# CompVis/retrieval-augmented-diffusion-models

Hardware: AMD Instinct MI355X
Metric: images/sec at 256x256, 50 DDIM steps, k=4 OpenImages retrieval (higher is better)
Workload: dtype bf16; 1 GPU; BASELINE config #3: RDM sampling, exact kNN (k=4) over a synthetic 20927907 x 512 fp16 CLIP DB -> 50-step DDIM (eta 0, CFG scale 2.0) over the shipped-config UNet (400.9M params, random weights) -> VQ-f4 decode to 256x256; batch_per_gpu=64, global_batch=64, sampler_steps=50, k=4, db_rows=20927907, parallelism=dp1 (batch-sharded, weights + DB replicated, all-gather of images only), deterministic_mode=False

## Files before the change

### include/rdm_hip.h

```cpp
#ifndef RDM_HIP_H
#define RDM_HIP_H
#include <stddef.h>
#include <stdint.h>

#ifdef __cplusplus
extern "C" {
#endif

typedef struct rdm_ctx rdm_ctx;

#define RDM_MAX_LEVELS 8

typedef struct {
    int in_channels, out_channels, model_channels, num_res_blocks;
    int n_attention_resolutions, attention_resolutions[RDM_MAX_LEVELS];
    int n_channel_mult, channel_mult[RDM_MAX_LEVELS];
    int num_head_channels, context_dim;
} rdm_unet_cfg;

typedef struct {
    int embed_dim, n_embed, z_channels, ch, n_ch_mult, ch_mult[RDM_MAX_LEVELS];
    int num_res_blocks, out_ch, resolution, mid_attn, kl;
    int n_attn_resolutions, attn_resolutions[RDM_MAX_LEVELS];
} rdm_vq_cfg;
// ... 45 lines not shown
    int lower_order_final;
    int log_every_t;
    int T; const float* alphas_cumprod;
    int n_nodes; const int* nodes;
} rdm_unipc_args;

typedef struct {
    int timesteps;
    int batch, k, channels, height, width;
    int clip_denoised; float temperature;
    int T;
    const float* sqrt_recip_alphas_cumprod; const float* sqrt_recipm1_alphas_cumprod;
    const float* posterior_mean_coef1; const float* posterior_mean_coef2;
    const float* posterior_log_variance_clipped;
} rdm_ddpm_args;

int rdm_ctx_create(int device_id, rdm_ctx** out);
void rdm_ctx_destroy(rdm_ctx* ctx);
const char* rdm_last_error(rdm_ctx* ctx);
int rdm_release_scratch(rdm_ctx* ctx);
int rdm_set_stream(rdm_ctx* ctx, void* hip_stream);
const char* rdm_version(void);
int rdm_set_deterministic(rdm_ctx* ctx, int on);
int rdm_get_deterministic(rdm_ctx* ctx);

long long rdm_unet_manifest(const rdm_unet_cfg* cfg, char* buf, size_t buflen, size_t* blob_bytes);
long long rdm_vq_manifest(const rdm_vq_cfg* cfg, char* buf, size_t buflen, size_t* blob_bytes);
long long rdm_clip_manifest(const rdm_clip_cfg* cfg, char* buf, size_t buflen, size_t* blob_bytes);
int rdm_load_unet(rdm_ctx* ctx, const rdm_unet_cfg* cfg, const void* packed, size_t nbytes);
int rdm_load_vq(rdm_ctx* ctx, const rdm_vq_cfg* cfg, const void* packed, size_t nbytes);
int rdm_load_clip(rdm_ctx* ctx, const rdm_clip_cfg* cfg, const void* packed, size_t nbytes);
long long rdm_rarm_manifest(const rdm_rarm_cfg* cfg, char* buf, size_t buflen, size_t* blob_bytes);
int rdm_load_rarm(rdm_ctx* ctx, const rdm_rarm_cfg* cfg, const void* packed, size_t nbytes);

int rdm_unet_forward(rdm_ctx* ctx, const float* x, const int64_t* t, const float* context, int b, int k, int H, int W,
                     float* eps_out);

int rdm_ddim_num_intermediates(int S, int log_every_t);
int rdm_ddim_sample(rdm_ctx* ctx, const rdm_ddim_args* args, const float* x_T, const float* cond, const float* uncond,
                    const float* noise, float* z_out, float* x_inter, float* pred_x0_inter);
int rdm_plms_sample(rdm_ctx* ctx, const rdm_ddim_args* args, const float* x_T, const float* cond, const float* uncond,
                    float* z_out, float* x_inter, float* pred_x0_inter);
int rdm_dpmpp_sample(rdm_ctx* ctx, const rdm_dpmpp_args* args, const float* x_T, const float* cond, const float* uncond,
                     float* z_out, float* x_inter, float* pred_x0_inter);
int rdm_dpmpp_timesteps(const float* alphas_cumprod, int T, int S, int skip_type, int* nodes_out);
int rdm_unipc_sample(rdm_ctx* ctx, const rdm_unipc_args* args, const float* x_T, const float* cond, const float* uncond,
                     float* z_out, float* x_inter, float* pred_x0_inter);
int rdm_unipc_coefficients(const float* alphas_cumprod, int T, const int* nodes, int n_nodes, int j, int order, int variant, int corrector,
                           int lower_order_final, double* out);
int rdm_ddpm_sample(rdm_ctx* ctx, const rdm_ddpm_args* args, const float* x_T, const float* cond, const float* noise,
                    float* z_out);

int rdm_rng_words(uint64_t seed, uint32_t row, uint32_t step, uint32_t stream, uint32_t block, uint32_t* out);
int rdm_op_rng_words(rdm_ctx* ctx, uint64_t seed, int64_t row0, int64_t B, int64_t per_row, uint32_t step, uint32_t stream, uint32_t* out);
int rdm_op_randn(rdm_ctx* ctx, uint64_t seed, int64_t row0, int64_t B, int64_t per_row, uint32_t step, uint32_t stream, float* out);
int rdm_ddim_sample_seeded(rdm_ctx* ctx, const rdm_ddim_args* args, uint64_t seed, int64_t row0, const float* x_T, const float* cond,
                           const float* uncond, float* z_out, float* x_inter, float* pred_x0_inter);
int rdm_ddpm_sample_seeded(rdm_ctx* ctx, const rdm_ddpm_args* args, uint64_t seed, int64_t row0, const float* x_T, const float* cond,
                           float* z_out);
int rdm_dpmpp_sde_sample(rdm_ctx* ctx, const rdm_dpmpp_args* args, const float* x_T, const float* cond, const float* uncond,
                         const float* noise, float* z_out, float* x_inter, float* pred_x0_inter);
int rdm_dpmpp_sde_sample_seeded(rdm_ctx* ctx, const rdm_dpmpp_args* args, uint64_t seed, int64_t row0, const float* x_T, const float* cond,
                                const float* uncond, float* z_out, float* x_inter, float* pred_x0_inter);

int rdm_ddim_decode(rdm_ctx* ctx, const rdm_ddim_args* args, int t_start, const float* x_latent, const float* cond, const float* uncond,
                    const float* noise, float* z_out, float* x_inter, float* pred_x0_inter);
int rdm_ddim_decode_seeded(rdm_ctx* ctx, const rdm_ddim_args* args, int t_start, uint64_t seed, int64_t row0, const float* x_latent,
                           const float* cond, const float* uncond, float* z_out, float* x_inter, float* pred_x0_inter);
int rdm_ddim_encode(rdm_ctx* ctx, const rdm_ddim_args* args, int t_enc, const float* x0, const float* cond, const float* uncond,
                    float* z_out, float* x_inter);
int rdm_op_ddim_inverse_step(rdm_ctx* ctx, const float* x, const float* eps, long long n, int cfg, float scale, float sqrt_a_cur,
                             float sqrt_one_minus_a_cur, float sqrt_a_next, float sqrt_one_minus_a_next, float* x_out,
                             float* x_dup_or_null, float* pred_x0_or_null);
int rdm_op_q_sample_seeded(rdm_ctx* ctx, const float* x0, int64_t B, int64_t per_row, float sqrt_a, float sqrt_1ma, uint64_t seed,
                           int64_t row0, float* out);

int rdm_op_masked_blend(rdm_ctx* ctx, const float* x, const float* x0, const float* mask, const float* z_or_null, int64_t B, int C, int H,
                        int W, int mask_channels, float sqrt_a, float sqrt_1ma, float* out, float* x_dup_or_null);
int rdm_op_masked_blend_seeded(rdm_ctx* ctx, const float* x, const float* x0, const float* mask, int64_t B, int C, int H, int W,
                               int mask_channels, float sqrt_a, float sqrt_1ma, uint64_t seed, int64_t row0, uint32_t step, float* out,
                               float* x_dup_or_null);
int rdm_ddim_inpaint(rdm_ctx* ctx, const rdm_ddim_args* args, int t_start, const float* x_latent, const float* x0, const float* mask,
                     int mask_channels, const float* cond, const float* uncond, const float* noise, const float* q_noise, float* z_out,
                     float* x_inter, float* pred_x0_inter);
int rdm_ddim_inpaint_seeded(rdm_ctx* ctx, const rdm_ddim_args* args, int t_start, uint64_t seed, int64_t row0, const float* x_latent,
                            const float* x0, const float* mask, int mask_channels, const float* cond, const float* uncond, float* z_out,
                            float* x_inter, float* pred_x0_inter);
int rdm_unet_forward_guided(rdm_ctx* ctx, const float* x, int64_t t, const float* cond, const float* uncond, int B, int k, int H, int W,
                            float* eps_out);

int rdm_vq_decode(rdm_ctx* ctx, const float* z, int b, int force_not_quantize, float* img_out, int32_t* indices_out);
int rdm_vq_quantize(rdm_ctx* ctx, const float* z, int b, float* zq_out, int32_t* indices_out);
int rdm_vq_decode_indices(rdm_ctx* ctx, const int64_t* indices, int b, float* img_out);
int rdm_vq_decode_hw(rdm_ctx* ctx, const float* z, int b, int h, int w, int force_not_quantize, float* img_out, int32_t* indices_out);
int rdm_vq_quantize_hw(rdm_ctx* ctx, const float* z, int b, int h, int w, float* zq_out, int32_t* indices_out);
long long rdm_vqenc_manifest(const rdm_vq_cfg* cfg, char* buf, size_t buflen, size_t* blob_bytes);
int rdm_load_vqenc(rdm_ctx* ctx, const rdm_vq_cfg* cfg, const void* packed, size_t nbytes);
int rdm_vq_encode(rdm_ctx* ctx, const float* img, int b, float* z_out);
int rdm_vq_encode_indices(rdm_ctx* ctx, const float* img , int b, int64_t* indices_out ,
                          float* quant_out_or_null );
int rdm_vq_encode_hw(rdm_ctx* ctx, const float* img, int b, int H, int W, float* z_out);
int rdm_to_uint8(rdm_ctx* ctx, const float* img, int b, int c, int h, int w, uint8_t* out);

int rdm_rarm_forward(rdm_ctx* ctx, const int64_t* tokens, int b, int t, const float* context, int k, float* logits_out);
int rdm_rarm_sample(rdm_ctx* ctx, const rdm_rarm_sample_args* args, const int64_t* cond_tokens, const float* context,
                    const float* uniforms, int64_t* tokens_out);
int rdm_rarm_sample_top_p(rdm_ctx* ctx, const rdm_rarm_sample_args* args, float top_p, const int64_t* cond_tokens, const float* context,
                          const float* uniforms, int64_t* tokens_out);
int rdm_rarm_forward_seq(rdm_ctx* ctx, const int64_t* tokens, int b, int t, const float* context, int k, float* logits_out);
int rdm_rarm_nll(rdm_ctx* ctx, const int64_t* tokens, const int64_t* targets, int b, int t, const float* context, int k, float* nll_out);
int rdm_rarm_sample_prefill(rdm_ctx* ctx, const rdm_rarm_sample_args* args, float top_p, const int64_t* cond_tokens, const float* context,
                            const float* uniforms, int64_t* tokens_out);

int rdm_clip_encode_text(rdm_ctx* ctx, const int64_t* tokens, int b, float* out);
int rdm_clip_encode_image(rdm_ctx* ctx, const float* image, int b, float* out);
int rdm_clip_preprocess(rdm_ctx* ctx, const float* image, int b, int h, int w, float* out);
int rdm_clip_encode_image_raw(rdm_ctx* ctx, const float* image, int b, int h, int w, float* out);

int rdm_db_load(rdm_ctx* ctx, const void* emb, long long n, int dim, int dtype, int is_device);
long long rdm_db_size(rdm_ctx* ctx);
int rdm_knn(rdm_ctx* ctx, const float* q, int b, int k, uint32_t* idx_out, float* score_out);
int rdm_knn_f64(rdm_ctx* ctx, const float* q, int b, int k, uint32_t* idx_out, double* score_out);
int rdm_knn_last_fallback(rdm_ctx* ctx);
int rdm_db_gather(rdm_ctx* ctx, const uint32_t* idx, long long n_idx, float* out);
enum { RDM_KNN_SCAN_GENERIC = 1, RDM_KNN_SCAN_D512 = 2, RDM_KNN_SCAN_BULK = 3 };
typedef struct rdm_knn_form { int path, ksel, rescored, lists_per_block, queries_per_launch; float eps; } rdm_knn_form;
typedef struct rdm_knn_stages {
    int rows_cap, nlists_cap;
    float* qn; void* qh; void* ql;
    float* cand_s; uint32_t* cand_i;
    int* flag; double* tau; uint32_t* tau_idx; float* theta;
    int rows, nlists; rdm_knn_form form;
} rdm_knn_stages;
int rdm_knn_select(long long n, int dim, int b, int k, rdm_knn_form* form_out);
int rdm_op_knn_stages(rdm_ctx* ctx, const float* q, int b, int k, uint32_t* idx_out, float* score_out, rdm_knn_stages* stages);
int rdm_db_rows(rdm_ctx* ctx, long long row0, long long rows, void* out_f16);

int rdm_comm_unique_id(rdm_ctx* ctx, void* id128 );
int rdm_comm_init(rdm_ctx* ctx, const void* id128 , int rank, int world);
int rdm_comm_all_gather(rdm_ctx* ctx, const void* send , void* recv , size_t nbytes);
int rdm_comm_all_reduce_f32(rdm_ctx* ctx, float* buf , size_t count, int average);
int rdm_comm_destroy(rdm_ctx* ctx);

enum { RDM_PROF_CONV3X3 = 0, RDM_PROF_LINEAR = 1, RDM_PROF_KNN = 2, RDM_PROF_ATTENTION = 3, RDM_PROF_GROUPNORM = 4,
       RDM_PROF_LAYERNORM = 5,
       RDM_PROF_UPSCONV = 6  };
int rdm_prof_enable(rdm_ctx* ctx, int kind_mask);
int rdm_prof_collect(rdm_ctx* ctx, int kind, long long* launches, double* ms, double* flops);
int rdm_prof_reset(rdm_ctx* ctx);
int rdm_prof_dump(rdm_ctx* ctx, const char* path);
int rdm_calib_probe(rdm_ctx* ctx, void* buf , size_t buf_bytes, double mfma_ms, size_t stream_bytes, int stream_reps,
                    double* mfma_tflops , double* stream_gbps );
int rdm_debug_tap(rdm_ctx* ctx, void* buf , size_t nbytes, int block, int sub);

int rdm_op_linear(rdm_ctx* ctx, const void* a_bf16, const void* w_bf16, const float* bias, const void* residual_bf16,
                  void* out_bf16, float* out_f32, int M, int N, int K, int act, float alpha);
int rdm_op_linear_rowvec(rdm_ctx* ctx, const void* a_bf16, const void* w_bf16, const float* bias, const float* rowvec, int rows_per_group,
                         const void* residual_bf16, void* out_bf16, int M, int N, int K);
int rdm_op_linear_ln(rdm_ctx* ctx, const void* x_bf16, const void* w_bf16, const float* bias, const float* gamma, const float* beta,
                     void* out_bf16, int M, int N, int K, int act, float eps);
int rdm_op_conv3x3(rdm_ctx* ctx, const void* x0_bf16, const void* x1_bf16, int C0, int C1, const void* w_bf16,
                   const float* bias, const float* rowvec, int rowvec_ld, const void* residual_bf16, void* out_bf16,
                   int B, int Hin, int Win, int N, int stride, int ups);
int rdm_op_vq_nearest_code(rdm_ctx* ctx, const float* z , const float* codebook , long long M, int N, int E,
                           int32_t* idx_out );
int rdm_op_moments_f64(rdm_ctx* ctx, const float* x, int n, int d, double* sum, double* outer);
int rdm_op_knn_radius(rdm_ctx* ctx, const float* x, int n, int d, int k, float* radius2_out);
int rdm_op_manifold_hits(rdm_ctx* ctx, const float* probe , int m, const float* ref , const float* ref_radius2, int n, int d,
                         unsigned char* hit_out);
int rdm_op_manifold_counts(rdm_ctx* ctx, const float* probe , int m, const float* ref , const float* ref_radius2 ,
                           int n, int d, int32_t* count_out );
int rdm_op_nearest_d2(rdm_ctx* ctx, const float* probe , int m, const float* ref , int n, int d, float* d2_out );
int rdm_op_poly3_rowsums(rdm_ctx* ctx, const float* probe , int m, const float* ref , int n, int d, int groups,
                         int exclude_same_index, float gamma, float coef0, double* rowsum_out );
int rdm_op_rarm_sampler(rdm_ctx* ctx, const float* logits, int b, int vocab, int cfg, float guidance_scale, float temperature,
                        int top_k, const float* uniforms, int64_t* tokens_out);
int rdm_op_rarm_sampler_top_p(rdm_ctx* ctx, const float* logits, int b, int vocab, int cfg, float guidance_scale, float temperature,
                              int top_k, float top_p, const float* uniforms, int64_t* tokens_out, int32_t* kept_out);
int rdm_op_conv3x3_dgrad(rdm_ctx* ctx, const void* dy_bf16 , const void* w_bf16, void* dx_bf16 , int B, int H, int W,
                         int C, int N);
int rdm_op_conv3x3_wgrad(rdm_ctx* ctx, const void* x_bf16 , const void* dy_bf16 , float* dw , int B, int H,
                         int W, int C, int N);
int rdm_op_groupnorm_bwd(rdm_ctx* ctx, const void* x_bf16, const void* dy_bf16, const float* gamma, const float* beta, int B, int HW, int C,
                         float eps, int silu, void* dx_bf16, float* dgamma, float* dbeta);
int rdm_op_layernorm_bwd(rdm_ctx* ctx, const void* x_bf16, const void* dy_bf16, const float* gamma, int M, int C, float eps, void* dx_bf16,
                         float* dgamma, float* dbeta);
int rdm_op_groupnorm_bwd_add(rdm_ctx* ctx, const void* x_bf16, const void* dy_bf16, const float* gamma, const float* beta, int B, int HW, int C,
                             float eps, int silu, const void* residual_bf16, void* dx_bf16, float* dgamma, float* dbeta);
int rdm_op_layernorm_bwd_add(rdm_ctx* ctx, const void* x_bf16, const void* dy_bf16, const float* gamma, int M, int C, float eps,
                             const void* residual_bf16, void* dx_bf16, float* dgamma, float* dbeta);
int rdm_op_linear_wgrad(rdm_ctx* ctx, const void* dy_bf16, const void* a_bf16, float* dw, long long M, int N, int K);
enum { RDM_WGRAD_CONV9_LW4 = 1, RDM_WGRAD_CONV9_LW5 = 2, RDM_WGRAD_CONV9_LW6 = 3, RDM_WGRAD_TN9 = 4, RDM_WGRAD_TN1 = 5, RDM_WGRAD_CONV_FALLBACK = 6,
       RDM_WGRAD_LINEAR_FALLBACK = 7 };
typedef struct rdm_wgrad_form { int path, Z, per_plane, remap; } rdm_wgrad_form;
int rdm_wgrad_select(int conv, int B, int H, int W, int C, int N, long long M, int K, rdm_wgrad_form* form_out);
int rdm_op_colsum(rdm_ctx* ctx, const void* x_bf16 , float* out , long long M, int N);
int rdm_op_transpose(rdm_ctx* ctx, const void* x_bf16 , void* y_bf16 , int rows, int cols);
int rdm_op_add(rdm_ctx* ctx, const void* a_bf16, const void* b_bf16, void* out_bf16, long long n);
int rdm_op_ddim_step(rdm_ctx* ctx, const float* x, const float* eps, const float* noise_or_null, long long n, int cfg, float scale, float a_t,
                     float a_prev, float sigma_t, float sqrt_one_minus_at, float temperature, float* x_prev, float* x_dup_or_null,
                     float* pred_x0_or_null);
int rdm_op_ddim_step_seeded(rdm_ctx* ctx, const float* x, const float* eps, long long n, int64_t per_row, int cfg, float scale, float a_t,
                            float a_prev, float sigma_t, float sqrt_one_minus_at, float temperature, uint64_t seed, int64_t row0,
                            uint32_t step, float* x_prev, float* x_dup_or_null, float* pred_x0_or_null);
int rdm_op_plms_step(rdm_ctx* ctx, const float* x, const float* eps, const float* e_prev_or_null, const float* h1_or_null,
                     const float* h2_or_null, const float* h3_or_null, long long n, int cfg, float scale, float a_t, float a_prev,
                     float sqrt_one_minus_at, int mode, int order, float* e_store_or_null, float* x_out, float* x_dup_or_null,
                     float* pred_x0_or_null);
int rdm_op_ddpm_step(rdm_ctx* ctx, const float* x, const float* eps, const float* noise_or_null, long long n, float sqrt_recip,
                     float sqrt_recipm1, float coef1, float coef2, float log_var, int clip, int nonzero, float temperature, float* x_prev);
int rdm_op_ddpm_step_seeded(rdm_ctx* ctx, const float* x, const float* eps, long long n, int64_t per_row, float sqrt_recip, float sqrt_recipm1,
                            float coef1, float coef2, float log_var, int clip, int nonzero, float temperature, uint64_t seed, int64_t row0,
                            uint32_t step, float* x_prev);
int rdm_op_dpmpp_step(rdm_ctx* ctx, const float* x, const float* eps, const float* m_prev_or_null, long long n, int cfg, float scale,
                      float sqrt_a_s, float sqrt_one_minus_a_s, float c_x, float c_0, float c_1, float* x_out, float* x_dup_or_null,
                      float* m_store_or_null, float* pred_x0_or_null);
int rdm_op_dpmpp_sde_step(rdm_ctx* ctx, const float* x, const float* eps, const float* m_prev_or_null, const float* noise, long long n, int cfg,
                          float scale, float sqrt_a_s, float sqrt_one_minus_a_s, float c_x, float c_0, float c_1, float c_n, float* x_out,
                          float* x_dup_or_null, float* m_store_or_null, float* pred_x0_or_null);
int rdm_op_dpmpp_sde_step_seeded(rdm_ctx* ctx, const float* x, const float* eps, const float* m_prev_or_null, long long n, int64_t per_row,
                                 int cfg, float scale, float sqrt_a_s, float sqrt_one_minus_a_s, float c_x, float c_0, float c_1, float c_n,
                                 uint64_t seed, int64_t row0, uint32_t step, float* x_out, float* x_dup_or_null, float* m_store_or_null,
                                 float* pred_x0_or_null);
int rdm_op_unipc_step(rdm_ctx* ctx, const float* u, const float* eps, const float* xc_prev_or_null, const float* h1_or_null,
                      const float* h2_or_null, const float* h3_or_null, long long n, int cfg, float scale, const double* coefficients,
                      float* xc_out_or_null, float* u_next, float* x_dup_or_null, float* m_store_or_null, float* pred_x0_or_null);
int rdm_op_silu(rdm_ctx* ctx, const float* x, const float* dy_or_null, void* out_bf16_or_f32, long long n);
int rdm_op_sumpool2(rdm_ctx* ctx, const void* x_bf16, void* out_bf16, int B, int H, int W, int C);
int rdm_op_q_sample(rdm_ctx* ctx, const float* x0, const float* noise, const float* sqrt_ac, const float* sqrt_1mac, float* out_or_null,
                    void* out_nhwc_bf16_or_null, int B, int C, int H, int W, int cpad);
int rdm_op_mse_loss(rdm_ctx* ctx, const void* eps_nhwc_bf16, const float* target, const float* coef_or_null, float* se, void* deps_nhwc_bf16_or_null,
                    int B, int C, int H, int W, int ldc);
int rdm_op_where_rows(rdm_ctx* ctx, const unsigned char* mask, const float* a, const float* x, float* out, long long rows, long long n);
int rdm_op_timestep_embedding(rdm_ctx* ctx, const int64_t* t, void* out_bf16, int B, int dim, int ld);
int rdm_op_colsum_samples(rdm_ctx* ctx, const void* x_bf16, void* out_bf16, int B, int HW, int N);
int rdm_op_expand2(rdm_ctx* ctx, const void* x_bf16, void* out_bf16, int B, int H, int W, int C, int mode);
int rdm_op_ema(rdm_ctx* ctx, float* shadow, const float* param, long long n, float one_minus_decay);
int rdm_op_adamw(rdm_ctx* ctx, float* p, const float* grad, float* exp_avg, float* exp_avg_sq, void* p_bf16_or_null, long long n, double lr,
                 double beta1, double beta2, double eps, double weight_decay, int step);
int rdm_op_adamw_multi(rdm_ctx* ctx, int n, float* const* p, const float* const* grad, float* const* exp_avg, float* const* exp_avg_sq,
                       void* const* p_bf16_or_null, const long long* numel, double lr, double beta1, double beta2, double eps, double weight_decay, int step);
int rdm_op_ema_multi(rdm_ctx* ctx, int n, float* const* shadow, const float* const* param, const long long* numel, float one_minus_decay);
int rdm_op_attention_bwd(rdm_ctx* ctx, const void* q, const void* k, const void* v, const void* o, const void* dout, int B, int n, int m, int heads,
                         void* dq, void* dk, void* dv);
int rdm_op_bmm(rdm_ctx* ctx, const void* a_bf16, const void* w_bf16, void* out_bf16_or_null, float* out_f32_or_null, int batch, int M, int N, int K,
               float alpha);
int rdm_op_heads(rdm_ctx* ctx, const void* x_bf16, void* out_bf16, int B, int n, int H, int D, int ldx, int mode);
int rdm_op_transpose_batched(rdm_ctx* ctx, const void* x_bf16, void* y_bf16, int batch, int rows, int cols);
int rdm_op_softmax(rdm_ctx* ctx, const float* scores, void* p_bf16, long long rows, int n, int n_valid );
int rdm_op_softmax_bwd(rdm_ctx* ctx, const void* p_bf16, const float* dp, void* ds_bf16, long long rows, int n);
int rdm_op_geglu(rdm_ctx* ctx, const void* pre_bf16, const void* dh_bf16_or_null, void* out_bf16, long long M, int F);
int rdm_op_groupnorm(rdm_ctx* ctx, const void* x0_bf16, const void* x1_bf16, int C0, int C1, int B, int HW,
                     const float* gamma, const float* beta, float eps, int silu, void* out_bf16);
int rdm_op_layernorm(rdm_ctx* ctx, const void* x, int in_is_f32, const float* gamma, const float* beta, int M, int C,
                     float eps, void* out_bf16);
int rdm_op_layernorm_f32(rdm_ctx* ctx, const float* x, const float* gamma, const float* beta, int M, int C, float eps, float* out_f32);
int rdm_op_linear_res_f32(rdm_ctx* ctx, const void* a_bf16, const void* w_bf16, const float* bias, const float* res_f32, float* out_f32,
                          int M, int N, int K, int act);
int rdm_op_self_attention(rdm_ctx* ctx, const void* qk_bf16, const void* vt_bf16, int B, int n, int heads,
                          void* out_bf16);
int rdm_op_self_attention_qkv(rdm_ctx* ctx, const void* qkv_bf16, int B, int n, int heads, void* out_bf16);
int rdm_op_xattn_fused(rdm_ctx* ctx, const void* x_bf16, const float* ln_gamma, const float* ln_beta, float ln_eps, const void* G_bf16,
                       const void* U_bf16, const float* bias, const void* res_bf16, int B, int n, int C, int NP, int ncols, int group,
                       void* out_bf16);
int rdm_op_xattn_fused_ln3(rdm_ctx* ctx, void* x_bf16_inout, const float* ln_gamma, const float* ln_beta, float ln_eps, const void* G_bf16,
                           const void* U_bf16, const float* bias, int B, int n, int C, int NP, int ncols, int group,
                           const float* ln3_gamma, const float* ln3_beta, void* ln3_out_bf16);
int rdm_op_causal_attention_d64(rdm_ctx* ctx, const void* qkv_bf16, int ldq, int B, int n, int heads, float scale, void* out_bf16, int ldo,
                                void* kcache_bf16_or_null, void* vcache_bf16_or_null, int L);
enum { RDM_LINEAR_ROWS_REFUSED = 0, RDM_LINEAR_ROWS_SGEMM = 1, RDM_LINEAR_ROWS_MGEMM = 2, RDM_LINEAR_ROWS_TILED = 3 };
typedef struct rdm_linear_rows_form { int kernel, ma, nb, u, nw, ln, geglu; } rdm_linear_rows_form;
int rdm_linear_rows_select(int M, int N, int K, int act, int ln, int deterministic, rdm_linear_rows_form* form_out);
int rdm_op_linear_rows(rdm_ctx* ctx, const void* a_bf16_or_null, const float* ln_x_f32_or_null, const float* ln_gamma, const float* ln_beta,
                       const void* w_bf16, const float* bias_or_null, const float* res_f32_or_null, void* out_bf16_or_null, float* out_f32_or_null,
                       int M, int N, int K, int act);
int rdm_op_rarm_decode_attention(rdm_ctx* ctx, const void* q_bf16, int ldq, const void* k_new_bf16_or_null, const void* v_new_bf16_or_null,
                                 void* kcache_bf16, void* vcache_bf16, long long batch_stride, int row_stride, long long head_stride, int nkv, int pos,
                                 float scale, void* out_bf16, int ldo, int heads, int batch);
int rdm_op_rarm_xattn_decode(rdm_ctx* ctx, float* x_f32_inout, const float* ln_gamma, const float* ln_beta, float ln_eps, const void* G_bf16,
                             const void* UT_bf16, const float* bias, int B2, int Bc, int C, int NP, int heads, int k, const float* ln3_gamma_or_null,
                             const float* ln3_beta_or_null, void* ln3_out_bf16_or_null);
int rdm_op_rarm_embed(rdm_ctx* ctx, const int64_t* tokens, int tok_ld, int tok_rows, int seq0, const float* emb_f32, const float* pos_t_f32,
                      float* x_f32, long long rows, int t, int C, int vocab, int L, int pos);
int rdm_op_vq_attention(rdm_ctx* ctx, const void* q_bf16, int ldq, const void* k_bf16, int ldk, const void* v_bf16, int ldv,
                        const float* bias_v_or_null, int B, int n, int C, float scale, void* out_bf16, int ldo);
int rdm_op_rarm_nll(rdm_ctx* ctx, const float* logits, long long rows, int vocab, const int64_t* targets, float* nll_out);
int rdm_op_causal_attention_d64_bwd(rdm_ctx* ctx, const void* qkv_bf16, int ldq, const void* out_bf16, int ldo, const void* dout_bf16, int lddo,
                                    int B, int n, int heads, float scale, void* dqkv_bf16, int ldd);
int rdm_op_rarm_nll_bwd(rdm_ctx* ctx, const float* logits, long long rows, int vocab, const int64_t* targets, float gscale, void* dlogits_bf16,
                        float* nll_out_or_null);
int rdm_op_embedding_grad(rdm_ctx* ctx, const int64_t* tokens, const void* dy_bf16, int M, int C, int V, float* dw_f32);
int rdm_op_head_conv(rdm_ctx* ctx, const void* x_bf16, const float* gn_gamma, const float* gn_beta, float gn_eps, const float* w,
                     const float* bias, int B, int H, int W, int C, int Cout, float* out_f32);
int rdm_op_small_attention(rdm_ctx* ctx, const void* q_bf16, int ldq, const void* k_bf16, const void* v_bf16, int ldkv,
                           int B, int nq, int nkv, int heads, int D, int causal, float scale, void* out_bf16, int ldo);
int rdm_op_small_attention_bwd(rdm_ctx* ctx, const void* q_bf16, int ldq, const void* k_bf16, const void* v_bf16, int ldkv, const void* dout_bf16, int ldo,
                               int B, int nq, int nkv, int heads, float scale, void* dq_bf16, void* dk_bf16, void* dv_bf16);
int rdm_op_conv_in(rdm_ctx* ctx, const float* x_f32, const float* w_f32, const float* bias_f32, int B, int Cin, int H, int W, int Cout,
                   void* out_bf16);
int rdm_op_conv_out(rdm_ctx* ctx, const void* x_bf16, const float* w_f32, const float* bias_f32, int B, int H, int W, int Cin, int Cout,
                    float* out_f32);

#ifdef __cplusplus
}
#endif
#endif
// ... 1 lines not shown
```

### retrieval-augmented-diffusion-models_amd/_lib.py

```python
import ctypes as C
import os

import numpy as np
import torch

_HERE = os.path.dirname(os.path.abspath(__file__))
LIB_PATH = os.environ.get("RDM_HIP_LIB") or os.path.join(_HERE, "librdm_hip.so")

RDM_MAX_LEVELS = 8
ACT_NONE, ACT_GEGLU, ACT_QUICKGELU, ACT_SILU = 0, 1, 2, 3
PROF_CONV3X3, PROF_LINEAR, PROF_KNN, PROF_ATTENTION, PROF_GROUPNORM, PROF_LAYERNORM, PROF_UPSCONV = range(7)


class UNetCfg(C.Structure):
    _fields_ = [("in_channels", C.c_int), ("out_channels", C.c_int), ("model_channels", C.c_int),
                ("num_res_blocks", C.c_int), ("n_attention_resolutions", C.c_int),
                ("attention_resolutions", C.c_int * RDM_MAX_LEVELS), ("n_channel_mult", C.c_int),
                ("channel_mult", C.c_int * RDM_MAX_LEVELS), ("num_head_channels", C.c_int), ("context_dim", C.c_int)]


class VqCfg(C.Structure):
    _fields_ = [("embed_dim", C.c_int), ("n_embed", C.c_int), ("z_channels", C.c_int), ("ch", C.c_int),
                ("n_ch_mult", C.c_int), ("ch_mult", C.c_int * RDM_MAX_LEVELS), ("num_res_blocks", C.c_int),
                ("out_ch", C.c_int), ("resolution", C.c_int), ("mid_attn", C.c_int), ("kl", C.c_int),
# ... 8 lines not shown
class RarmSampleArgs(C.Structure):
    _fields_ = [("batch", C.c_int), ("k", C.c_int), ("cond_len", C.c_int), ("steps", C.c_int), ("temperature", C.c_float),
                ("top_k", C.c_int), ("guidance_scale", C.c_float)]


class LinearRowsForm(C.Structure):
    _fields_ = [("kernel", C.c_int), ("ma", C.c_int), ("nb", C.c_int), ("u", C.c_int), ("nw", C.c_int), ("ln", C.c_int), ("geglu", C.c_int)]


LINEAR_ROWS_REFUSED, LINEAR_ROWS_SGEMM, LINEAR_ROWS_MGEMM, LINEAR_ROWS_TILED = range(4)


class WgradForm(C.Structure):
    _fields_ = [("path", C.c_int), ("Z", C.c_int), ("per_plane", C.c_int), ("remap", C.c_int)]


WGRAD_PATHS = (None, "conv9<4>", "conv9<5>", "conv9<6>", "tn9", "tn1", "conv_fallback", "linear_fallback")


class ClipCfg(C.Structure):
    _fields_ = [("embed_dim", C.c_int), ("image_resolution", C.c_int), ("vision_layers", C.c_int),
                ("vision_width", C.c_int), ("vision_patch_size", C.c_int), ("context_length", C.c_int),
                ("vocab_size", C.c_int), ("transformer_width", C.c_int), ("transformer_heads", C.c_int),
                ("transformer_layers", C.c_int)]


class DdimArgs(C.Structure):
    _fields_ = [("S", C.c_int), ("batch", C.c_int), ("k", C.c_int), ("channels", C.c_int), ("height", C.c_int),
                ("width", C.c_int), ("eta", C.c_float), ("temperature", C.c_float),
                ("unconditional_guidance_scale", C.c_float), ("log_every_t", C.c_int), ("T", C.c_int),
                ("alphas_cumprod", C.POINTER(C.c_float))]


class DpmppArgs(C.Structure):
    _fields_ = [("batch", C.c_int), ("k", C.c_int), ("channels", C.c_int), ("height", C.c_int), ("width", C.c_int),
                ("unconditional_guidance_scale", C.c_float), ("order", C.c_int), ("lower_order_final", C.c_int),
                ("log_every_t", C.c_int), ("T", C.c_int), ("alphas_cumprod", C.POINTER(C.c_float)), ("n_nodes", C.c_int),
                ("nodes", C.POINTER(C.c_int))]


DPMPP_SKIP_TYPES = {"time_uniform": 0, "logSNR": 1}


class UnipcArgs(C.Structure):
    _fields_ = [("batch", C.c_int), ("k", C.c_int), ("channels", C.c_int), ("height", C.c_int), ("width", C.c_int),
                ("unconditional_guidance_scale", C.c_float), ("order", C.c_int), ("variant", C.c_int), ("corrector", C.c_int),
                ("lower_order_final", C.c_int), ("log_every_t", C.c_int), ("T", C.c_int), ("alphas_cumprod", C.POINTER(C.c_float)),
                ("n_nodes", C.c_int), ("nodes", C.POINTER(C.c_int))]


UNIPC_VARIANTS = {"bh1": 0, "bh2": 1}
UNIPC_COEFFICIENTS = ("alpha", "sigma", "a_x", "a_t", "a_1", "a_2", "a_3", "b_x", "b_0", "b_1", "b_2", "order_c", "order_p")
PLMS_STEP, PLMS_EULER_A, PLMS_EULER_B = 0, 1, 2


class DdpmArgs(C.Structure):
    _fields_ = [("timesteps", C.c_int), ("batch", C.c_int), ("k", C.c_int), ("channels", C.c_int), ("height", C.c_int),
                ("width", C.c_int), ("clip_denoised", C.c_int), ("temperature", C.c_float), ("T", C.c_int),
                ("sqrt_recip_alphas_cumprod", C.POINTER(C.c_float)), ("sqrt_recipm1_alphas_cumprod", C.POINTER(C.c_float)),
                ("posterior_mean_coef1", C.POINTER(C.c_float)), ("posterior_mean_coef2", C.POINTER(C.c_float)),
                ("posterior_log_variance_clipped", C.POINTER(C.c_float))]


KNN_SCAN_PATHS = (None, "generic", "d512", "bulk")


class KnnForm(C.Structure):
    _fields_ = [("path", C.c_int), ("ksel", C.c_int), ("rescored", C.c_int), ("lists_per_block", C.c_int), ("queries_per_launch", C.c_int),
                ("eps", C.c_float)]


class KnnStages(C.Structure):
    _fields_ = [("rows_cap", C.c_int), ("nlists_cap", C.c_int), ("qn", C.c_void_p), ("qh", C.c_void_p), ("ql", C.c_void_p),
                ("cand_s", C.c_void_p), ("cand_i", C.c_void_p), ("flag", C.c_void_p), ("tau", C.c_void_p), ("tau_idx", C.c_void_p),
                ("theta", C.c_void_p), ("rows", C.c_int), ("nlists", C.c_int), ("form", KnnForm)]


_P = C.c_void_p
SIGNATURES = {
    "rdm_ctx_create": (C.c_int, [C.c_int, C.POINTER(_P)]),
    "rdm_ctx_destroy": (None, [_P]),
    "rdm_last_error": (C.c_char_p, [_P]),
    "rdm_set_stream": (C.c_int, [_P, _P]),
    "rdm_version": (C.c_char_p, []),
    "rdm_unet_manifest": (C.c_longlong, [C.POINTER(UNetCfg), C.c_char_p, C.c_size_t, C.POINTER(C.c_size_t)]),
    "rdm_vq_manifest": (C.c_longlong, [C.POINTER(VqCfg), C.c_char_p, C.c_size_t, C.POINTER(C.c_size_t)]),
    "rdm_clip_manifest": (C.c_longlong, [C.POINTER(ClipCfg), C.c_char_p, C.c_size_t, C.POINTER(C.c_size_t)]),
    "rdm_load_unet": (C.c_int, [_P, C.POINTER(UNetCfg), _P, C.c_size_t]),
    "rdm_load_vq": (C.c_int, [_P, C.POINTER(VqCfg), _P, C.c_size_t]),
    "rdm_load_clip": (C.c_int, [_P, C.POINTER(ClipCfg), _P, C.c_size_t]),
    "rdm_rarm_manifest": (C.c_longlong, [C.POINTER(RarmCfg), C.c_char_p, C.c_size_t, C.POINTER(C.c_size_t)]),
    "rdm_load_rarm": (C.c_int, [_P, C.POINTER(RarmCfg), _P, C.c_size_t]),
    "rdm_rarm_forward": (C.c_int, [_P, _P, C.c_int, C.c_int, _P, C.c_int, _P]),
    "rdm_rarm_sample": (C.c_int, [_P, C.POINTER(RarmSampleArgs), _P, _P, _P, _P]),
    "rdm_rarm_sample_top_p": (C.c_int, [_P, C.POINTER(RarmSampleArgs), C.c_float, _P, _P, _P, _P]),
    "rdm_rarm_forward_seq": (C.c_int, [_P, _P, C.c_int, C.c_int, _P, C.c_int, _P]),
    "rdm_rarm_nll": (C.c_int, [_P, _P, _P, C.c_int, C.c_int, _P, C.c_int, _P]),
    "rdm_rarm_sample_prefill": (C.c_int, [_P, C.POINTER(RarmSampleArgs), C.c_float, _P, _P, _P, _P]),
    "rdm_vq_decode_indices": (C.c_int, [_P, _P, C.c_int, _P]),
    "rdm_unet_forward": (C.c_int, [_P, _P, _P, _P, C.c_int, C.c_int, C.c_int, C.c_int, _P]),
    "rdm_ddim_num_intermediates": (C.c_int, [C.c_int, C.c_int]),
    "rdm_ddim_sample": (C.c_int, [_P, C.POINTER(DdimArgs), _P, _P, _P, _P, _P, _P, _P]),
    "rdm_plms_sample": (C.c_int, [_P, C.POINTER(DdimArgs), _P, _P, _P, _P, _P, _P]),
    "rdm_dpmpp_sample": (C.c_int, [_P, C.POINTER(DpmppArgs), _P, _P, _P, _P, _P, _P]),
    "rdm_dpmpp_timesteps": (C.c_int, [C.POINTER(C.c_float), C.c_int, C.c_int, C.c_int, C.POINTER(C.c_int)]),
    "rdm_unipc_sample": (C.c_int, [_P, C.POINTER(UnipcArgs), _P, _P, _P, _P, _P, _P]),
    "rdm_unipc_coefficients": (C.c_int, [C.POINTER(C.c_float), C.c_int, C.POINTER(C.c_int), C.c_int, C.c_int, C.c_int, C.c_int, C.c_int,
                                         C.c_int, C.POINTER(C.c_double)]),
    "rdm_ddpm_sample": (C.c_int, [_P, C.POINTER(DdpmArgs), _P, _P, _P, _P]),
    "rdm_rng_words": (C.c_int, [C.c_uint64, C.c_uint32, C.c_uint32, C.c_uint32, C.c_uint32, C.POINTER(C.c_uint32)]),
    "rdm_op_rng_words": (C.c_int, [_P, C.c_uint64, C.c_int64, C.c_int64, C.c_int64, C.c_uint32, C.c_uint32, _P]),
    "rdm_op_randn": (C.c_int, [_P, C.c_uint64, C.c_int64, C.c_int64, C.c_int64, C.c_uint32, C.c_uint32, _P]),
    "rdm_ddim_sample_seeded": (C.c_int, [_P, C.POINTER(DdimArgs), C.c_uint64, C.c_int64, _P, _P, _P, _P, _P, _P]),
    "rdm_ddpm_sample_seeded": (C.c_int, [_P, C.POINTER(DdpmArgs), C.c_uint64, C.c_int64, _P, _P, _P]),
    "rdm_dpmpp_sde_sample": (C.c_int, [_P, C.POINTER(DpmppArgs), _P, _P, _P, _P, _P, _P, _P]),
    "rdm_dpmpp_sde_sample_seeded": (C.c_int, [_P, C.POINTER(DpmppArgs), C.c_uint64, C.c_int64, _P, _P, _P, _P, _P, _P]),
    "rdm_unet_forward_guided": (C.c_int, [_P, _P, C.c_int64, _P, _P, C.c_int, C.c_int, C.c_int, C.c_int, _P]),
    "rdm_ddim_decode": (C.c_int, [_P, C.POINTER(DdimArgs), C.c_int, _P, _P, _P, _P, _P, _P, _P]),
    "rdm_ddim_decode_seeded": (C.c_int, [_P, C.POINTER(DdimArgs), C.c_int, C.c_uint64, C.c_int64, _P, _P, _P, _P, _P, _P]),
    "rdm_ddim_encode": (C.c_int, [_P, C.POINTER(DdimArgs), C.c_int, _P, _P, _P, _P, _P]),
    "rdm_op_ddim_inverse_step": (C.c_int, [_P, _P, _P, C.c_longlong, C.c_int, C.c_float, C.c_float, C.c_float, C.c_float, C.c_float, _P, _P, _P]),
    "rdm_op_q_sample_seeded": (C.c_int, [_P, _P, C.c_int64, C.c_int64, C.c_float, C.c_float, C.c_uint64, C.c_int64, _P]),
    "rdm_op_masked_blend": (C.c_int, [_P, _P, _P, _P, _P, C.c_int64, C.c_int, C.c_int, C.c_int, C.c_int, C.c_float, C.c_float, _P, _P]),
    "rdm_op_masked_blend_seeded": (C.c_int, [_P, _P, _P, _P, C.c_int64, C.c_int, C.c_int, C.c_int, C.c_int, C.c_float, C.c_float, C.c_uint64,
                                             C.c_int64, C.c_uint32, _P, _P]),
    "rdm_ddim_inpaint": (C.c_int, [_P, C.POINTER(DdimArgs), C.c_int, _P, _P, _P, C.c_int, _P, _P, _P, _P, _P, _P, _P]),
    "rdm_ddim_inpaint_seeded": (C.c_int, [_P, C.POINTER(DdimArgs), C.c_int, C.c_uint64, C.c_int64, _P, _P, _P, C.c_int, _P, _P, _P, _P, _P]),
    "rdm_vq_decode": (C.c_int, [_P, _P, C.c_int, C.c_int, _P, _P]),
    "rdm_release_scratch": (C.c_int, [_P]),
    "rdm_vq_quantize": (C.c_int, [_P, _P, C.c_int, _P, _P]),
    "rdm_vq_decode_hw": (C.c_int, [_P, _P, C.c_int, C.c_int, C.c_int, C.c_int, _P, _P]),
    "rdm_vq_quantize_hw": (C.c_int, [_P, _P, C.c_int, C.c_int, C.c_int, _P, _P]),
    "rdm_to_uint8": (C.c_int, [_P, _P, C.c_int, C.c_int, C.c_int, C.c_int, _P]),
    "rdm_clip_encode_text": (C.c_int, [_P, _P, C.c_int, _P]),
    "rdm_clip_encode_image": (C.c_int, [_P, _P, C.c_int, _P]),
    "rdm_clip_preprocess": (C.c_int, [_P, _P, C.c_int, C.c_int, C.c_int, _P]),
    "rdm_clip_encode_image_raw": (C.c_int, [_P, _P, C.c_int, C.c_int, C.c_int, _P]),
    "rdm_db_load": (C.c_int, [_P, _P, C.c_longlong, C.c_int, C.c_int, C.c_int]),
    "rdm_db_size": (C.c_longlong, [_P]),
    "rdm_knn": (C.c_int, [_P, _P, C.c_int, C.c_int, _P, _P]),
    "rdm_knn_f64": (C.c_int, [_P, _P, C.c_int, C.c_int, _P, _P]),
    "rdm_knn_last_fallback": (C.c_int, [_P]),
    "rdm_db_gather": (C.c_int, [_P, _P, C.c_longlong, _P]),
    "rdm_knn_select": (C.c_int, [C.c_longlong, C.c_int, C.c_int, C.c_int, C.POINTER(KnnForm)]),
    "rdm_op_knn_stages": (C.c_int, [_P, _P, C.c_int, C.c_int, _P, _P, C.POINTER(KnnStages)]),
    "rdm_db_rows": (C.c_int, [_P, C.c_longlong, C.c_longlong, _P]),
    "rdm_set_deterministic": (C.c_int, [_P, C.c_int]),
    "rdm_get_deterministic": (C.c_int, [_P]),
    "rdm_prof_enable": (C.c_int, [_P, C.c_int]),
    "rdm_prof_collect": (C.c_int, [_P, C.c_int, C.POINTER(C.c_longlong), C.POINTER(C.c_double), C.POINTER(C.c_double)]),
    "rdm_prof_reset": (C.c_int, [_P]),
    "rdm_prof_dump": (C.c_int, [_P, C.c_char_p]),
    "rdm_debug_tap": (C.c_int, [_P, _P, C.c_size_t, C.c_int, C.c_int]),
    "rdm_calib_probe": (C.c_int, [_P, _P, C.c_size_t, C.c_double, C.c_size_t, C.c_int, C.POINTER(C.c_double), C.POINTER(C.c_double)]),
    "rdm_comm_unique_id": (C.c_int, [_P, _P]),
    "rdm_comm_init": (C.c_int, [_P, _P, C.c_int, C.c_int]),
    "rdm_comm_all_gather": (C.c_int, [_P, _P, _P, C.c_size_t]),
    "rdm_comm_all_reduce_f32": (C.c_int, [_P, _P, C.c_size_t, C.c_int]),
    "rdm_comm_destroy": (C.c_int, [_P]),
    "rdm_vqenc_manifest": (C.c_longlong, [_P, _P, C.c_size_t, _P]),
    "rdm_load_vqenc": (C.c_int, [_P, _P, _P, C.c_size_t]),
    "rdm_vq_encode": (C.c_int, [_P, _P, C.c_int, _P]),
    "rdm_vq_encode_hw": (C.c_int, [_P, _P, C.c_int, C.c_int, C.c_int, _P]),
    "rdm_vq_encode_indices": (C.c_int, [_P, _P, C.c_int, _P, _P]),
    "rdm_op_q_sample": (C.c_int, [_P, _P, _P, _P, _P, _P, _P, C.c_int, C.c_int, C.c_int, C.c_int, C.c_int]),
    "rdm_op_mse_loss": (C.c_int, [_P, _P, _P, _P, _P, _P, C.c_int, C.c_int, C.c_int, C.c_int, C.c_int]),
    "rdm_op_where_rows": (C.c_int, [_P, _P, _P, _P, _P, C.c_longlong, C.c_longlong]),
    "rdm_op_timestep_embedding": (C.c_int, [_P, _P, _P, C.c_int, C.c_int, C.c_int]),
    "rdm_op_colsum_samples": (C.c_int, [_P, _P, _P, C.c_int, C.c_int, C.c_int]),
    "rdm_op_expand2": (C.c_int, [_P, _P, _P, C.c_int, C.c_int, C.c_int, C.c_int, C.c_int]),
    "rdm_op_linear": (C.c_int, [_P, _P, _P, _P, _P, _P, _P, C.c_int, C.c_int, C.c_int, C.c_int, C.c_float]),
    "rdm_op_conv3x3": (C.c_int, [_P, _P, _P, C.c_int, C.c_int, _P, _P, _P, C.c_int, _P, _P, C.c_int, C.c_int, C.c_int,
                                 C.c_int, C.c_int, C.c_int]),
    "rdm_op_vq_nearest_code": (C.c_int, [_P, _P, _P, C.c_longlong, C.c_int, C.c_int, _P]),
    "rdm_op_moments_f64": (C.c_int, [_P, _P, C.c_int, C.c_int, _P, _P]),
    "rdm_op_knn_radius": (C.c_int, [_P, _P, C.c_int, C.c_int, C.c_int, _P]),
    "rdm_op_manifold_hits": (C.c_int, [_P, _P, C.c_int, _P, _P, C.c_int, C.c_int, _P]),
    "rdm_op_manifold_counts": (C.c_int, [_P, _P, C.c_int, _P, _P, C.c_int, C.c_int, _P]),
    "rdm_op_nearest_d2": (C.c_int, [_P, _P, C.c_int, _P, C.c_int, C.c_int, _P]),
    "rdm_op_poly3_rowsums": (C.c_int, [_P, _P, C.c_int, _P, C.c_int, C.c_int, C.c_int, C.c_int, C.c_float, C.c_float, _P]),
    "rdm_op_rarm_sampler": (C.c_int, [_P, _P, C.c_int, C.c_int, C.c_int, C.c_float, C.c_float, C.c_int, _P, _P]),
    "rdm_op_rarm_sampler_top_p": (C.c_int, [_P, _P, C.c_int, C.c_int, C.c_int, C.c_float, C.c_float, C.c_int, C.c_float, _P, _P, _P]),
    "rdm_op_conv3x3_dgrad": (C.c_int, [_P, _P, _P, _P, C.c_int, C.c_int, C.c_int, C.c_int, C.c_int]),
    "rdm_op_conv3x3_wgrad": (C.c_int, [_P, _P, _P, _P, C.c_int, C.c_int, C.c_int, C.c_int, C.c_int]),
    "rdm_op_groupnorm_bwd": (C.c_int, [_P, _P, _P, _P, _P, C.c_int, C.c_int, C.c_int, C.c_float, C.c_int, _P, _P, _P]),
    "rdm_op_layernorm_bwd": (C.c_int, [_P, _P, _P, _P, C.c_int, C.c_int, C.c_float, _P, _P, _P]),
    "rdm_op_groupnorm_bwd_add": (C.c_int, [_P, _P, _P, _P, _P, C.c_int, C.c_int, C.c_int, C.c_float, C.c_int, _P, _P, _P, _P]),
    "rdm_op_layernorm_bwd_add": (C.c_int, [_P, _P, _P, _P, C.c_int, C.c_int, C.c_float, _P, _P, _P, _P]),
    "rdm_op_colsum": (C.c_int, [_P, _P, _P, C.c_longlong, C.c_int]),
    "rdm_op_transpose": (C.c_int, [_P, _P, _P, C.c_int, C.c_int]),
    "rdm_op_add": (C.c_int, [_P, _P, _P, _P, C.c_longlong]),
    "rdm_op_dpmpp_step": (C.c_int, [_P, _P, _P, _P, C.c_longlong, C.c_int, C.c_float, C.c_float, C.c_float, C.c_float, C.c_float, C.c_float,
                                    _P, _P, _P, _P]),
    "rdm_op_dpmpp_sde_step": (C.c_int, [_P, _P, _P, _P, _P, C.c_longlong, C.c_int, C.c_float, C.c_float, C.c_float, C.c_float, C.c_float,
                                        C.c_float, C.c_float, _P, _P, _P, _P]),
    "rdm_op_dpmpp_sde_step_seeded": (C.c_int, [_P, _P, _P, _P, C.c_longlong, C.c_int64, C.c_int, C.c_float, C.c_float, C.c_float, C.c_float,
                                               C.c_float, C.c_float, C.c_float, C.c_uint64, C.c_int64, C.c_uint32, _P, _P, _P, _P]),
    "rdm_op_unipc_step": (C.c_int, [_P, _P, _P, _P, _P, _P, _P, C.c_longlong, C.c_int, C.c_float, C.POINTER(C.c_double), _P, _P, _P, _P, _P]),
    "rdm_op_ddim_step": (C.c_int, [_P, _P, _P, _P, C.c_longlong, C.c_int, C.c_float, C.c_float, C.c_float, C.c_float, C.c_float, C.c_float,
                                   _P, _P, _P]),
    "rdm_op_ddim_step_seeded": (C.c_int, [_P, _P, _P, C.c_longlong, C.c_int64, C.c_int, C.c_float, C.c_float, C.c_float, C.c_float, C.c_float,
                                          C.c_float, C.c_uint64, C.c_int64, C.c_uint32, _P, _P, _P]),
    "rdm_op_plms_step": (C.c_int, [_P, _P, _P, _P, _P, _P, _P, C.c_longlong, C.c_int, C.c_float, C.c_float, C.c_float, C.c_float, C.c_int,
                                   C.c_int, _P, _P, _P, _P]),
    "rdm_op_ddpm_step": (C.c_int, [_P, _P, _P, _P, C.c_longlong, C.c_float, C.c_float, C.c_float, C.c_float, C.c_float, C.c_int, C.c_int,
                                   C.c_float, _P]),
    "rdm_op_ddpm_step_seeded": (C.c_int, [_P, _P, _P, C.c_longlong, C.c_int64, C.c_float, C.c_float, C.c_float, C.c_float, C.c_float, C.c_int,
                                          C.c_int, C.c_float, C.c_uint64, C.c_int64, C.c_uint32, _P]),
    "rdm_op_geglu": (C.c_int, [_P, _P, _P, _P, C.c_longlong, C.c_int]),
    "rdm_op_linear_ln": (C.c_int, [_P, _P, _P, _P, _P, _P, _P, C.c_int, C.c_int, C.c_int, C.c_int, C.c_float]),
    "rdm_op_linear_wgrad": (C.c_int, [_P, _P, _P, _P, C.c_longlong, C.c_int, C.c_int]),
    "rdm_op_ema": (C.c_int, [_P, _P, _P, C.c_longlong, C.c_float]),
    "rdm_op_silu": (C.c_int, [_P, _P, _P, _P, C.c_longlong]),
    "rdm_op_sumpool2": (C.c_int, [_P, _P, _P, C.c_int, C.c_int, C.c_int, C.c_int]),
    "rdm_op_adamw": (C.c_int, [_P, _P, _P, _P, _P, _P, C.c_longlong, C.c_double, C.c_double, C.c_double, C.c_double, C.c_double, C.c_int]),
    "rdm_op_attention_bwd": (C.c_int, [_P, _P, _P, _P, _P, _P, C.c_int, C.c_int, C.c_int, C.c_int, _P, _P, _P]),
    "rdm_op_bmm": (C.c_int, [_P, _P, _P, _P, _P, C.c_int, C.c_int, C.c_int, C.c_int, C.c_float]),
    "rdm_op_heads": (C.c_int, [_P, _P, _P, C.c_int, C.c_int, C.c_int, C.c_int, C.c_int, C.c_int]),
    "rdm_op_transpose_batched": (C.c_int, [_P, _P, _P, C.c_int, C.c_int, C.c_int]),
    "rdm_op_softmax": (C.c_int, [_P, _P, _P, C.c_longlong, C.c_int, C.c_int]),
    "rdm_op_softmax_bwd": (C.c_int, [_P, _P, _P, _P, C.c_longlong, C.c_int]),
    "rdm_op_groupnorm": (C.c_int, [_P, _P, _P, C.c_int, C.c_int, C.c_int, C.c_int, _P, _P, C.c_float, C.c_int, _P]),
    "rdm_op_layernorm": (C.c_int, [_P, _P, C.c_int, _P, _P, C.c_int, C.c_int, C.c_float, _P]),
    "rdm_op_layernorm_f32": (C.c_int, [_P, _P, _P, _P, C.c_int, C.c_int, C.c_float, _P]),
    "rdm_op_linear_res_f32": (C.c_int, [_P, _P, _P, _P, _P, _P, C.c_int, C.c_int, C.c_int, C.c_int]),
    "rdm_op_self_attention": (C.c_int, [_P, _P, _P, C.c_int, C.c_int, C.c_int, _P]),
    "rdm_op_self_attention_qkv": (C.c_int, [_P, _P, C.c_int, C.c_int, C.c_int, _P]),
    "rdm_op_head_conv": (C.c_int, [_P, _P, _P, _P, C.c_float, _P, _P, C.c_int, C.c_int, C.c_int, C.c_int, C.c_int, _P]),
    "rdm_op_conv_in": (C.c_int, [_P, _P, _P, _P, C.c_int, C.c_int, C.c_int, C.c_int, C.c_int, _P]),
    "rdm_op_conv_out": (C.c_int, [_P, _P, _P, _P, C.c_int, C.c_int, C.c_int, C.c_int, C.c_int, _P]),
    "rdm_op_linear_rowvec": (C.c_int, [_P, _P, _P, _P, _P, C.c_int, _P, _P, C.c_int, C.c_int, C.c_int]),
    "rdm_op_xattn_fused_ln3": (C.c_int, [_P, _P, _P, _P, C.c_float, _P, _P, _P, C.c_int, C.c_int, C.c_int, C.c_int, C.c_int, C.c_int, _P, _P, _P]),
    "rdm_op_xattn_fused": (C.c_int, [_P, _P, _P, _P, C.c_float, _P, _P, _P, _P, C.c_int, C.c_int, C.c_int, C.c_int, C.c_int, C.c_int, _P]),
    "rdm_op_causal_attention_d64": (C.c_int, [_P, _P, C.c_int, C.c_int, C.c_int, C.c_int, C.c_float, _P, C.c_int, _P, _P, C.c_int]),
    "rdm_op_rarm_nll": (C.c_int, [_P, _P, C.c_longlong, C.c_int, _P, _P]),
    "rdm_linear_rows_select": (C.c_int, [C.c_int, C.c_int, C.c_int, C.c_int, C.c_int, C.c_int, C.POINTER(LinearRowsForm)]),
    "rdm_op_linear_rows": (C.c_int, [_P, _P, _P, _P, _P, _P, _P, _P, _P, _P, C.c_int, C.c_int, C.c_int, C.c_int]),
    "rdm_wgrad_select": (C.c_int, [C.c_int, C.c_int, C.c_int, C.c_int, C.c_int, C.c_int, C.c_longlong, C.c_int, C.POINTER(WgradForm)]),
    "rdm_op_rarm_decode_attention": (C.c_int, [_P, _P, C.c_int, _P, _P, _P, _P, C.c_longlong, C.c_int, C.c_longlong, C.c_int, C.c_int, C.c_float, _P,
                                               C.c_int, C.c_int, C.c_int]),
    "rdm_op_rarm_xattn_decode": (C.c_int, [_P, _P, _P, _P, C.c_float, _P, _P, _P, C.c_int, C.c_int, C.c_int, C.c_int, C.c_int, C.c_int, _P, _P, _P]),
    "rdm_op_rarm_embed": (C.c_int, [_P, _P, C.c_int, C.c_int, C.c_int, _P, _P, _P, C.c_longlong, C.c_int, C.c_int, C.c_int, C.c_int, C.c_int]),
    "rdm_op_vq_attention": (C.c_int, [_P, _P, C.c_int, _P, C.c_int, _P, C.c_int, _P, C.c_int, C.c_int, C.c_int, C.c_float, _P, C.c_int]),
    "rdm_op_causal_attention_d64_bwd": (C.c_int, [_P, _P, C.c_int, _P, C.c_int, _P, C.c_int, C.c_int, C.c_int, C.c_int, C.c_float, _P, C.c_int]),
    "rdm_op_rarm_nll_bwd": (C.c_int, [_P, _P, C.c_longlong, C.c_int, _P, C.c_float, _P, _P]),
    "rdm_op_embedding_grad": (C.c_int, [_P, _P, _P, C.c_int, C.c_int, C.c_int, _P]),
    "rdm_op_small_attention": (C.c_int, [_P, _P, C.c_int, _P, _P, C.c_int, C.c_int, C.c_int, C.c_int, C.c_int, C.c_int,
                                         C.c_int, C.c_float, _P, C.c_int]),
    "rdm_op_adamw_multi": (C.c_int, [_P, C.c_int, _P, _P, _P, _P, _P, _P, C.c_double, C.c_double, C.c_double, C.c_double, C.c_double, C.c_int]),
    "rdm_op_ema_multi": (C.c_int, [_P, C.c_int, _P, _P, _P, C.c_float]),
    "rdm_op_small_attention_bwd": (C.c_int, [_P, _P, C.c_int, _P, _P, C.c_int, _P, C.c_int, C.c_int, C.c_int, C.c_int, C.c_int, C.c_float, _P, _P, _P]),
}


def load_library(path: str = LIB_PATH):
    if not os.path.exists(path):
        raise ImportError(
            f"librdm_hip.so not found at {path}. Build it with `python -c 'import __graft_entry__ as g; g.build()'` "
            f"(or `make -C retrieval-augmented-diffusion-models_amd/csrc`). There is no CPU fallback.")
    lib = C.CDLL(path)
    for name, (res, args) in SIGNATURES.items():
        fn = getattr(lib, name)
        fn.restype, fn.argtypes = res, args
    return lib


lib = load_library()


def linear_rows_select(M, N, K, act=ACT_NONE, ln=False, deterministic=False):
    f = LinearRowsForm()
    rc = lib.rdm_linear_rows_select(int(M), int(N), int(K), int(act), int(bool(ln)), int(bool(deterministic)), C.byref(f))
    if rc != 0:
        raise RdmError(f"rdm_linear_rows_select({M}, {N}, {K}, act={act}, ln={ln}, deterministic={deterministic}) failed ({rc})")
    if f.kernel == LINEAR_ROWS_SGEMM:
        return ("sgemm", f.ma, f.nb, f.u, f.nw, bool(f.ln), bool(f.geglu))
    return (("refused", "sgemm", "mgemm", "tiled")[f.kernel],)


def wgrad_select(*shape):
    f = WgradForm()
    if len(shape) == 5:
        B, H, W, Cc, N = (int(v) for v in shape)
        rc = lib.rdm_wgrad_select(1, B, H, W, Cc, N, 0, 0, C.byref(f))
    elif len(shape) == 3:
        M, N, K = (int(v) for v in shape)
        rc = lib.rdm_wgrad_select(0, 0, 0, 0, 0, N, M, K, C.byref(f))
    else:
        raise RdmError(f"wgrad_select takes (B, H, W, C, N) or (M, N, K), got {shape}")
    if rc != 0:
        raise RdmError(f"rdm_wgrad_select{shape} failed ({rc})")
    return (WGRAD_PATHS[f.path], f.Z, f.per_plane, f.remap)


def knn_select(n, dim, b, k):
    f = KnnForm()
    if lib.rdm_knn_select(int(n), int(dim), int(b), int(k), C.byref(f)) != 0:
        raise RdmError(f"rdm_knn_select(n={n}, dim={dim}, b={b}, k={k}): arguments the search refuses")
    return {"path": KNN_SCAN_PATHS[f.path], "ksel": f.ksel, "rescored": f.rescored, "lists_per_block": f.lists_per_block,
            "queries_per_launch": f.queries_per_launch, "eps": float(f.eps)}


def _ptr(t):
    if t is None:
        return None
    if isinstance(t, torch.Tensor):
# ... 828 lines not shown

    def clip_encode_image(self, image):
        image = self._dev(image, torch.float32)
        cfg = self._need("clip_encode_image", "clip")
        if image.ndim != 4 or tuple(image.shape[1:]) != (3, cfg.image_resolution, cfg.image_resolution):
            raise RdmError(f"clip_encode_image: image must be [b,3,{cfg.image_resolution},{cfg.image_resolution}] (already resized / normalised), got {tuple(image.shape)}")
        out = torch.empty((image.shape[0], self.clip_cfg.embed_dim), device=self.device, dtype=torch.float32)
        self._check(lib.rdm_clip_encode_image(self._h, _ptr(image), image.shape[0], _ptr(out)))
        return out

    def clip_preprocess(self, image):
        image = self._dev(image, torch.float32)
        if image.ndim != 4 or image.shape[1] != 3:
            raise RdmError(f"clip_preprocess: image must be [b,3,h,w], got {tuple(image.shape)}")
        r = self._need("clip_preprocess", "clip").image_resolution
        out = torch.empty((image.shape[0], 3, r, r), device=self.device, dtype=torch.float32)
        self._check(lib.rdm_clip_preprocess(self._h, _ptr(image), image.shape[0], image.shape[2], image.shape[3], _ptr(out)))
        return out

    def clip_encode_image_raw(self, image):
        image = self._dev(image, torch.float32)
        if image.ndim != 4 or image.shape[1] != 3:
            raise RdmError(f"clip_encode_image_raw: image must be [b,3,h,w], got {tuple(image.shape)}")
        self._need("clip_encode_image_raw", "clip")
        out = torch.empty((image.shape[0], self.clip_cfg.embed_dim), device=self.device, dtype=torch.float32)
        self._check(lib.rdm_clip_encode_image_raw(self._h, _ptr(image), image.shape[0], image.shape[2], image.shape[3], _ptr(out)))
        return out

    def db_load(self, emb):
        if isinstance(emb, torch.Tensor) and emb.is_cuda:
            emb = emb.contiguous()
            dt = {torch.float16: 0, torch.float32: 1}[emb.dtype]
            self._check(lib.rdm_db_load(self._h, _ptr(emb), emb.shape[0], emb.shape[1], dt, 1))
            self._db_dim = int(emb.shape[1])
        else:
            emb = np.ascontiguousarray(emb.numpy() if isinstance(emb, torch.Tensor) else emb)
            dt = {np.dtype(np.float16): 0, np.dtype(np.float32): 1}[emb.dtype]
            self._check(lib.rdm_db_load(self._h, emb.ctypes.data_as(_P), emb.shape[0], emb.shape[1], dt, 0))
            self._db_dim = int(emb.shape[1])

    def db_size(self):
        return int(lib.rdm_db_size(self._h))

    def knn(self, q, k, f64=False):
        q = self._dev(q, torch.float32)
        if q.ndim != 2:
            raise RdmError(f"knn: queries must be [b,dim], got {tuple(q.shape)}")
        idx = torch.empty((q.shape[0], k), device=self.device, dtype=torch.int32)
        sc = torch.empty((q.shape[0], k), device=self.device, dtype=torch.float64 if f64 else torch.float32)
        fn = lib.rdm_knn_f64 if f64 else lib.rdm_knn
        self._check(fn(self._h, _ptr(q), q.shape[0], k, _ptr(idx), _ptr(sc)))
        return idx, sc

    def knn_last_fallback(self):
        return int(lib.rdm_knn_last_fallback(self._h))

    def knn_stages(self, q, k):
        q = self._dev(q, torch.float32)
        if q.ndim != 2:
            raise RdmError(f"knn_stages: queries must be [b,dim], got {tuple(q.shape)}")
        b, dim = q.shape
        n = self.db_size()
        form = knn_select(n, dim, b, k)
        rows = form["queries_per_launch"]
        ntiles = (n + 255) // 256
        cap = 8 * min(ntiles, torch.cuda.get_device_properties(self.device).multi_processor_count)
        dv = self.device
        t = {"idx": torch.empty((b, k), device=dv, dtype=torch.int32), "score": torch.empty((b, k), device=dv, dtype=torch.float32),
             "qn": torch.zeros((rows, dim), device=dv, dtype=torch.float32), "qh": torch.zeros((rows, dim), device=dv, dtype=torch.float16),
             "ql": torch.zeros((rows, dim), device=dv, dtype=torch.float16),
             "cand_s": torch.zeros(rows * cap * form["ksel"], device=dv, dtype=torch.float32),
             "cand_i": torch.zeros(rows * cap * form["ksel"], device=dv, dtype=torch.int32),
             "flag": torch.zeros(b, device=dv, dtype=torch.int32), "tau": torch.zeros(b, device=dv, dtype=torch.float64),
             "tau_idx": torch.zeros(b, device=dv, dtype=torch.int32), "theta": torch.zeros(b, device=dv, dtype=torch.float32)}
        st = KnnStages(rows_cap=rows, nlists_cap=cap)
        for name in ("qn", "qh", "ql", "cand_s", "cand_i", "flag", "tau", "tau_idx", "theta"):
            setattr(st, name, t[name].data_ptr())
        self._check(lib.rdm_op_knn_stages(self._h, _ptr(q), b, k, _ptr(t["idx"]), _ptr(t["score"]), C.byref(st)))
        used = st.rows * st.nlists * st.form.ksel
        for name in ("qn", "qh", "ql"):
            t[name] = t[name][:st.rows]
        for name in ("cand_s", "cand_i"):
            t[name] = t[name][:used].reshape(st.rows, st.nlists, st.form.ksel)
        t.update(form)
        return t

    def db_rows(self, row0, rows):
        dim = self._db_dim
        out = torch.empty((rows, dim), device=self.device, dtype=torch.float16)
        self._check(lib.rdm_db_rows(self._h, int(row0), int(rows), _ptr(out)))
        return out

    def db_gather(self, idx, dim):
        idx = idx.contiguous()
        out = torch.empty((idx.numel(), dim), device=self.device, dtype=torch.float32)
        self._check(lib.rdm_db_gather(self._h, _ptr(idx), idx.numel(), _ptr(out)))
        return out.reshape(tuple(idx.shape) + (dim,))

    def prof_enable(self, kinds=(0, 1)):
        if kinds is True:
            kinds = (PROF_CONV3X3, PROF_LINEAR)
        mask = 0
        for k in (kinds or ()):
            mask |= 1 << int(k)
        self._check(lib.rdm_prof_enable(self._h, mask))

    def set_deterministic(self, on: bool = True):
        self._check(lib.rdm_set_deterministic(self._h, int(bool(on))))

    @property
    def deterministic(self) -> bool:
        return lib.rdm_get_deterministic(self._h) == 1

    def comm_unique_id(self) -> bytes:
        buf = C.create_string_buffer(128)
        self._check(lib.rdm_comm_unique_id(self._h, buf))
        return buf.raw

    def new_comm_context(self):
        c = Context(self.device.index)
        c._side_stream = torch.cuda.Stream(self.device)
        c._check(lib.rdm_set_stream(c._h, C.c_void_p(c._side_stream.cuda_stream)))
        return c

    def comm_init(self, uid: bytes, rank: int, world: int):
        if len(uid) != 128:
            raise RdmError(f"comm_init: the unique id is 128 bytes, got {len(uid)}")
        self._check(lib.rdm_comm_init(self._h, C.create_string_buffer(uid, 128), int(rank), int(world)))
        self.comm_world = int(world)

    def comm_all_gather(self, local: torch.Tensor, world: int) -> torch.Tensor:
        local = local.contiguous()
        out = torch.empty((world,) + tuple(local.shape), device=self.device, dtype=local.dtype)
        self._check(lib.rdm_comm_all_gather(self._h, _ptr(local), _ptr(out), local.numel() * local.element_size()))
        return out

    def comm_all_reduce(self, buf: torch.Tensor, average=True):
        if buf.dtype != torch.float32 or not buf.is_contiguous():
            raise RdmError("comm_all_reduce: contiguous float32 tensor required")
        self._check(lib.rdm_comm_all_reduce_f32(self._h, _ptr(buf), buf.numel(), int(bool(average))))
        return buf

    def comm_destroy(self):
        self._check(lib.rdm_comm_destroy(self._h))
        self.comm_world = 0

    def prof_reset(self):
        self._check(lib.rdm_prof_reset(self._h))

    def debug_tap(self, buf, block, sub=0):
        self._tap_keepalive = buf
        self._check(lib.rdm_debug_tap(self._h, _ptr(buf) if buf is not None else None, 0 if buf is None else buf.numel() * buf.element_size(), int(block), int(sub)))

    def calib_probe(self, mfma_ms=800.0, stream_bytes=1 << 30, stream_reps=6):
        buf = torch.empty(max(1 << 20, 2 * stream_bytes), device=self.device, dtype=torch.uint8)
        tf, gb = C.c_double(0.0), C.c_double(0.0)
        self._check(lib.rdm_calib_probe(self._h, _ptr(buf), buf.numel(), float(mfma_ms), int(stream_bytes), int(stream_reps), C.byref(tf), C.byref(gb)))
        del buf
        return float(tf.value), float(gb.value)

    def prof_dump(self, path):
        self._check(lib.rdm_prof_dump(self._h, os.fsencode(path)))

    def prof_collect(self, kind):
        n, ms, fl = C.c_longlong(0), C.c_double(0), C.c_double(0)
        self._check(lib.rdm_prof_collect(self._h, kind, C.byref(n), C.byref(ms), C.byref(fl)))
        return int(n.value), float(ms.value), float(fl.value)

    def op_linear(self, a, w, bias=None, residual=None, act=ACT_NONE, alpha=1.0, out_f32=False):
        M, K = a.shape; N = w.shape[0]
        No = N // 2 if act == ACT_GEGLU else N
        ob = None if out_f32 else torch.empty((M, No), device=self.device, dtype=torch.bfloat16)
        of = torch.empty((M, No), device=self.device, dtype=torch.float32) if out_f32 else None
        self._check(lib.rdm_op_linear(self._h, _ptr(a), _ptr(w), _ptr(bias), _ptr(residual), _ptr(ob), _ptr(of), M, N, K,
                                      act, float(alpha)))
        return of if out_f32 else ob

    def op_linear_rowvec(self, a, w, bias, rowvec, rows_per_group, residual=None):
        M, K = a.shape; N = w.shape[0]
        assert rowvec.dtype == torch.float32 and rowvec.shape == ((M + rows_per_group - 1) // rows_per_group, N) and rowvec.is_contiguous()
        out = torch.empty((M, N), device=self.device, dtype=torch.bfloat16)
        self._check(lib.rdm_op_linear_rowvec(self._h, _ptr(a), _ptr(w), _ptr(bias), _ptr(rowvec), int(rows_per_group), _ptr(residual), _ptr(out), M, N, K))
        return out

    def op_linear_ln(self, x, w, bias, gamma, beta, act=ACT_NONE, eps=1e-5):
        M, K = x.shape; N = w.shape[0]
        out = torch.empty((M, N // 2 if act == ACT_GEGLU else N), device=self.device, dtype=torch.bfloat16)
        self._check(lib.rdm_op_linear_ln(self._h, _ptr(x), _ptr(w), _ptr(bias), _ptr(gamma), _ptr(beta), _ptr(out), M, N, K, act, float(eps)))
        return out

    def op_conv3x3(self, x0, w, bias, x1=None, rowvec=None, residual=None, stride=1, ups=0):
        B, Hin, Win, C0 = x0.shape
        C1 = 0 if x1 is None else x1.shape[3]
        N = w.shape[0]
        Ho = Hin * 2 if ups else (Hin // 2 if stride == 2 else Hin)
        Wo = Win * 2 if ups else (Win // 2 if stride == 2 else Win)
        out = torch.empty((B, Ho, Wo, N), device=self.device, dtype=torch.bfloat16)
        self._check(lib.rdm_op_conv3x3(self._h, _ptr(x0), _ptr(x1), C0, C1, _ptr(w), _ptr(bias), _ptr(rowvec),
                                       0 if rowvec is None else rowvec.shape[1], _ptr(residual), _ptr(out), B, Hin, Win, N,
                                       stride, ups))
        return out

    def op_rarm_sampler(self, logits, uniforms, guidance_scale=1.0, temperature=1.0, top_k=None, top_p=None, return_kept=False):
        top_p = check_top_p("op_rarm_sampler", top_p)
        logits = self._dev(logits, torch.float32); uniforms = self._dev(uniforms, torch.float32)
        b = uniforms.shape[0]
        cfg = guidance_scale > 1.0
        if logits.ndim != 2 or logits.shape[0] != (2 * b if cfg else b):
            raise RdmError(f"op_rarm_sampler: logits must be [{2 * b if cfg else b}, vocab], got {tuple(logits.shape)}")
        out = torch.empty((b,), device=self.device, dtype=torch.int64)
        k = int(top_k) if top_k is not None else 0
        if top_p is None and not return_kept:
            self._check(lib.rdm_op_rarm_sampler(self._h, _ptr(logits), b, logits.shape[1], int(cfg), float(guidance_scale), float(temperature),
                                                k, _ptr(uniforms), _ptr(out)))
            return out
        kept = torch.empty((b,), device=self.device, dtype=torch.int32) if return_kept else None
        self._check(lib.rdm_op_rarm_sampler_top_p(self._h, _ptr(logits), b, logits.shape[1], int(cfg), float(guidance_scale), float(temperature),
                                                  k, 1.0 if top_p is None else top_p, _ptr(uniforms), _ptr(out), _ptr(kept)))
        return (out, kept) if return_kept else out

    def op_conv3x3_dgrad(self, dy, w):
        B, H, W, N = dy.shape
        Cc = w.shape[3]
        dx = torch.empty((B, H, W, Cc), device=self.device, dtype=torch.bfloat16)
        self._check(lib.rdm_op_conv3x3_dgrad(self._h, _ptr(dy), _ptr(w), _ptr(dx), B, H, W, Cc, N))
        return dx

    def op_conv3x3_wgrad(self, x, dy):
        B, H, W, Cc = x.shape
        N = dy.shape[3]
        dw = torch.empty((N, 3, 3, Cc), device=self.device, dtype=torch.float32)
        self._check(lib.rdm_op_conv3x3_wgrad(self._h, _ptr(x), _ptr(dy), _ptr(dw), B, H, W, Cc, N))
        return dw

    def op_groupnorm_bwd(self, x, dy, gamma, beta, eps, silu, residual=None):
        B, HW, Cc = x.shape
        dx = torch.empty_like(x); dg = torch.empty((Cc,), device=self.device, dtype=torch.float32); db = torch.empty_like(dg)
        assert residual is None or (residual.is_contiguous() and residual.numel() == x.numel())
        self._check(lib.rdm_op_groupnorm_bwd_add(self._h, _ptr(x), _ptr(dy), _ptr(gamma), _ptr(beta), B, HW, Cc, float(eps), int(silu), _ptr(residual),
                                                 _ptr(dx), _ptr(dg), _ptr(db)))
        return dx, dg, db

    def op_layernorm_bwd(self, x, dy, gamma, eps=1e-5, residual=None):
        M, Cc = x.shape
        dx = torch.empty_like(x); dg = torch.empty((Cc,), device=self.device, dtype=torch.float32); db = torch.empty_like(dg)
        assert residual is None or (residual.is_contiguous() and residual.numel() == x.numel())
        self._check(lib.rdm_op_layernorm_bwd_add(self._h, _ptr(x), _ptr(dy), _ptr(gamma), M, Cc, float(eps), _ptr(residual), _ptr(dx), _ptr(dg), _ptr(db)))
        return dx, dg, db

    def op_colsum(self, x):
        M, N = x.shape
        out = torch.empty((N,), device=self.device, dtype=torch.float32)
        self._check(lib.rdm_op_colsum(self._h, _ptr(x), _ptr(out), M, N))
        return out

    def op_transpose(self, x):
        r, c_ = x.shape
        y = torch.empty((c_, r), device=self.device, dtype=torch.bfloat16)
        self._check(lib.rdm_op_transpose(self._h, _ptr(x), _ptr(y), r, c_))
        return y

    def op_add(self, a, b):
        out = torch.empty_like(a)
        self._check(lib.rdm_op_add(self._h, _ptr(a), _ptr(b), _ptr(out), a.numel()))
        return out

    def op_linear_wgrad(self, dy, a):
        M, N = dy.shape; K = a.shape[1]
        dw = torch.empty((N, K), device=self.device, dtype=torch.float32)
        self._check(lib.rdm_op_linear_wgrad(self._h, _ptr(dy), _ptr(a), _ptr(dw), M, N, K))
        return dw

    @staticmethod
    def _ptr_array(ts, optional=False):
        arr = (C.c_void_p * len(ts))()
        for i, t in enumerate(ts):
            if t is None:
                assert optional
                arr[i] = None
            else:
                assert t.is_contiguous(), "tensor must be contiguous"
                arr[i] = t.data_ptr()
        return arr

    def op_adamw_multi(self, ps, gs, ms, vs, step, lr=1e-3, betas=(0.9, 0.999), eps=1e-8, weight_decay=1e-2, p_bf16s=None):
        n = len(ps)
        assert n == len(gs) == len(ms) == len(vs) and all(g.numel() == p.numel() and g.dtype == torch.float32 for p, g in zip(ps, gs))
        numel = (C.c_longlong * n)(*[p.numel() for p in ps])
        self._check(lib.rdm_op_adamw_multi(self._h, n, self._ptr_array(ps), self._ptr_array(gs), self._ptr_array(ms), self._ptr_array(vs),
                                           self._ptr_array(p_bf16s, True) if p_bf16s is not None else None, numel, float(lr), float(betas[0]),
                                           float(betas[1]), float(eps), float(weight_decay), int(step)))

    def op_ema_multi(self, shadows, ps, one_minus_decay):
        n = len(ps)
        numel = (C.c_longlong * n)(*[p.numel() for p in ps])
        self._check(lib.rdm_op_ema_multi(self._h, n, self._ptr_array(shadows), self._ptr_array(ps), numel, float(one_minus_decay)))

    def op_ema(self, shadow, p, one_minus_decay):
        self._check(lib.rdm_op_ema(self._h, _ptr(shadow), _ptr(p), p.numel(), float(one_minus_decay)))

    def op_silu(self, x, dy=None):
        out = torch.empty(x.shape, device=self.device, dtype=torch.bfloat16 if dy is None else torch.float32)
        self._check(lib.rdm_op_silu(self._h, _ptr(x), _ptr(dy) if dy is not None else None, _ptr(out), x.numel()))
        return out

    def op_q_sample(self, x0, noise, sqrt_ac, sqrt_1mac, want_nchw=True, cpad=0):
# ... 386 lines not shown
```

### retrieval-augmented-diffusion-models_amd/csrc/common.h

```cpp
#pragma once
#include <hip/hip_runtime.h>
#include <stdint.h>
#include <stdlib.h>

typedef uint16_t bf16_t;
typedef __attribute__((ext_vector_type(8))) short bf16x8;
typedef __attribute__((ext_vector_type(4))) short bf16x4;
typedef __attribute__((ext_vector_type(16))) float f32x16;
typedef __attribute__((ext_vector_type(4))) float f32x4;
typedef __attribute__((ext_vector_type(8))) _Float16 f16x8;

#define GLOBAL_AS __attribute__((address_space(1)))
#define LDS_AS __attribute__((address_space(3)))

__device__ __forceinline__ float bf2f(bf16_t v) { return __uint_as_float(((uint32_t)v) << 16); }
__device__ __forceinline__ bf16_t f2bf(float f) {
    uint32_t u = __float_as_uint(f);
    u += 0x7fffu + ((u >> 16) & 1u);
    return (bf16_t)(u >> 16);
}
__device__ __forceinline__ uint32_t pack2bf(float lo, float hi) {
    return (uint32_t)f2bf(lo) | ((uint32_t)f2bf(hi) << 16);
}
__device__ __forceinline__ uint32_t cvt_pk_bf16(float lo, float hi) {
    uint32_t r;
    asm("v_cvt_pk_bf16_f32 %0, %1, %2" : "=v"(r) : "v"(lo), "v"(hi));
    return r;
}
__device__ __forceinline__ float swap_adjacent_lane(float v) {
    return __builtin_bit_cast(float, __builtin_amdgcn_update_dpp(0, __builtin_bit_cast(int, v), 0xB1, 0xf, 0xf, true));
}
__device__ __forceinline__ float silu_f(float x) { return x * __builtin_amdgcn_rcpf(1.0f + __expf(-x)); }
__device__ __forceinline__ float gelu_erf_f(float x) {
    const float z = fabsf(x) * 0.70710678118654752f;
    const float t = __builtin_amdgcn_rcpf(1.0f + 0.3275911f * z);
    const float poly = t * (0.254829592f + t * (-0.284496736f + t * (1.421413741f + t * (-1.453152027f + t * 1.061405429f))));
    const float erf_abs = 1.0f - poly * __expf(-z * z);
    return 0.5f * x + 0.5f * fabsf(x) * erf_abs;
}
typedef float f32x2_t __attribute__((ext_vector_type(2)));
__device__ __forceinline__ f32x2_t gelu_erf_f2(f32x2_t x) {
    f32x2_t ax; ax.x = fabsf(x.x); ax.y = fabsf(x.y);
    const f32x2_t z = ax * 0.70710678118654752f;
    const f32x2_t d = z * 0.3275911f + 1.0f;
    f32x2_t t; t.x = __builtin_amdgcn_rcpf(d.x); t.y = __builtin_amdgcn_rcpf(d.y);
    const f32x2_t poly = t * (0.254829592f + t * (-0.284496736f + t * (1.421413741f + t * (-1.453152027f + t * 1.061405429f))));
    const f32x2_t a = (z * z) * -1.4426950408889634f;
    f32x2_t e; e.x = __builtin_amdgcn_exp2f(a.x); e.y = __builtin_amdgcn_exp2f(a.y);
    const f32x2_t erf_abs = 1.0f - poly * e;
    return (x + ax * erf_abs) * 0.5f;
}
__device__ __forceinline__ float quickgelu_f(float x) { return x * __builtin_amdgcn_rcpf(1.0f + __expf(-1.702f * x)); }

__device__ __forceinline__ void glds16(const void* gptr, void* lds_wave_base) {
    __builtin_amdgcn_global_load_lds((const GLOBAL_AS void*)gptr, (LDS_AS void*)lds_wave_base, 16, 0, 0);
}

enum { ACT_NONE = 0, ACT_GEGLU = 1, ACT_QUICKGELU = 2, ACT_SILU = 3, ACT_SOFTMAXG = 4 };

constexpr int RDM_EYE_OFFSET = 4096, RDM_EYE_N = 256;

constexpr int RDM_MAX_DEVICES = 32;
inline int rdm_cur_device() { int d = 0; (void)hipGetDevice(&d); return (d >= 0 && d < RDM_MAX_DEVICES) ? d : 0; }

inline int rdm_env_int(const char* value, int def) { return value ? atoi(value) : def; }

struct IgemmParams {
    const bf16_t* A0; const bf16_t* A1;
    int C0, C1;
    const bf16_t* W;
    int M, N, K;
    int Hin, Win, Hout, Wout, stride, ups;
    int phase2;
    int asym;
    float alpha;
    const float* bias;
    const float* rowvec;
    int rowvec_ld, rows_per_sample;
    const bf16_t* res_bf16;
    const float* res_f32;
    bf16_t* out_bf16; float* out_f32;
    int ldo;
    int act;
    int sm_group;
    long long sA, sW, sO;
    const void* zero_page;
    int ksplit; float* ws;
    int res_k;
    int lda, ldw;
    int l4_any_tiles;
    int res_wrap_rows;
    int a1_wrap_rows;
    const bf16_t* Wfrag;
    const float* ln_sb; float ln_inv_c, ln_eps;
    int dbg;
};
inline IgemmParams igemm_plain(int M, int N, int K, const void* zero_page) {
    IgemmParams p{}; p.M = M; p.N = N; p.K = K; p.alpha = 1.f; p.ldo = N; p.zero_page = zero_page;
    p.Hin = p.Win = p.Hout = p.Wout = 1; p.stride = 1; p.rows_per_sample = 1; return p;
}

struct Halo4Geom { int RS, NS, HPW, NROW, RSTR, NPR, NPT, HBYTES; };
__host__ __device__ inline Halo4Geom halo4_geom(int H, int W) {
    Halo4Geom g;
    const int HW = H * W;
    g.RS = (HW >= 256) ? 256 / W : H;
    g.NS = 256 / (g.RS * W);
    g.HPW = W + 2;
    g.NROW = g.NS * (g.RS + 2);
    g.RSTR = g.HPW * 144 + (W <= 16 ? 224 : 0);
    g.NPR = (g.HPW + 7) >> 3;
    g.NPT = g.NROW * g.NPR;
    g.HBYTES = (g.NROW * g.RSTR + 255) & ~255;
    return g;
}
constexpr int H4_HALO_MAX = 66560;
```

### retrieval-augmented-diffusion-models_amd/csrc/dispatch.hip

```cpp
#include "host.h"

static int gn_chunks(int HW) { const int n = HW / 64; return n < 1 ? 1 : n > 32 ? 32 : n; }

static bool skinny_rows(bool deterministic, bool single_row, int M, int single_max) {
    return deterministic ? single_row : (M <= 128 || (single_row && M <= single_max));
}
static int linear_kernel(SgemmParams& q, bool deterministic, bool single_row) {
    constexpr int SGEMM_MAX_ROWS = 4096;
    constexpr int SGEMM_GEGLU_MAX_ROWS = 192;
    if (skinny_rows(deterministic, single_row, q.M, q.act == ACT_GEGLU ? SGEMM_GEGLU_MAX_ROWS : SGEMM_MAX_ROWS)) {
        static const int mg_from = rdm_env_int(getenv("RDM_MGEMM_FROM"), 1536);
        if (!deterministic && single_row && mg_from > 0 && q.M >= mg_from && q.act != ACT_GEGLU && mgemm_supported(q)) return RDM_LINEAR_ROWS_MGEMM;
        q.fixed_split = deterministic ? 1 : 0;
        if (sgemm_supported(q)) return RDM_LINEAR_ROWS_SGEMM;
    }
    static const int mg_any = rdm_env_int(getenv("RDM_MGEMM_ANY"), 0);
    if (!single_row && mg_any > 0 && q.M >= mg_any && q.act != ACT_GEGLU && mgemm_supported(q)) return RDM_LINEAR_ROWS_MGEMM;
    return RDM_LINEAR_ROWS_TILED;
}
static bool linear_ln_takes(SgemmParams& q, bool deterministic, bool single_row) {
    constexpr int SGEMM_LN_MAX_ROWS = 192;
    if (!deterministic && q.M > SGEMM_LN_MAX_ROWS) return false;
    q.fixed_split = deterministic ? 1 : 0;
    return skinny_rows(deterministic, single_row, q.M, 1024) && sgemm_supported(q);
}

const bf16_t* Ops::derived(const bf16_t* W, int N, int K, int kind) {
    if (const_weights) return c->cached_derived(W, N, K, kind);
    if (ensure_bytes(c, &c->wfrag_tmp, &c->wfrag_tmp_bytes, rdm_ctx::derived_bytes(kind, N, K)) != 0) return nullptr;
    bf16_t* d = (bf16_t*)c->wfrag_tmp;
    return c->pack_derived(kind, W, d, N, K) == hipSuccess ? d : nullptr;
}

static SgemmParams skinny_params(const LinearOp& op) {
    SgemmParams q{}; q.A = op.A0; q.lda = op.C0; q.W = op.W; q.M = op.M; q.N = op.N; q.K = op.C0; q.bias = op.bias;
    q.act = op.act; q.res_f32 = op.res_f32; q.res_bf16 = op.res_bf16; q.out_f32 = op.out_f32; q.out_bf16 = op.out_bf16;
    q.ldo = op.act == ACT_GEGLU ? op.N / 2 : op.N;
    return q;
}
bool Ops::lin4_takes(const LinearOp& op) {
    if (c->deterministic) return false;
    IgemmParams t = base(op.M, op.N, op.C0 + op.C1);
    t.C0 = op.C0; t.C1 = op.C1; t.W = (const bf16_t*)blob; t.Wfrag = t.W; t.out_bf16 = (bf16_t*)blob; t.a1_wrap_rows = op.a1_wrap_rows;
    if (op.res_wrap_rows > 0) { t.res_bf16 = (const bf16_t*)blob; t.res_wrap_rows = op.res_wrap_rows; }
    return lin4_supported(t, 1);
}
void Ops::linear(const LinearOp& op) {
    if (plan) return;
    const int M = op.M, N = op.N, K = op.C0 + op.C1;
    if (!op.A1 && op.C1 == 0 && !op.rowvec && op.alpha == 1.f) {
        SgemmParams q = skinny_params(op);
        const int kernel = linear_kernel(q, c->deterministic, op.single_row);
        if (kernel != RDM_LINEAR_ROWS_TILED) {
            const bool mid = kernel == RDM_LINEAR_ROWS_MGEMM;
            prof_begin(RDM_PROF_LINEAR, 2.0 * M * N * (double)K, M, N, K);
            check(mid ? launch_mgemm(q, c->stream) : launch_sgemm(q, c->stream), mid ? "mid-size linear" : "skinny linear");
            prof_end();
            return;
        }
    }
    IgemmParams p = base(M, N, K);
    p.A0 = op.A0; p.A1 = op.A1; p.C0 = op.C0; p.C1 = op.C1; p.W = op.W; p.bias = op.bias; p.alpha = op.alpha;
    p.act = op.act; p.res_bf16 = op.res_bf16; p.res_f32 = op.res_f32; p.out_bf16 = op.out_bf16; p.out_f32 = op.out_f32;
    p.a1_wrap_rows = op.a1_wrap_rows; p.res_wrap_rows = op.res_wrap_rows;
    if (op.rowvec) { p.rowvec = op.rowvec; p.rowvec_ld = op.rowvec_ld; p.rows_per_sample = op.rows_per_sample; }
    if (op.act == ACT_GEGLU) p.ldo = N / 2;
    {
        IgemmParams t = p; t.Wfrag = p.W;
        const int tile_rows = (N % 384 == 0) ? 128 : 256;
        const bool det_ok = op.sample_rows > 0 && op.sample_rows % tile_rows == 0;
        if (c->deterministic) t.l4_any_tiles = p.l4_any_tiles = 1;
        if ((!c->deterministic || det_ok) && lin4_supported(t, 1)) p.Wfrag = derived(p.W, N, K, op.act == ACT_GEGLU ? 2 : 1);
    }
    prof_begin(RDM_PROF_LINEAR, 2.0 * M * N * (double)K, M, N, K);
    check(launch_igemm(p, false, 1, c->stream), "linear");
    prof_end();
}
bool Ops::linear_ln(const LinearOp& op) {
    SgemmParams q = skinny_params(op);
    q.ln_x = op.ln_x; q.ln_g = op.ln_g; q.ln_b = op.ln_b; q.ln_eps = 1e-5f;
    if (!linear_ln_takes(q, c->deterministic, op.single_row)) return false;
    if (plan) return true;
    prof_begin(RDM_PROF_LINEAR, 2.0 * op.M * op.N * (double)op.C0, op.M, op.N, op.C0);
    check(launch_sgemm(q, c->stream), "skinny linear on a LayerNorm");
    prof_end();
    return true;
}
void Ops::conv3(const Conv3Op& op) {
    if (plan) return;
    const bf16_t* A0 = op.A0; const bf16_t* A1 = op.A1; const bf16_t* W = op.W; const float* bias = op.bias;
    const int C0 = op.C0, C1 = op.C1, B = op.B, Hin = op.Hin, Win = op.Win, N = op.N, stride = op.stride, ups = op.ups;
    const float* rowvec = op.rowvec; const bf16_t* res = op.res_bf16; bf16_t* out = op.out_bf16;
    const int Hout = ups ? Hin * 2 : (stride == 2 ? Hin / 2 : Hin), Wout = ups ? Win * 2 : (stride == 2 ? Win / 2 : Win);
    IgemmParams p = base(B * Hout * Wout, N, 9 * (C0 + C1));
    p.asym = op.asym;
    p.A0 = A0; p.A1 = A1; p.C0 = C0; p.C1 = C1; p.W = W; p.bias = bias;
    p.Hin = Hin; p.Win = Win; p.Hout = Hout; p.Wout = Wout; p.stride = stride; p.ups = ups;
    p.rowvec = rowvec; p.rowvec_ld = op.rowvec_ld; p.rows_per_sample = Hout * Wout; p.res_bf16 = res; p.out_bf16 = out;
    if (ups && !A1 && C1 == 0 && C0 % 64 == 0 && N % 8 == 0 && !rowvec && !res && stride == 1) {
        const bf16_t* wp = derived(W, N, C0, 5);
        if (wp) {
            IgemmParams q = base(B * Hin * Win, N, 4 * C0);
            q.A0 = A0; q.C0 = C0; q.W = wp; q.bias = bias; q.out_bf16 = out; q.phase2 = 1;
            q.Hin = Hin; q.Win = Win; q.Hout = Hout; q.Wout = Wout; q.stride = 1; q.rows_per_sample = Hin * Win;
            q.sA = 0; q.sW = (long long)N * 4 * C0; q.sO = 0;
            prof_begin(RDM_PROF_UPSCONV, 2.0 * 4.0 * q.M * N * (double)q.K, 4 * q.M, N, q.K);
            check(launch_igemm(q, true, 4, c->stream), "conv3x3 on a 2x upsample, by phase");
            prof_end();
            return;
        }
    }
    const bool det_generic = c->deterministic && ((Hout * Wout) % 256 != 0);
    if (!det_generic && conv3x3_kernel(p) != CONV_IGEMM) p.Wfrag = derived(W, N, C0 + C1, 0);
    const int ks = (p.Wfrag && !c->deterministic) ? conv_halo_ksplit(p) : 1;
    if (ks > 1 && ensure_bytes(c, &c->splitk_ws, &c->splitk_ws_bytes, (size_t)ks * p.M * N * 4) == 0) { p.ksplit = ks; p.ws = (float*)c->splitk_ws; }
    prof_begin(RDM_PROF_CONV3X3, 2.0 * p.M * N * (double)p.K, p.M, N, p.K);
    check(launch_conv3x3(p, c->stream), "conv3x3");
    prof_end();
}
void Ops::tap(int stage, const void* ptr, size_t nbytes) {
    if (plan || !c->tap_buf || c->tap_block != cur_block || c->tap_sub != cur_layer * 16 + stage) return;
    if (nbytes > c->tap_bytes) nbytes = c->tap_bytes;
    check(hipMemcpyAsync(c->tap_buf, ptr, nbytes, hipMemcpyDeviceToDevice, c->stream), "debug tap");
}
void Ops::prof_begin(int kind, double work, int d0, int d1, int d2) {
    prof_open = (c->prof >> kind) & 1u;
    if (!prof_open) return;
    rdm_ctx::ProfRec r; r.a = c->prof_event(); r.b = c->prof_event(); r.kind = kind; r.flops = work; r.tag = tag; r.d0 = d0; r.d1 = d1; r.d2 = d2;
    hipEventRecord(r.a, c->stream); c->prof_recs.push_back(r);
}
void Ops::prof_end() { if (prof_open) hipEventRecord(c->prof_recs.back().b, c->stream); prof_open = false; }
void Ops::groupnorm(GnParams p) {
    if (plan) return;
    p.groups = 32; p.nchunk = gn_chunks(p.HW); p.partial = c->gn_partial;
    if (p.L0 <= 0) p.L0 = p.C0;
    if (p.L1 <= 0) p.L1 = p.C1;
    prof_begin(RDM_PROF_GROUPNORM, (double)p.B * p.HW * (p.C0 + p.C1) * 4.0, p.B * p.HW, p.C0 + p.C1, p.silu);
    check(launch_groupnorm(p, c->stream), "groupnorm");
    prof_end();
}
HeadParams Ops::head_params(HeadParams hp) const {
    hp.groups = 32;
    if (hp.gamma) { hp.partial = c->gn_partial; hp.nchunk = gn_chunks(hp.H * hp.W); }
    return hp;
}
void Ops::head(HeadParams hp, int Clog, bf16_t* tmp) {
    if (plan) return;
    hp = head_params(hp);
    const int B = hp.B, H = hp.H, W = hp.W, C = hp.C;
    if ((Clog <= 0 || Clog == C) && head_conv_supported(hp)) {
        if (hp.gamma) {
            GnParams p{}; p.x0 = hp.x; p.C0 = C; p.HW = H * W; p.B = B; p.groups = 32; p.L0 = C; p.nchunk = hp.nchunk; p.partial = c->gn_partial;
            prof_begin(RDM_PROF_GROUPNORM, (double)B * H * W * C * 2.0, B * H * W, C, 2);
            check(launch_gn_stats(p, c->stream), "head groupnorm statistics");
            prof_end();
        }
        check(launch_head_conv(hp, c->stream), "head conv");
        return;
    }
    groupnorm({.x0 = hp.x, .C0 = C, .HW = H * W, .B = B, .L0 = Clog, .gamma = hp.gamma, .beta = hp.beta, .eps = hp.eps, .silu = 1, .out = tmp});
    check(launch_conv_out(tmp, hp.w, hp.bias, hp.out, B, H, W, C, hp.Cout, c->stream), "conv_out");
}
void Ops::vq_nearest(const VqNearestOp& op) {
    if (plan) return;
    check(launch_vq_nearest(op.z, op.codebook, op.norms, op.M, op.N, op.E, op.ws, op.idx32, op.idx64, c->stream), "vq nearest code");
}
void Ops::layernorm(const LayerNormOp& op) {
    if (plan) return;
    const bool in_f32 = op.x_f32 != nullptr, out_f32 = op.out_f32 != nullptr;
    prof_begin(RDM_PROF_LAYERNORM, (double)op.M * op.C * ((in_f32 ? 4.0 : 2.0) + (out_f32 ? 4.0 : 2.0)), op.M, op.C, 0);
    check(launch_layernorm(in_f32 ? (const void*)op.x_f32 : op.x_bf16, in_f32, op.gamma, op.beta, out_f32 ? (void*)op.out_f32 : op.out_bf16, out_f32,
                           op.M, op.C, op.eps, c->stream, op.Clog < 0 ? op.C : op.Clog), "layernorm");
    prof_end();
}
void Ops::flash_d32(FlashParams f, int heads, int B) {
    if (plan) return;
    const int C = heads * 32, n = f.n;
    f.k = f.q + C; f.ldk = f.ldq; f.ldv = f.v ? f.ldq : 0; f.ldo = C; f.C = C;
    f.scale_log2e = (1.0f / sqrtf(32.f)) * 1.4426950408889634f;
    prof_begin(RDM_PROF_ATTENTION, 4.0 * B * heads * (double)n * n * 32, B, n, C);
    check(launch_flash_d32(f, heads, B, c->stream), "flash attention");
    prof_end();
}
void Ops::causal_d64(CausalD64Params f, int heads, int B, float scale) {
    if (plan) return;
    const int n = f.n;
    f.C = heads * 64; f.scale_log2e = scale * 1.4426950408889634f;
    prof_begin(RDM_PROF_ATTENTION, 2.0 * B * heads * (double)n * n * 64, B, n, f.C);
    check(launch_causal_d64(f, heads, B, c->stream), "causal attention");
    prof_end();
}
void Ops::vq_attention(const VqAttnParams& f, int B) {
    if (plan) return;
    prof_begin(RDM_PROF_ATTENTION, 6.0 * B * (double)f.n * f.n * f.C, B, f.n, f.C);
    check(launch_vq_attn_stream(f, B, c->stream), "vq attention");
    prof_end();
}
void Ops::small_attention(const SmallAttnParams& p, int D, int heads, int B, const char* what) {
    if (plan) return;
    check(launch_small_attention(p, D, heads, B, c->stream), what);
}
void Ops::xattn_fused(const XattnParams& q) {
    if (plan) return;
    prof_begin(RDM_PROF_LINEAR, 4.0 * q.rows * q.NP * (double)q.C, q.rows, q.NP, q.C);
    check(launch_xattn_fused(q, c->stream), "fused cross attention");
    prof_end();
}

int rdm_linear_rows_select(int M, int N, int K, int act, int ln, int deterministic, rdm_linear_rows_form* out) {
    if (!out || M < 1 || N < 1 || K < 1 || act < ACT_NONE || act > ACT_SILU) return -1;
    *out = rdm_linear_rows_form{};
    static const float some = 0.f;
    SgemmParams q{}; q.M = M; q.N = N; q.K = K; q.lda = K; q.act = act; q.ldo = act == ACT_GEGLU ? N / 2 : N;
    if (ln) { q.ln_x = &some; q.ln_g = &some; q.ln_b = &some; q.ln_eps = 1e-5f; }
    out->kernel = ln ? (linear_ln_takes(q, deterministic != 0, true) ? RDM_LINEAR_ROWS_SGEMM : RDM_LINEAR_ROWS_REFUSED) : linear_kernel(q, deterministic != 0, true);
    if (out->kernel == RDM_LINEAR_ROWS_SGEMM) {
        const SgemmForm f = sgemm_form(q);
        if (!sgemm_form_compiled(f)) return -3;
        out->ma = f.ma; out->nb = f.nb; out->u = f.u; out->nw = f.nw; out->ln = f.ln; out->geglu = f.geglu;
    }
    return 0;
}
```

### retrieval-augmented-diffusion-models_amd/csrc/host.h

```cpp
#pragma once
#include <stdarg.h>
#include <stdio.h>
#include <stdlib.h>
#include <string.h>

#include <cmath>
#include <string>
#include <unordered_map>
#include <vector>

#include "../../include/rdm_hip.h"
#include "kernels.h"
#include "knn.h"

#define RDM_CHECK_HIP(ctx, expr)                                                            \
    do {                                                                                    \
        hipError_t _e = (expr);                                                             \
        if (_e != hipSuccess) return (ctx)->fail(-2, "%s failed: %s (%s:%d)", #expr, hipGetErrorString(_e), __FILE__, __LINE__); \
    } while (0)
#define RDM_TRY(expr)            \
    do {                         \
        int _r = (expr);         \
        if (_r != 0) return _r;  \
    } while (0)
// ... 17 lines not shown
        const size_t off = total;
        text += std::to_string(off) + " " + std::to_string(nbytes) + " " + kind + " "; text += srcs; text += "\n";
        total += nbytes;
        return off;
    }
    size_t f32(const std::string& n, size_t numel) { return add("f32", n, numel * 4); }
    size_t bf16(const std::string& n, size_t numel) { return add("bf16", n, numel * 2); }
    size_t conv3(const std::string& n, size_t cout, size_t cin) { return add("conv3", n, cout * cin * 9 * 2); }
};

struct Arena {
    char* base = nullptr; size_t cap = 0, off = 0, peak = 0; bool planning = false;
    void reset() { off = 0; }
    void* alloc(size_t bytes) {
        off = (off + 255) & ~(size_t)255;
        void* p = base ? base + off : (void*)(uintptr_t)(off + 256);
        off += bytes;
        if (off > peak) peak = off;
        return p;
    }
};

template <typename T> static void free_dev(T*& p, size_t& bytes) { if (p) (void)hipFree(p); p = nullptr; bytes = 0; }
struct ModelBase {
    char* blob = nullptr; size_t blob_bytes = 0; Arena arena; bool loaded = false;
    void release() { free_dev(blob, blob_bytes); free_dev(arena.base, arena.cap); loaded = false; }
};

inline int pad64(int c) { return (c + 63) & ~63; }
struct ResW { int cin, cout; size_t gn1g, gn1b, w1, b1, gn2g, gn2b, w2, b2, wsk, bsk; int emb_off; bool skip; int l0, l1, lout, p0, p1; };
constexpr int XA_NP = 128;

struct StW {
    int c, heads; size_t gng, gnb, win, bin, ln1g, ln1b, wqk, wv, wo1, bo1, ln2g, ln2b, wq2, wo2, bo2, ln3g, ln3b, wff1,
        bff1, wff2, bff2, wout, bout, wfo, bfo; int kv_off; long long xa_unit;
    int lc;
    bool v_follows;
};
struct ConvW { int c; size_t w, b; int lc; };
struct ULayer { int kind; int idx; };
struct UBlock { int where; std::vector<ULayer> layers; };

struct UNet : ModelBase {
    rdm_unet_cfg cfg{};
    std::vector<UBlock> blocks; std::vector<ResW> res; std::vector<StW> st; std::vector<ConvW> down, up;
    size_t te0w, te0b, te2w, te2b, embw, embb, kvw, cinw, cinb, outg, outb, outw, outbias;
    int emb_total = 0, kv_total = 0; long long xa_total = 0;
    bf16_t* xa_cache = nullptr; size_t xa_cache_bytes = 0;
    bf16_t* kv_cache = nullptr; size_t kv_cache_bytes = 0;
    float* emb_table = nullptr; size_t emb_table_bytes = 0;
    int ctx_rows = 0;
    void release() { free_dev(xa_cache, xa_cache_bytes); free_dev(kv_cache, kv_cache_bytes); free_dev(emb_table, emb_table_bytes); ModelBase::release(); }
};

struct VqRes { int cin, cout; size_t n1g, n1b, w1, b1, n2g, n2b, w2, b2, wsk, bsk; bool skip; };
struct VqAttn { int c; size_t ng, nb, wq, bq, wk, bk, wv, bv, wo, bo; };
struct VqLevel {
    std::vector<VqRes> blocks;
    std::vector<VqAttn> attn;
    ConvW resample{};
};
struct VqMid { VqRes res1, res2; VqAttn attn; bool has_attn; };

struct VqModel : ModelBase {
    rdm_vq_cfg cfg{};
    bool wide = false;
    size_t codebook, pqw, pqb, cinw, cinb, noutg, noutb, coutw, coutb;
    VqMid mid;
    std::vector<VqLevel> levels;
    float* code_norms = nullptr;
    void release() { if (code_norms) (void)hipFree(code_norms); code_norms = nullptr; ModelBase::release(); }
};

struct VqEncModel : ModelBase {
    rdm_vq_cfg cfg{};
    bool wide = false;
    size_t cinw, cinb, noutg, noutb, coutw, coutb, qw, qb;
    std::vector<VqLevel> levels;
    VqMid mid;
};

struct ClipBlk { size_t ln1g, ln1b, wqkv, bqkv, wo, bo, ln2g, ln2b, wfc, bfc, wpj, bpj; };
struct ClipModel : ModelBase {
    rdm_clip_cfg cfg{};
    std::vector<ClipBlk> text, vis;
    size_t tok, pos, lnfg, lnfb, tproj;
    size_t conv1, cls, vpos, lnpreg, lnpreb, lnpostg, lnpostb, vproj;
};

struct RarmBlk { size_t ln1g, ln1b, wqkv, wo1, bo1, ln2g, ln2b, wq2, wo2, bo2, ln3g, ln3b, wff1, bff1, wff2, bff2; };
struct RarmModel : ModelBase {
    rdm_rarm_cfg cfg{}; int C = 0, kv_total = 0;
    std::vector<RarmBlk> blk;
    size_t emb, pos, kvw, wpo, bpo;
    char* cache = nullptr; size_t cache_bytes = 0;
    char* ctxkv = nullptr; size_t ctxkv_bytes = 0;
    char* state = nullptr; size_t state_bytes = 0;
    char* xa = nullptr; size_t xa_bytes = 0; int xa_B = 0, xa_k = 0;
    void release() { free_dev(cache, cache_bytes); free_dev(ctxkv, ctxkv_bytes); free_dev(state, state_bytes); free_dev(xa, xa_bytes); xa_B = xa_k = 0; ModelBase::release(); }
};

struct rdm_ctx {
    int device = 0; hipStream_t stream = nullptr; char err[512] = {0};
    void* zero_page = nullptr; float* eye3 = nullptr;
    UNet unet; VqModel vq; VqEncModel vqenc; ClipModel clip; RarmModel rarm; KnnDb db;
    float* gn_partial = nullptr; size_t gn_partial_bytes = 0;
    char* splitk_ws = nullptr; size_t splitk_ws_bytes = 0;
    char* samp = nullptr; size_t samp_bytes = 0;
    struct FragKey {
        const void* W; int N, K, kind; const void* aux;
        bool operator==(const FragKey& o) const { return W == o.W && N == o.N && K == o.K && kind == o.kind && aux == o.aux; }
    };
    struct FragKeyHash {
        size_t operator()(const FragKey& k) const {
            size_t h = std::hash<const void*>()(k.W);
            for (size_t v : {(size_t)k.N, (size_t)k.K, (size_t)k.kind, (size_t)(uintptr_t)k.aux}) h = (h ^ v) * 0x9E3779B97F4A7C15ull + (h >> 29);
            return h;
        }
    };
    struct FragVal { bf16_t* frag; float* sb; };
    std::unordered_map<FragKey, FragVal, FragKeyHash> wfrag;
    char* bwd_tmp = nullptr; size_t bwd_tmp_bytes = 0;
    char* wfrag_tmp = nullptr; size_t wfrag_tmp_bytes = 0;
    void drop_frags() { for (auto& kv : wfrag) { (void)hipFree(kv.second.frag); if (kv.second.sb) (void)hipFree(kv.second.sb); } wfrag.clear(); }
    static size_t derived_bytes(int kind, int N, int K) { return (size_t)N * K * 2 * (kind == 0 ? 9 : kind == 5 ? 16 : 1); }
    hipError_t pack_derived(int kind, const bf16_t* W, bf16_t* d, int N, int K) {
        return kind == 0 ? launch_conv_w_fragpack(W, d, N, K, stream)
             : kind == 5 ? launch_conv_phase_weights(W, d, N, K, stream)
                         : launch_lin_w_fragpack(W, d, N, K, K, kind == 2, stream);
    }
    const bf16_t* cached_derived(const bf16_t* W, int N, int K, int kind) {
        const FragKey key{W, N, K, kind, nullptr};
        auto it = wfrag.find(key);
        if (it != wfrag.end()) return it->second.frag;
        bf16_t* d = nullptr;
        if (hipMalloc((void**)&d, derived_bytes(kind, N, K)) != hipSuccess) return nullptr;
        if (pack_derived(kind, W, d, N, K) != hipSuccess) { (void)hipFree(d); return nullptr; }
        wfrag[key] = FragVal{d, nullptr};
        return d;
    }
    const float* zero_bias_pair(const float* b, int C) {
        const FragKey key{b, C, 2, 6, nullptr};
        auto it = wfrag.find(key);
        if (it != wfrag.end()) return it->second.sb;
        float* t = nullptr;
        if (hipMalloc((void**)&t, (size_t)2 * C * sizeof(float)) != hipSuccess) return nullptr;
        if (hipMemsetAsync(t, 0, (size_t)C * sizeof(float), stream) != hipSuccess ||
            hipMemcpyAsync(t + C, b, (size_t)C * sizeof(float), hipMemcpyDeviceToDevice, stream) != hipSuccess) { (void)hipFree(t); return nullptr; }
        wfrag[key] = FragVal{nullptr, t};
        return t;
    }
    bool deterministic = rdm_env_int(getenv("RDM_DETERMINISTIC"), 0) != 0;
    void* tap_buf = nullptr; size_t tap_bytes = 0; int tap_block = -1, tap_sub = 0;
    void* rccl_lib = nullptr; void* comm = nullptr; int comm_world = 0;
    unsigned prof = 0;
    struct ProfRec { hipEvent_t a, b; int kind; double flops; const char* tag; int d0, d1, d2; };
    std::vector<ProfRec> prof_recs; std::vector<hipEvent_t> prof_pool;
    hipEvent_t prof_event() {
        if (!prof_pool.empty()) { hipEvent_t e = prof_pool.back(); prof_pool.pop_back(); return e; }
        hipEvent_t e; hipEventCreate(&e); return e;
    }
    int fail(int code, const char* fmt, ...) {
        va_list ap; va_start(ap, fmt); vsnprintf(err, sizeof err, fmt, ap); va_end(ap); return code;
    }
};

inline int ensure_bytes(rdm_ctx* c, char** p, size_t* have, size_t need) {
    if (*have >= need) return 0;
    if (*p) { RDM_CHECK_HIP(c, hipStreamSynchronize(c->stream)); RDM_CHECK_HIP(c, hipFree(*p)); *p = nullptr; *have = 0; }
    RDM_CHECK_HIP(c, hipMalloc((void**)p, need));
    *have = need; return 0;
}

inline int ensure_gn_partial(rdm_ctx* c, int B) {
    const size_t need = (size_t)B * 32 * 64 * 2 * sizeof(float);
    return ensure_bytes(c, (char**)&c->gn_partial, &c->gn_partial_bytes, need);
}


struct LinearOp {
    const bf16_t* A0 = nullptr; const bf16_t* A1 = nullptr; int C0 = 0, C1 = 0;
    const float* ln_x = nullptr; const float* ln_g = nullptr; const float* ln_b = nullptr;
    const bf16_t* W = nullptr; const float* bias = nullptr;
    int M = 0, N = 0;
    int act = ACT_NONE;
    const bf16_t* res_bf16 = nullptr; const float* res_f32 = nullptr;
    bf16_t* out_bf16 = nullptr; float* out_f32 = nullptr;
    const float* rowvec = nullptr; int rowvec_ld = 0, rows_per_sample = 1;
    int a1_wrap_rows = 0, res_wrap_rows = 0;
    float alpha = 1.f;
    bool single_row = false;
    int sample_rows = 0;
};
struct Conv3Op {
    const bf16_t* A0 = nullptr; const bf16_t* A1 = nullptr; int C0 = 0, C1 = 0;
    const bf16_t* W = nullptr; const float* bias = nullptr;
    int B = 0, Hin = 0, Win = 0, N = 0, stride = 1, ups = 0;
    const bf16_t* res_bf16 = nullptr; bf16_t* out_bf16 = nullptr;
    const float* rowvec = nullptr; int rowvec_ld = 0;
    int asym = 0;
};
struct LayerNormOp {
    const float* x_f32 = nullptr; const bf16_t* x_bf16 = nullptr;
    const float* gamma = nullptr; const float* beta = nullptr;
    int M = 0, C = 0;
    float* out_f32 = nullptr; bf16_t* out_bf16 = nullptr;
    int Clog = -1;
    float eps = 1e-5f;
};
struct VqNearestOp {
    const float* z = nullptr; const float* codebook = nullptr; const float* norms = nullptr;
    long long M = 0; int N = 0, E = 0;
    char* ws = nullptr; int* idx32 = nullptr; long long* idx64 = nullptr;
};

struct Ops {
    rdm_ctx* c; Arena* ar; const char* blob; bool plan; int rc = 0;
    template <typename T> const T* w(size_t off) const { return (const T*)(blob + off); }
    bf16_t* abf(size_t n) { return (bf16_t*)ar->alloc(n * 2); }
    float* af32(size_t n) { return (float*)ar->alloc(n * 4); }
    void check(hipError_t e, const char* what) {
        if (e != hipSuccess && rc == 0) rc = c->fail(-3, "%s: %s", what, hipGetErrorString(e));
    }
    IgemmParams base(int M, int N, int K) const { return igemm_plain(M, N, K, c->zero_page); }
    bool const_weights = true;
    const bf16_t* derived(const bf16_t* W, int N, int K, int kind);
    bool lin4_takes(const LinearOp& op);
    void linear(const LinearOp& op);
    bool linear_ln(const LinearOp& op);
    void conv3(const Conv3Op& op);
    int cur_block = -1, cur_layer = 0;
    void tap(int stage, const void* ptr, size_t nbytes);
    bool prof_open = false;
    const char* tag = "";
    void prof_begin(int kind, double work, int d0 = 0, int d1 = 0, int d2 = 0);
    void prof_end();
    void groupnorm(GnParams p);
    HeadParams head_params(HeadParams hp) const;
    void head(HeadParams hp, int Clog = 0, bf16_t* tmp = nullptr);
    void vq_nearest(const VqNearestOp& op);
    void layernorm(const LayerNormOp& op);
    void flash_d32(FlashParams f, int heads, int B);
    void causal_d64(CausalD64Params f, int heads, int B, float scale);
    void vq_attention(const VqAttnParams& f, int B);
    void small_attention(const SmallAttnParams& p, int D, int heads, int B, const char* what);
    void xattn_fused(const XattnParams& q);
};

template <typename F>
static int run_with_arena(rdm_ctx* c, Arena& ar, const char* blob, F&& body) {
    Ops plan{c, &ar, blob, true};
    char* keep = ar.base; ar.base = nullptr; ar.reset(); ar.peak = 0;
    body(plan);
    const size_t need = ar.peak + 4096;
    ar.base = keep;
    RDM_TRY(ensure_bytes(c, &ar.base, &ar.cap, need));
    ar.reset();
    Ops run{c, &ar, blob, false};
    body(run);
    return run.rc;
}

int unet_prepare_kv(rdm_ctx* c, float* cat, const float* cond, const float* uncond, int B, int k);
int unet_emb_table(rdm_ctx* c, const std::vector<int>& ts, const float** table);
int unet_forward_impl(rdm_ctx* c, const float* x, const int64_t* t, const float* context, const bf16_t* kv_cached,
                      int b, int k, int H, int W, float* eps_out, int ctx_rows = -1, int shared_half = 0, const float* emb_row = nullptr);
```

### retrieval-augmented-diffusion-models_amd/csrc/igemm.hip

```cpp

#include <type_traits>

#include "kernels.h"

__device__ __forceinline__ void softmax_group16(float (&v)[16], int g) {
#pragma unroll
    for (int r = 0; r < 16; r++) {
        float mx = v[r];
        if (g >= 2) mx = fmaxf(mx, __shfl_xor(mx, 1));
        if (g >= 4) mx = fmaxf(mx, __shfl_xor(mx, 2));
        const float e = __expf(v[r] - mx);
        float sum = e;
        if (g >= 2) sum += __shfl_xor(sum, 1);
        if (g >= 4) sum += __shfl_xor(sum, 2);
        v[r] = e / sum;
    }
}

template <int BM, int BN, int WAVES_M, int CONV, bool GEGLU>
__global__ __launch_bounds__(WAVES_M * 128, 2) void igemm_kernel(IgemmParams p) {
    constexpr int BK = 64;
    constexpr int WAVES_N = 2, NW = WAVES_M * WAVES_N, NT = NW * 64;
    constexpr int WM = BM / WAVES_M, WN = BN / WAVES_N;
    constexpr int FM = WM / 32, FN = WN / 32;
// ... 361 lines not shown
            const bool plain = simple && (GEGLU || p.act == ACT_NONE);
            bool done = false;
            if constexpr (BN == 128 && CONV == 0 && !GEGLU) {
                if (simple && p.act == ACT_SOFTMAXG) { lds_epilogue(std::integral_constant<int, 2>{}); done = true; }
            }
            if (!done) { if (plain) lds_epilogue(std::integral_constant<int, 1>{}); else lds_epilogue(std::integral_constant<int, 0>{}); }
        } else {
#pragma unroll
            for (int i = 0; i < FM; i++) {
                const int mf = em0 + wm * WM + i * 32;
                constexpr bool BATCH_RES = !GEGLU && (CONV == 0 || BN == 128);
                uint32_t rw[2][8];
                auto load_res = [&](int j0) {
                    if constexpr (BATCH_RES) {
                        if (rb) {
#pragma unroll
                            for (int jj = 0; jj < 2; jj++) {
                                const int j = j0 + jj;
                                if (j >= FN) continue;
                                const int pc = en0 + wn * WN + j * 32 + frow - odd;
                                const long long rbase = (long long)(mf + 4 * fhalf + odd) * p.ldo + pc;
                                const bool pok = full || (pc + 1 < p.N);
#pragma unroll
                                for (int t = 0; t < 8; t++) {
                                    const int roff = ((2 * t) & 3) + 8 * ((2 * t) >> 2);
                                    rw[jj][t] = 0;
                                    if (full || (pok && mf + 4 * fhalf + odd + roff < p.M)) rw[jj][t] = *(const uint32_t*)(rb + rbase + (long long)roff * p.ldo);
                                }
                            }
                        }
                    }
                };
#pragma unroll
                for (int j = 0; j < FN; j++) {
                    if constexpr (GEGLU) { if (j & 1) continue; }
                    if ((j & 1) == 0) load_res(j);
                    const int ncol = en0 + wn * WN + j * 32 + frow;
                    const bool col_ok = full || ncol < p.N;
                    const int ocol = GEGLU ? ((en0 + wn * WN + j * 32) >> 1) + frow : ncol;
                    const float bias = pbias[i][j];
                    float gbias = 0.f;
                    if constexpr (GEGLU) gbias = pbias[i][(j + 1) < FN ? (j + 1) : j];
                    float v[16];
#pragma unroll
                    for (int r = 0; r < 16; r++) {
                        float x = acc[i][j][r] * p.alpha + bias;
                        if (p.rowvec && !uniform_sample) {
                            const int m = mf + (r & 3) + 8 * (r >> 2) + 4 * fhalf;
                            if (col_ok && m < p.M) x += p.rowvec[(long long)(m / p.rows_per_sample) * p.rowvec_ld + ncol];
                        }
                        if constexpr (GEGLU) {
                            const float g = acc[i][(j + 1) < FN ? (j + 1) : j][r] * p.alpha + gbias;
                            x = x * gelu_erf_f(g);
                        } else {
                            if (p.act == ACT_QUICKGELU) x = quickgelu_f(x);
                            else if (p.act == ACT_SILU) x = silu_f(x);
                        }
                        v[r] = x;
                    }
                    const int mrow = mf + 4 * fhalf + odd;
                    const int pcol = ocol - odd;
                    const bool pair_ok = full || (pcol + 1 < (GEGLU ? p.N / 2 : p.N));
                    const long long base = (long long)mrow * p.ldo + pcol;
#pragma unroll
                    for (int t = 0; t < 8; t++) {
                        const int roff = ((2 * t) & 3) + 8 * ((2 * t) >> 2);
                        const float give = odd ? v[2 * t] : v[2 * t + 1];
                        const float got = swap_adjacent_lane(give);
                        float lo = odd ? got : v[2 * t];
                        float hi = odd ? v[2 * t + 1] : got;
                        if (full || (pair_ok && mrow + roff < p.M)) {
                            long long o = base + (long long)roff * p.ldo;
                            if constexpr (BATCH_RES) { if (rb) { const uint32_t u = rw[j & 1][t]; lo += __uint_as_float(u << 16); hi += __uint_as_float(u & 0xffff0000u); } }
                            else { if (rb) { const uint32_t u = *(const uint32_t*)(rb + o); lo += __uint_as_float(u << 16); hi += __uint_as_float(u & 0xffff0000u); } }
                            if (rf) { const float2 f = *(const float2*)(rf + o); lo += f.x; hi += f.y; }
                            if (ob) *(uint32_t*)(ob + o) = cvt_pk_bf16(lo, hi);
                            if (of) *(float2*)(of + o) = make_float2(lo, hi);
                        }
                    }
                }
            }
        }
        if (!has_next) break;
        tile = next;
        {
            constexpr int NFRAG = GEGLU ? FM * FN / 2 : FM * FN;
            const int nout = (ob ? 1 : 0) + (of ? 1 : 0);
            if (lds_epi) pending_stores = full ? FM * ((32 * (WNO / 8)) / 64) : 0;
            else pending_stores = (full && nout == 1) ? NFRAG * 8 : 0;
            if (pending_stores == 0) asm volatile("s_waitcnt vmcnt(0)" ::: "memory");
        }
    }
}

template <int BM, int BN, int WAVES_M, int CONV, bool GEGLU>
static hipError_t launch_cfg(const IgemmParams& p, int batch, hipStream_t st) {
    constexpr int smem = ((BM >= 256 ? 3 : 2) * BM + 2 * BN) * 128;
    constexpr int NT = WAVES_M * 128;
    static int bpc_dev[RDM_MAX_DEVICES] = {0}, ncu_dev[RDM_MAX_DEVICES] = {0};
    const int dev = rdm_cur_device();
    if (!bpc_dev[dev]) {
        hipError_t e = hipFuncSetAttribute((const void*)igemm_kernel<BM, BN, WAVES_M, CONV, GEGLU>,
                                           hipFuncAttributeMaxDynamicSharedMemorySize, smem);
        if (e != hipSuccess) return e;
        hipDeviceGetAttribute(&ncu_dev[dev], hipDeviceAttributeMultiprocessorCount, dev);
        int occ = 0;
        e = hipOccupancyMaxActiveBlocksPerMultiprocessor(&occ, (const void*)igemm_kernel<BM, BN, WAVES_M, CONV, GEGLU>, NT, smem);
        if (e != hipSuccess) return e;
        bpc_dev[dev] = occ < 1 ? 1 : occ;
    }
    const int blocks_per_cu = bpc_dev[dev], ncu = ncu_dev[dev];
    const int nbm = (p.M + BM - 1) / BM, nbn = (p.N + BN - 1) / BN;
    const long long ntiles = (long long)nbm * nbn;
    long long g = (long long)ncu * blocks_per_cu;
    if (batch > 1) g = (g + batch - 1) / batch;
    g = (g + 7) & ~7LL;
    if (g > ntiles) g = ntiles;
    if (g < 1) g = 1;
    dim3 grid((unsigned)g, 1, batch);
    igemm_kernel<BM, BN, WAVES_M, CONV, GEGLU><<<grid, NT, smem, st>>>(p);
    return hipGetLastError();
}

__global__ __launch_bounds__(256) void conv_phase_weights_kernel(const bf16_t* __restrict__ W, bf16_t* __restrict__ Wp, int N, int C) {
    const long long total = (long long)4 * N * 4 * C;
    for (long long i = (long long)blockIdx.x * 256 + threadIdx.x; i < total; i += (long long)gridDim.x * 256) {
        const int c = (int)(i % C); long long r = i / C;
        const int tx = (int)(r & 1), ty = (int)((r >> 1) & 1); r >>= 2;
        const int n = (int)(r % N), ph = (int)(r / N), a = ph >> 1, b = ph & 1;
        const int ky0 = a == 0 ? (ty == 0 ? 0 : 1) : (ty == 0 ? 0 : 2), ky1 = a == 0 ? (ty == 0 ? 0 : 2) : (ty == 0 ? 1 : 2);
        const int kx0 = b == 0 ? (tx == 0 ? 0 : 1) : (tx == 0 ? 0 : 2), kx1 = b == 0 ? (tx == 0 ? 0 : 2) : (tx == 0 ? 1 : 2);
        float s = 0.f;
        for (int ky = ky0; ky <= ky1; ky++)
            for (int kx = kx0; kx <= kx1; kx++) s += bf2f(W[((long long)n * 9 + ky * 3 + kx) * C + c]);
        Wp[i] = f2bf(s);
    }
}
hipError_t launch_conv_phase_weights(const bf16_t* W, bf16_t* Wp, int N, int C, hipStream_t st) {
    long long g = ((long long)16 * N * C + 255) / 256; if (g > 8192) g = 8192;
    conv_phase_weights_kernel<<<dim3((unsigned)g), 256, 0, st>>>(W, Wp, N, C);
    return hipGetLastError();
}

hipError_t launch_igemm(const IgemmParams& p_in, bool conv, int batch, hipStream_t st) {
    IgemmParams p = p_in;
    p.res_k = 0;
    if (p.K % 64 != 0 || p.C0 % 64 != 0 || p.C1 % 64 != 0) return hipErrorInvalidValue;
    if (p.N % 2 != 0 || p.ldo % 2 != 0 || p.sO % 2 != 0) return hipErrorInvalidValue;
    if (p.act == ACT_GEGLU && (p.N % 64 != 0)) return hipErrorInvalidValue;
    if (p.act == ACT_SOFTMAXG && (conv || p.N % 192 == 0 || p.alpha != 1.0f || !p.out_bf16 || p.out_f32 || p.res_f32 || p.ldo % 8 ||
                                  !(p.sm_group == 1 || p.sm_group == 2 || p.sm_group == 4)))
        return hipErrorInvalidValue;
    const bool wide = (p.N % 192 == 0);
    const long long tiles256 = (long long)((p.M + 255) / 256) * ((p.N + (wide ? 191 : 127)) / (wide ? 192 : 128)) * batch;
    const bool tall = tiles256 >= 256 && p.M > 128;
    if (!conv && p.Wfrag && lin4_supported(p, batch)) return launch_lin4(p, st);
    if (p.a1_wrap_rows > 0 || p.res_wrap_rows > 0) return hipErrorInvalidValue;
    if (p.act == ACT_GEGLU) {
        if (conv) return hipErrorInvalidValue;
        if (tall && p.N % 256 == 0 && (long long)((p.M + 255) / 256) * (p.N / 256) * batch >= 256)
            return launch_cfg<256, 256, 4, 0, true>(p, batch, st);
        return tall ? launch_cfg<256, 128, 4, 0, true>(p, batch, st) : launch_cfg<128, 128, 2, 0, true>(p, batch, st);
    }
    if (conv && p.phase2) {
        if (batch != 4 || !p.out_bf16 || p.out_f32 || p.res_bf16 || p.res_f32 || p.rowvec || p.act != ACT_NONE || p.alpha != 1.0f || p.ldo % 8 || p.N % 8 ||
            p.C1 != 0 || p.K != 4 * p.C0 || p.M != (long long)(p.M / (p.Hin * p.Win)) * p.Hin * p.Win || p.Hout != 2 * p.Hin || p.Wout != 2 * p.Win)
            return hipErrorInvalidValue;
        if (wide) return tall ? launch_cfg<256, 192, 4, 3, false>(p, batch, st) : launch_cfg<128, 192, 2, 3, false>(p, batch, st);
        return tall ? launch_cfg<256, 128, 4, 3, false>(p, batch, st) : launch_cfg<128, 128, 2, 3, false>(p, batch, st);
    }
    if (conv && p.ups) {
        if (wide) return tall ? launch_cfg<256, 192, 4, 2, false>(p, batch, st) : launch_cfg<128, 192, 2, 2, false>(p, batch, st);
        return tall ? launch_cfg<256, 128, 4, 2, false>(p, batch, st) : launch_cfg<128, 128, 2, 2, false>(p, batch, st);
    }
    if (conv) {
        if (wide) return tall ? launch_cfg<256, 192, 4, 1, false>(p, batch, st) : launch_cfg<128, 192, 2, 1, false>(p, batch, st);
        return tall ? launch_cfg<256, 128, 4, 1, false>(p, batch, st) : launch_cfg<128, 128, 2, 1, false>(p, batch, st);
    }
    if (p.res_bf16 && !p.res_f32 && p.out_bf16 && !p.out_f32 && p.alpha == 1.0f && p.act == ACT_NONE &&
        p.N % (wide ? 192 : 128) == 0 && p.ldo % 8 == 0 && p.ldo >= p.N)
        p.res_k = 1;
    if (wide) return tall ? launch_cfg<256, 192, 4, 0, false>(p, batch, st) : launch_cfg<128, 192, 2, 0, false>(p, batch, st);
    return tall ? launch_cfg<256, 128, 4, 0, false>(p, batch, st) : launch_cfg<128, 128, 2, 0, false>(p, batch, st);
}
```

### retrieval-augmented-diffusion-models_amd/csrc/lin4.hip

```cpp

#include <type_traits>

#include "kernels.h"
#include "h4_asm.h"

__host__ __device__ inline int l4_geglu_row(int n) {
    const int nb = n >> 5, fr = n & 31;
    return 64 * (nb >> 1) + 16 * (nb & 1) + (fr < 16 ? fr : 32 + (fr - 16));
}
__global__ __launch_bounds__(256) void lin_w_fragpack_kernel(const bf16_t* __restrict__ W, bf16_t* __restrict__ dst, int N, int K, int ldw, int geglu,
                                                             const float* __restrict__ gamma) {
    const int KQ = K >> 4;
    const long long nvec = (long long)N * K / 8;
    for (long long v = (long long)blockIdx.x * 256 + threadIdx.x; v < nvec; v += (long long)gridDim.x * 256) {
        const int lane = (int)(v & 63);
        const long long f = v >> 6;
        const int kq = (int)(f % KQ), nb = (int)(f / KQ);
        int n = nb * 32 + (lane & 31);
        const int c = kq * 16 + (lane >> 5) * 8;
        if (geglu) n = l4_geglu_row(n);
        uint4 w = *(const uint4*)(W + (long long)n * ldw + c);
        if (gamma) {
            uint32_t* u = (uint32_t*)&w;
#pragma unroll
            for (int e = 0; e < 4; e++)
                u[e] = pack2bf(gamma[c + 2 * e] * __uint_as_float(u[e] << 16), gamma[c + 2 * e + 1] * __uint_as_float(u[e] & 0xffff0000u));
        }
        *(uint4*)(dst + v * 8) = w;
    }
}
hipError_t launch_lin_w_fragpack(const bf16_t* W, bf16_t* dst, int N, int K, int ldw, int geglu, hipStream_t st, const float* gamma) {
    const long long nvec = (long long)N * K / 8;
    long long g = (nvec + 255) / 256; if (g > 8192) g = 8192;
    lin_w_fragpack_kernel<<<dim3((unsigned)g), 256, 0, st>>>(W, dst, N, K, ldw > 0 ? ldw : K, geglu, gamma);
    return hipGetLastError();
}
__global__ __launch_bounds__(256) void lin_ln_sb_kernel(const bf16_t* __restrict__ W, const float* __restrict__ gamma, const float* __restrict__ beta,
                                                        const float* __restrict__ bias, float* __restrict__ sb, int N, int K) {
    const int lane = threadIdx.x & 63, n = blockIdx.x * 4 + (threadIdx.x >> 6);
    if (n >= N) return;
    float s = 0.f, b = 0.f;
    for (int k = lane; k < K; k += 64) {
        const float w = bf2f(W[(long long)n * K + k]);
        s += bf2f(f2bf(gamma[k] * w));
        b += beta[k] * w;
    }
#pragma unroll
    for (int o = 32; o > 0; o >>= 1) { s += __shfl_xor(s, o); b += __shfl_xor(b, o); }
    if (lane == 0) { sb[2 * n] = s; sb[2 * n + 1] = b + (bias ? bias[n] : 0.f); }
}
hipError_t launch_lin_ln_sb(const bf16_t* W, const float* gamma, const float* beta, const float* bias, float* sb, int N, int K, hipStream_t st) {
    lin_ln_sb_kernel<<<dim3((unsigned)((N + 3) / 4)), 256, 0, st>>>(W, gamma, beta, bias, sb, N, K);
    return hipGetLastError();
}


struct ASrc { const char* base; unsigned pstride; unsigned voff; };
__device__ __forceinline__ unsigned long long l4_uni64(unsigned long long v) {
    const unsigned lo = __builtin_amdgcn_readfirstlane((unsigned)v), hi = __builtin_amdgcn_readfirstlane((unsigned)(v >> 32));
    return ((unsigned long long)hi << 32) | lo;
}
__device__ __forceinline__ ASrc l4_asrc(bool dead, int row0, int kc, int C0, const char* A0p, const char* A1p, unsigned ld0, unsigned ld1,
                                        const char* zero, unsigned voffA0, unsigned voffA1, unsigned lane16, int wrap1) {
    ASrc s;
    const bool second = kc >= C0;
    const unsigned ld = second ? ld1 : ld0;
    if (second && row0 >= wrap1) row0 -= wrap1;
    const char* b = (second ? A1p : A0p) + (unsigned long long)row0 * ld + (unsigned)((second ? kc - C0 : kc) * 2);
    s.base = (const char*)l4_uni64((unsigned long long)(dead ? zero : b));
    s.pstride = (unsigned)__builtin_amdgcn_readfirstlane((int)(dead ? 0u : 32u * ld));
    s.voff = dead ? lane16 : (second ? voffA1 : voffA0);
    return s;
}

template <bool GEGLU, int WM, bool LN>
__global__ __launch_bounds__(256, 1) void lin4_kernel(IgemmParams p) {
    constexpr int BM = 128 * WM, BK = 64, FM = 4, FN = 3, WN = FN * 32, BN = (4 / WM) * WN;
    constexpr int L4_ABUF = BM * 144;
    constexpr int NPC = 4 * WM;
    extern __shared__ __attribute__((aligned(16))) char smem[];

    const int tid = threadIdx.x, lane = tid & 63;
    const int wave = __builtin_amdgcn_readfirstlane(tid >> 6);
    const int wm = WM == 2 ? wave >> 1 : 0, wn = WM == 2 ? wave & 1 : wave;
    const int frow = lane & 31, fhalf = lane >> 5;
    const int lp = lane >> 3, lc = lane & 7;

    const int K = p.K, nslice = K / BK, KQ = K >> 4;
    const int nbn = p.N / BN, nbm = p.M / BM;
    const int ntiles = nbm * nbn;
    const int G = gridDim.x, xcd = blockIdx.x & 7;
    const int gx = (G - xcd + 7) >> 3;
    const int tq = ntiles >> 3, tr = ntiles & 7;
    const int t_begin = xcd < tr ? xcd * (tq + 1) : tr * (tq + 1) + (xcd - tr) * tq;
    const int t_end = t_begin + tq + (xcd < tr ? 1 : 0);
    const int tile0 = t_begin + (blockIdx.x >> 3);
    if (tile0 >= t_end) return;
    const int gxq = gx / nbn, gxr = gx - gxq * nbn;

    const char* const A0p = (const char*)p.A0; const char* const A1p = (const char*)p.A1;
    const int C0 = p.C0;
    const float* const biasp = p.bias;
    const int ldo = p.ldo;
    const char* const zero = (const char*)p.zero_page;
    const char* const Wf = (const char*)p.Wfrag;
    const unsigned ld0 = (unsigned)(p.lda > 0 ? p.lda : p.C0) * 2u, ld1 = (unsigned)p.C1 * 2u;
    const int wrap1 = p.a1_wrap_rows > 0 ? p.a1_wrap_rows : 0x7fffffff;

    unsigned vbase[FM];
#pragma unroll
    for (int i = 0; i < FM; i++) vbase[i] = (unsigned)((wm * 128 + i * 32 + frow) * 144 + fhalf * 16);
    unsigned voffj[FN];
#pragma unroll
    for (int j = 0; j < FN; j++) voffj[j] = (unsigned)(lane * 16) + (unsigned)j * (unsigned)(KQ * 1024);
    const unsigned voffA0 = (unsigned)(wave * 8 + lp) * ld0 + (unsigned)(lc * 16);
    const unsigned voffA1 = (unsigned)(wave * 8 + lp) * ld1 + (unsigned)(lc * 16);
    const unsigned lane16 = (unsigned)(lane * 16);
    const unsigned ldsw0 = (unsigned)((wave * 8 + lp) * 144 + lc * 16);
    const unsigned ldsw1 = ldsw0 + (unsigned)L4_ABUF;

    bf16_t* const ob = p.out_bf16;
    const bf16_t* const rb = p.res_bf16;

    struct Cur { int tile, bm, bn, sl; };
    auto cur_adv = [&](Cur& c) __attribute__((always_inline)) {
        c.sl++;
        if (c.sl == nslice) { c.sl = 0; c.tile += gx; c.bn += gxr; c.bm += gxq; if (c.bn >= nbn) { c.bn -= nbn; c.bm++; } }
    };
    auto w_base = [&](const Cur& c) __attribute__((always_inline)) -> const char* {
        const int nb0 = c.bn * (BN / 32) + wn * FN;
        const long long off = ((long long)nb0 * KQ + c.sl * 4) * 1024;
        return (const char*)l4_uni64((unsigned long long)(Wf + off));
    };
    auto a_src = [&](const Cur& c) __attribute__((always_inline)) {
        return l4_asrc(c.tile >= t_end, c.bm * BM, c.sl * BK, C0, A0p, A1p, ld0, ld1, zero, voffA0, voffA1, lane16, wrap1);
    };

    asm volatile("" ::: H4_ACC_CLOBBERS);
    bf16x8 fa[2][FM];
    bf16x8 fb[2][4][FN];
    h4_u32x4 hreg[2][NPC];
    float lsum[NPC], lsq[NPC];
#pragma unroll
    for (int q = 0; q < NPC; q++) { lsum[q] = 0.f; lsq[q] = 0.f; }
    const unsigned ones_bf = (unsigned)__builtin_amdgcn_readfirstlane(0x3f803f80);
    auto stat_half = [&](int q, const h4_u32x4& h, int half) __attribute__((always_inline)) {
        if constexpr (LN) {
            if (half == 0)
                asm volatile("v_dot2_f32_bf16 %0, %2, %4, %0\n\tv_dot2_f32_bf16 %1, %2, %2, %1\n\tv_dot2_f32_bf16 %0, %3, %4, %0\n\tv_dot2_f32_bf16 %1, %3, %3, %1"
                             : "+v"(lsum[q]), "+v"(lsq[q]) : "v"(h.x), "v"(h.y), "s"(ones_bf));
            else
                asm volatile("v_dot2_f32_bf16 %0, %2, %4, %0\n\tv_dot2_f32_bf16 %1, %2, %2, %1\n\tv_dot2_f32_bf16 %0, %3, %4, %0\n\tv_dot2_f32_bf16 %1, %3, %3, %1"
                             : "+v"(lsum[q]), "+v"(lsq[q]) : "v"(h.z), "v"(h.w), "s"(ones_bf));
        }
    };

    Cur cc{tile0, tile0 / nbn, tile0 % nbn, 0};
    Cur cb = cc, ca = cc;

    constexpr int L4_STG = 2 * L4_ABUF;
    constexpr int L4_BIAS = L4_STG + 4 * 32 * 400;
    const int L4_STAT = L4_BIAS + p.N * 8;
    const int L4_RV = L4_BIAS + p.N * 4;
    const bool has_rv = !LN && p.rowvec != nullptr;
    const int rv_split = has_rv ? p.rows_per_sample : 0x7fffffff;
    if constexpr (LN) {
        for (int n = tid; n < p.N; n += 256)
            *(float2*)(smem + L4_BIAS + n * 8) = *(const float2*)(p.ln_sb + 2 * (GEGLU ? l4_geglu_row(n) : n));
    } else {
        for (int n = tid; n < p.N; n += 256) {
            const float bv = biasp ? biasp[GEGLU ? l4_geglu_row(n) : n] : 0.f;
            const uint32_t hi = cvt_pk_bf16(bv, 0.f) & 0xffffu;
            const uint32_t lo = cvt_pk_bf16(bv - __uint_as_float(hi << 16), 0.f) & 0xffffu;
            *(uint32_t*)(smem + L4_BIAS + n * 4) = hi | (lo << 16);
        }
        if (has_rv) {
            for (int i = tid; i < 2 * p.N; i += 256) {
                const int g = i >= p.N ? 1 : 0, n = i - g * p.N;
                const float bv = ((long long)g * p.rows_per_sample < p.M) ? p.rowvec[(long long)g * p.rowvec_ld + (GEGLU ? l4_geglu_row(n) : n)] : 0.f;
                const uint32_t hi = cvt_pk_bf16(bv, 0.f) & 0xffffu;
                const uint32_t lo = cvt_pk_bf16(bv - __uint_as_float(hi << 16), 0.f) & 0xffffu;
                *(uint32_t*)(smem + L4_RV + i * 4) = hi | (lo << 16);
            }
        }
    }
    __syncthreads();
    typedef __attribute__((ext_vector_type(4))) unsigned u32x4_t;
    union FragU { u32x4_t u; bf16x8 f; };
    auto bias_frags = [&](int bn, int bm, int row, int half, bf16x8 (&bf)[FN], bf16x8& ones) __attribute__((always_inline)) {
        const int rvoff = L4_RV + ((bm * BM >= rv_split) ? p.N * 4 : 0);
#pragma unroll
        for (int j = 0; j < FN; j++) {
            uint32_t w = 0u, w2 = 0u;
            if constexpr (!LN) {
                w = *(const uint32_t*)(smem + L4_BIAS + (bn * BN + wn * WN + j * 32 + row) * 4);
                if (has_rv) w2 = *(const uint32_t*)(smem + rvoff + (bn * BN + wn * WN + j * 32 + row) * 4);
            }
            FragU t; t.u = (u32x4_t){half ? 0u : w, half ? 0u : w2, 0u, 0u};
            bf[j] = t.f;
        }
        FragU o; o.u = (u32x4_t){half ? 0u : 0x3f803f80u, half ? 0u : 0x3f803f80u, 0u, 0u};
        ones = o.f;
    };
    auto acc_init = [&](int bn, int bm) __attribute__((always_inline)) {
        bf16x8 bf[FN], ones;
        bias_frags(bn, bm, frow, fhalf, bf, ones);
        asm volatile("s_nop 7" : "+v"(bf[0]), "+v"(bf[1]), "+v"(bf[2]), "+v"(ones));
#pragma unroll
        for (int i = 0; i < FM; i++)
#pragma unroll
            for (int j = 0; j < FN; j++) H4_MFMA0(i * FN + j, bf[j], ones);
    };

    {
        ASrc s0 = a_src(ca); cur_adv(ca);
#pragma unroll
        for (int q = 0; q < NPC; q++) H4_GLOADB(hreg[0][q], s0.voff, s0.base + (unsigned)q * s0.pstride, 0);
        asm volatile("s_waitcnt vmcnt(0)" ::: "memory");
#pragma unroll
        for (int q = 0; q < NPC; q++) { H4_LDSWO(ldsw0, hreg[0][q], q * 4608); stat_half(q, hreg[0][q], 0); stat_half(q, hreg[0][q], 1); }
        ASrc s1 = a_src(ca); cur_adv(ca);
#pragma unroll
        for (int q = 0; q < NPC; q++) H4_GLOADB(hreg[0][q], s1.voff, s1.base + (unsigned)q * s1.pstride, 0);
        const char* sb = w_base(cb); cur_adv(cb);
#pragma unroll
        for (int ks = 0; ks < 4; ks++)
#pragma unroll
            for (int j = 0; j < FN; j++) { H4_GLOADB(fb[0][ks][j], voffj[j], sb, ks * 1024); fb[1][ks][j] = fb[0][ks][j]; }
        ASrc s2 = a_src(ca); cur_adv(ca);
#pragma unroll
        for (int q = 0; q < NPC; q++) H4_GLOADB(hreg[1][q], s2.voff, s2.base + (unsigned)q * s2.pstride, 0);
        asm volatile("s_waitcnt lgkmcnt(0)" ::: "memory");
        __builtin_amdgcn_s_barrier();
#pragma unroll
        for (int i = 0; i < FM; i++) { H4_LDSR(fa[0][i], vbase[i], 0); fa[1][i] = fa[0][i]; }
    }
    acc_init(cc.bn, cc.bm);

    int epi_stores = 0;
    const char* sbn = Wf; ASrc an{zero, 0u, lane16};
    auto describe = [&]() __attribute__((always_inline)) {
        sbn = (const char*)l4_uni64((unsigned long long)((cb.tile < t_end) ? w_base(cb) : Wf));
        cur_adv(cb);
        an = a_src(ca);
        cur_adv(ca);
    };
    auto step = [&](auto ptag) __attribute__((always_inline)) {
        constexpr int P = decltype(ptag)::value;
        constexpr int RB = P * L4_ABUF;
        auto mfma = [&](int ks, int m) {
            const int j = m / FM, i = m % FM;
            H4_MFMA(i * FN + j, fb[P][ks][j], fa[ks & 1][i]);
        };
        if (epi_stores == 0) asm volatile("s_waitcnt vmcnt(%0) lgkmcnt(0)" :: "i"(NPC) : "memory");
        else asm volatile("s_waitcnt vmcnt(%0) lgkmcnt(0)" :: "i"(NPC + (GEGLU ? FM * FN : 2 * FM * FN)) : "memory");
        epi_stores = 0;
#pragma unroll
        for (int m = 0; m < FM * FN; m++) {
            mfma(0, m);
            H4_GLOADB(fb[P ^ 1][m / FN][m % FN], voffj[m % FN], sbn, (m / FN) * 1024);
            if (m == 3) {
#pragma unroll
                for (int i = 0; i < FM; i++) H4_LDSR(fa[1][i], vbase[i], RB + 32);
            }
        }
#pragma unroll
        for (int ks = 1; ks < 4; ks++) {
            const int q0 = NPC == 8 ? (ks - 1) * 3 : (ks == 1 ? 0 : ks), nq = NPC == 8 ? (ks < 3 ? 3 : 2) : (ks == 1 ? 2 : 1);
            asm volatile("s_waitcnt lgkmcnt(0)" ::: "memory");
#pragma unroll
            for (int q = q0; q < q0 + nq; q++) {
                if (P == 0) H4_LDSWO(ldsw1, hreg[P][q], q * 4608); else H4_LDSWO(ldsw0, hreg[P][q], q * 4608);
            }
            auto stat_at = [&](int m) __attribute__((always_inline)) { if (m < 2 * nq) stat_half(q0 + (m >> 1), hreg[P][q0 + (m >> 1)], m & 1); };
            mfma(ks, 0); stat_at(0); mfma(ks, 1); stat_at(1); mfma(ks, 2); stat_at(2); mfma(ks, 3); stat_at(3);
            if (ks < 3) {
#pragma unroll
                for (int i = 0; i < FM; i++) H4_LDSR(fa[(ks + 1) & 1][i], vbase[i], RB + (ks + 1) * 32);
            } else {
                asm volatile("s_waitcnt lgkmcnt(0)" ::: "memory");
                __builtin_amdgcn_s_barrier();
#pragma unroll
                for (int i = 0; i < FM; i++) H4_LDSR(fa[0][i], vbase[i], (P ^ 1) * L4_ABUF);
            }
            mfma(ks, 4); stat_at(4); mfma(ks, 5); stat_at(5);
#pragma unroll
            for (int q = q0; q < q0 + nq; q++) {
                H4_GLOADB(hreg[P][q], an.voff, an.base + (unsigned)q * an.pstride, 0);
// ... 58 lines not shown
            asm volatile("s_waitcnt lgkmcnt(0)" ::: "memory");
#pragma unroll
            for (int j = 0; j < FN; j++) H4_MFMA0(i * FN + j, nbf[j], nones);
        };
        if constexpr (GEGLU) {
            const int eno_o = (en0 >> 1) + wn * (WN / 2);
            unsigned voffs[3], lrd[3], sbo[3], srow[3];
#pragma unroll
            for (int it = 0; it < 3; it++) {
                const int idx = it * 64 + lane_e, row = idx / 6, c6 = idx - row * 6;
                voffs[it] = (unsigned)(row * ldo + c6 * 8) * 2u;
                lrd[it] = (unsigned)(row * 400 + ((c6 >> 1) * 32 + (c6 & 1) * 8) * 4);
                sbo[it] = (unsigned)(L4_BIAS + (en0 + wn * WN + (c6 >> 1) * 32 + (c6 & 1) * 8) * 8);
                srow[it] = (unsigned)(L4_STAT + (wm * 128 + row) * 8);
            }
            const char* const obase = (const char*)(ob + (long long)(em0 + wm * 128) * ldo + eno_o);
            const unsigned long long rowstep = (unsigned long long)(32 * ldo) * 2ull;
            auto store_row = [&](int i) __attribute__((always_inline)) {
                const char* const op = (const char*)l4_uni64((unsigned long long)(obase + i * rowstep));
#pragma unroll
                for (int it = 0; it < 3; it++) {
                    float4 x0 = *(const float4*)(stgr + lrd[it]), x1 = *(const float4*)(stgr + lrd[it] + 16);
                    float4 g0 = *(const float4*)(stgr + lrd[it] + 64), g1 = *(const float4*)(stgr + lrd[it] + 80);
                    if constexpr (LN) {
                        const float2 st = *(const float2*)(smem + srow[it] + i * 256);
                        const float r = st.y, m2 = -st.x * st.y;
                        const float4* const qx = (const float4*)(smem + sbo[it]); const float4* const qg = (const float4*)(smem + sbo[it] + 128);
                        const float4 a = qx[0], b = qx[1], c = qx[2], d = qx[3];
                        x0.x = fmaf(r, x0.x, fmaf(m2, a.x, a.y)); x0.y = fmaf(r, x0.y, fmaf(m2, a.z, a.w));
                        x0.z = fmaf(r, x0.z, fmaf(m2, b.x, b.y)); x0.w = fmaf(r, x0.w, fmaf(m2, b.z, b.w));
                        x1.x = fmaf(r, x1.x, fmaf(m2, c.x, c.y)); x1.y = fmaf(r, x1.y, fmaf(m2, c.z, c.w));
                        x1.z = fmaf(r, x1.z, fmaf(m2, d.x, d.y)); x1.w = fmaf(r, x1.w, fmaf(m2, d.z, d.w));
                        const float4 e = qg[0], f = qg[1], g = qg[2], h = qg[3];
                        g0.x = fmaf(r, g0.x, fmaf(m2, e.x, e.y)); g0.y = fmaf(r, g0.y, fmaf(m2, e.z, e.w));
                        g0.z = fmaf(r, g0.z, fmaf(m2, f.x, f.y)); g0.w = fmaf(r, g0.w, fmaf(m2, f.z, f.w));
                        g1.x = fmaf(r, g1.x, fmaf(m2, g.x, g.y)); g1.y = fmaf(r, g1.y, fmaf(m2, g.z, g.w));
                        g1.z = fmaf(r, g1.z, fmaf(m2, h.x, h.y)); g1.w = fmaf(r, g1.w, fmaf(m2, h.z, h.w));
                    }
                    const f32x2_t r0 = (f32x2_t){x0.x, x0.y} * gelu_erf_f2((f32x2_t){g0.x, g0.y});
                    const f32x2_t r1 = (f32x2_t){x0.z, x0.w} * gelu_erf_f2((f32x2_t){g0.z, g0.w});
                    const f32x2_t r2 = (f32x2_t){x1.x, x1.y} * gelu_erf_f2((f32x2_t){g1.x, g1.y});
                    const f32x2_t r3 = (f32x2_t){x1.z, x1.w} * gelu_erf_f2((f32x2_t){g1.z, g1.w});
                    const h4_u32x4 dv = {cvt_pk_bf16(r0.x, r0.y), cvt_pk_bf16(r1.x, r1.y), cvt_pk_bf16(r2.x, r2.y), cvt_pk_bf16(r3.x, r3.y)};
                    H4_GSTORES_NT(voffs[it], dv, op);
                }
            };
            stage_row(0); store_row(0);
            stage_row(1); store_row(1);
            stage_row(2); store_row(2);
            stage_row(3); store_row(3);
        } else {
            const int eno = en0 + wn * WN;
            unsigned voffs[6], lrd[6], sbo[3], srow[3];
#pragma unroll
            for (int it = 0; it < 6; it++) {
                const int idx = it * 64 + lane_e, row = idx / 12, ch = idx - row * 12;
                voffs[it] = (unsigned)(row * ldo + ch * 8) * 2u;
                lrd[it] = (unsigned)(row * 400 + ch * 32);
                if (it < 3) { sbo[it] = (unsigned)(L4_BIAS + (en0 + wn * WN + ch * 8) * 8); srow[it] = (unsigned)(L4_STAT + (wm * 128 + row) * 8); }
            }
            const char* const obase = (const char*)(ob + (long long)(em0 + wm * 128) * ldo + eno);
            const int er0 = (p.res_wrap_rows > 0 && em0 >= p.res_wrap_rows) ? em0 - p.res_wrap_rows : em0;
            const char* const rbase = (const char*)(rb + (long long)(er0 + wm * 128) * ldo + eno);
            const unsigned long long rowstep = (unsigned long long)(32 * ldo) * 2ull;
            h4_u32x4 rr4[2][6];
            auto res_request = [&](int i, h4_u32x4 (&dst)[6]) __attribute__((always_inline)) {
                const char* const rp = (const char*)l4_uni64((unsigned long long)(rbase + i * rowstep));
#pragma unroll
                for (int it = 0; it < 6; it++) H4_GLOADB(dst[it], voffs[it], rp, 0);
            };
            auto store_row = [&](int i) __attribute__((always_inline)) {
                const char* const op = (const char*)l4_uni64((unsigned long long)(obase + i * rowstep));
#pragma unroll
                for (int it = 0; it < 6; it++) {
                    float4 a0 = *(const float4*)(stgr + lrd[it]), a1 = *(const float4*)(stgr + lrd[it] + 16);
                    if constexpr (LN) {
                        const float2 st = *(const float2*)(smem + srow[it % 3] + i * 256 + (it / 3) * 128);
                        const float r = st.y, m2 = -st.x * st.y;
                        const float4* const qs = (const float4*)(smem + sbo[it % 3]);
                        const float4 a = qs[0], b = qs[1], c = qs[2], d = qs[3];
                        a0.x = fmaf(r, a0.x, fmaf(m2, a.x, a.y)); a0.y = fmaf(r, a0.y, fmaf(m2, a.z, a.w));
                        a0.z = fmaf(r, a0.z, fmaf(m2, b.x, b.y)); a0.w = fmaf(r, a0.w, fmaf(m2, b.z, b.w));
                        a1.x = fmaf(r, a1.x, fmaf(m2, c.x, c.y)); a1.y = fmaf(r, a1.y, fmaf(m2, c.z, c.w));
                        a1.z = fmaf(r, a1.z, fmaf(m2, d.x, d.y)); a1.w = fmaf(r, a1.w, fmaf(m2, d.z, d.w));
                    }
                    if (!LN && rb) {
                        const h4_u32x4 r4 = rr4[i & 1][it];
                        a0.x += __uint_as_float(r4.x << 16); a0.y += __uint_as_float(r4.x & 0xffff0000u);
                        a0.z += __uint_as_float(r4.y << 16); a0.w += __uint_as_float(r4.y & 0xffff0000u);
                        a1.x += __uint_as_float(r4.z << 16); a1.y += __uint_as_float(r4.z & 0xffff0000u);
                        a1.z += __uint_as_float(r4.w << 16); a1.w += __uint_as_float(r4.w & 0xffff0000u);
                    }
                    const h4_u32x4 dv = {cvt_pk_bf16(a0.x, a0.y), cvt_pk_bf16(a0.z, a0.w), cvt_pk_bf16(a1.x, a1.y), cvt_pk_bf16(a1.z, a1.w)};
                    H4_GSTORES(voffs[it], dv, op);
                }
            };
            constexpr int NST = 6;
            if (!LN && rb) {
                res_request(0, rr4[0]); res_request(1, rr4[1]);
                stage_row(0);
                asm volatile("s_waitcnt vmcnt(6)" : "+v"(rr4[0][0]), "+v"(rr4[0][1]), "+v"(rr4[0][2]), "+v"(rr4[0][3]), "+v"(rr4[0][4]), "+v"(rr4[0][5]) :: "memory");
                store_row(0);
                res_request(2, rr4[0]);
                stage_row(1);
                asm volatile("s_waitcnt vmcnt(%6)" : "+v"(rr4[1][0]), "+v"(rr4[1][1]), "+v"(rr4[1][2]), "+v"(rr4[1][3]), "+v"(rr4[1][4]), "+v"(rr4[1][5]) : "i"(6 + NST) : "memory");
                store_row(1);
                res_request(3, rr4[1]);
                stage_row(2);
                asm volatile("s_waitcnt vmcnt(%6)" : "+v"(rr4[0][0]), "+v"(rr4[0][1]), "+v"(rr4[0][2]), "+v"(rr4[0][3]), "+v"(rr4[0][4]), "+v"(rr4[0][5]) : "i"(6 + NST) : "memory");
                store_row(2);
                stage_row(3);
                asm volatile("s_waitcnt vmcnt(%6)" : "+v"(rr4[1][0]), "+v"(rr4[1][1]), "+v"(rr4[1][2]), "+v"(rr4[1][3]), "+v"(rr4[1][4]), "+v"(rr4[1][5]) : "i"(NST) : "memory");
                store_row(3);
            } else {
                stage_row(0); store_row(0);
                stage_row(1); store_row(1);
                stage_row(2); store_row(2);
                stage_row(3); store_row(3);
            }
        }
        epi_stores = GEGLU ? FM * FN : 2 * FM * FN;
        if (!has_next) return true;
        cc = nx;
        return false;
    };
    while (true) {
        describe(); step(std::integral_constant<int, 0>{}); if (advance()) break;
        describe(); step(std::integral_constant<int, 1>{}); if (advance()) break;
    }
}

static int lin4_wm(const IgemmParams& p) {
    if (p.N % 384 == 0 && p.M % 128 == 0) return 1;
    if (p.N % 192 == 0 && p.M % 256 == 0) return 2;
    return 0;
}
static int lin4_smem_bytes(const IgemmParams& p, int wm) {
    return 2 * (128 * wm * 144) + 4 * 32 * 400 + (p.ln_sb ? p.N * 8 + 128 * wm * 8 : p.N * 4 + (p.rowvec ? 2 * p.N * 4 : 0));
}
bool lin4_supported(const IgemmParams& p, int batch) {
    if (!p.Wfrag || batch != 1) return false;
    const int wm = lin4_wm(p);
    if (!wm || p.K % 64 || p.C0 % 64 || p.C1 % 64 || p.K != p.C0 + p.C1) return false;
    if (p.alpha != 1.0f || p.res_f32 || p.out_f32 || !p.out_bf16) return false;
    if (p.rowvec && (p.ln_sb || p.rows_per_sample <= 0 || p.rows_per_sample % (128 * wm) != 0 || 2LL * p.rows_per_sample < p.M || p.rowvec_ld < p.N)) return false;
    const bool geglu = p.act == ACT_GEGLU;
    if (p.act != ACT_NONE && !geglu) return false;
    if (geglu && p.res_bf16) return false;
    const int No = geglu ? p.N / 2 : p.N;
    if (p.N > 8192 || p.ldo % 8 || p.ldo < No || (p.ldw > 0 && p.ldw != p.K)) return false;
    if (p.C1 > 0 && p.lda > 0) return false;
    if (p.res_wrap_rows > 0 && (!p.res_bf16 || p.res_wrap_rows % (128 * wm) != 0 || 2LL * p.res_wrap_rows < p.M)) return false;
    if (p.a1_wrap_rows > 0 && (p.C1 == 0 || p.a1_wrap_rows % (128 * wm) != 0 || 2LL * p.a1_wrap_rows < p.M)) return false;
    if (p.ln_sb && (p.C1 > 0 || p.K < 128 || p.res_bf16 || p.bias || lin4_smem_bytes(p, wm) > 160 * 1024 || !(p.ln_inv_c > 0.f))) return false;
    constexpr int L4_MIN_TILES = 128;
    if (!p.l4_any_tiles && (long long)(p.M / (128 * wm)) * (p.N / (wm == 1 ? 384 : 192)) < L4_MIN_TILES) return false;
    return true;
}

template <bool GEGLU, int WM, bool LN>
static hipError_t launch_lin4_cfg(const IgemmParams& p, hipStream_t st) {
    const int smem = lin4_smem_bytes(p, WM);
    static int ncu_dev[RDM_MAX_DEVICES] = {0};
    const int dev = rdm_cur_device();
    if (!ncu_dev[dev]) {
        hipError_t e = hipFuncSetAttribute((const void*)lin4_kernel<GEGLU, WM, LN>, hipFuncAttributeMaxDynamicSharedMemorySize, 160 * 1024);
        if (e != hipSuccess) return e;
        hipDeviceGetAttribute(&ncu_dev[dev], hipDeviceAttributeMultiprocessorCount, dev);
    }
    const long long ntiles = (long long)(p.M / (128 * WM)) * (p.N / (WM == 1 ? 384 : 192));
    long long g = (ncu_dev[dev] + 7) & ~7;
    if (g > ntiles) g = ntiles;
    lin4_kernel<GEGLU, WM, LN><<<dim3((unsigned)g), 256, smem, st>>>(p);
    return hipGetLastError();
}
hipError_t launch_lin4(const IgemmParams& p, hipStream_t st) {
    const int wm = lin4_wm(p);
    if (p.ln_sb) {
        if (p.act == ACT_GEGLU) return wm == 1 ? launch_lin4_cfg<true, 1, true>(p, st) : launch_lin4_cfg<true, 2, true>(p, st);
        return wm == 1 ? launch_lin4_cfg<false, 1, true>(p, st) : launch_lin4_cfg<false, 2, true>(p, st);
    }
    if (p.act == ACT_GEGLU) return wm == 1 ? launch_lin4_cfg<true, 1, false>(p, st) : launch_lin4_cfg<true, 2, false>(p, st);
    return wm == 1 ? launch_lin4_cfg<false, 1, false>(p, st) : launch_lin4_cfg<false, 2, false>(p, st);
}
```

### retrieval-augmented-diffusion-models_amd/csrc/unet_exec.hip

```cpp
#include "host.h"

static void unet_compute_kv(Ops& o, UNet& u, const float* context, int B, int k, bf16_t* kv_out) {
    const int cd = u.cfg.context_dim;
    bf16_t* cb = o.abf((size_t)B * k * cd);
    if (!o.plan) o.check(launch_cast_f32_bf16(context, cb, (long long)B * k * cd, o.c->stream), "cast ctx");
    o.linear({.A0 = cb, .C0 = cd, .W = o.w<bf16_t>(u.kvw), .M = B * k, .N = u.kv_total, .out_bf16 = kv_out});
}

static bool xattn_skinny_ok(const UNet& u, int k) {
    if (!(k == 1 || k == 2 || k == 4)) return false;
    for (const StW& s : u.st) if (s.heads * k > XA_NP || s.c != s.heads * 32) return false;
    return !u.st.empty();
}
static void unet_compute_xattn(Ops& o, UNet& u, const bf16_t* kv, int B, int k, bf16_t* xa) {
    int cmax = 0;
    for (const StW& s : u.st) cmax = s.c > cmax ? s.c : cmax;
    bf16_t* kexp = o.abf((size_t)B * XA_NP * cmax);
    bf16_t* vexp = o.abf((size_t)B * XA_NP * cmax);
    bf16_t* wqt = o.abf((size_t)cmax * cmax);
    if (o.plan) return;
    for (const StW& s : u.st) {
        const int C = s.c;
        bf16_t* G = xa + (size_t)B * s.xa_unit;
        bf16_t* U = G + (size_t)B * XA_NP * C;
        o.check(launch_expand_heads(kv + s.kv_off, u.kv_total, B, k, s.heads, 32, XA_NP, 1.0f / sqrtf(32.f), kexp, o.c->stream), "expand K");
        o.check(launch_expand_heads(kv + s.kv_off + C, u.kv_total, B, k, s.heads, 32, XA_NP, 1.0f, vexp, o.c->stream), "expand V");
        o.check(launch_transpose_bf16(o.w<bf16_t>(s.wq2), wqt, C, C, o.c->stream), "transpose Wq");
        {
            IgemmParams p = o.base(B * XA_NP, C, C);
            p.A0 = kexp; p.C0 = C; p.W = wqt; p.out_bf16 = G;
            o.check(launch_igemm(p, false, 1, o.c->stream), "xattn G");
        }
        {
            IgemmParams p = o.base(C, XA_NP, C);
            p.A0 = o.w<bf16_t>(s.wo2); p.C0 = C; p.W = vexp; p.sA = 0; p.sW = (long long)XA_NP * C; p.sO = (long long)C * XA_NP;
            p.out_bf16 = U; p.ldo = XA_NP;
            o.check(launch_igemm(p, false, B, o.c->stream), "xattn U");
        }
        o.check(launch_xattn_pack(G, U, U + (size_t)B * C * XA_NP, U + (size_t)B * C * XA_NP + (size_t)B * XA_NP * C, B, XA_NP, C, o.c->stream), "xattn pack");
    }
}

static void unet_time_rows(Ops& o, UNet& u, const long long* t, int B, float* emb_all) {
    const int mcl = u.cfg.model_channels, mc = pad64(mcl), ted = mcl * 4;
    bf16_t* temb = o.abf((size_t)B * mc);
    if (!o.plan) o.check(launch_timestep_embedding(t, temb, B, mcl, mc, o.c->stream), "timestep_embedding");
    bf16_t* e1 = o.abf((size_t)B * ted);
    o.tag = "time_embed";
    o.linear({.A0 = temb, .C0 = mc, .W = o.w<bf16_t>(u.te0w), .bias = o.w<float>(u.te0b), .M = B, .N = ted, .act = ACT_SILU, .out_bf16 = e1, .single_row = true});
    bf16_t* semb = o.abf((size_t)B * ted);
    o.linear({.A0 = e1, .C0 = ted, .W = o.w<bf16_t>(u.te2w), .bias = o.w<float>(u.te2b), .M = B, .N = ted, .act = ACT_SILU, .out_bf16 = semb, .single_row = true});
    o.linear({.A0 = semb, .C0 = ted, .W = o.w<bf16_t>(u.embw), .bias = o.w<float>(u.embb), .M = B, .N = u.emb_total, .out_f32 = emb_all,
              .single_row = true});
}

static void unet_body(Ops& o, UNet& u, const float* x, const long long* t, const bf16_t* kv, const bf16_t* xa, const int Bfull, int k, int H, int W,
                      float* eps_out, int Bx , int Bshared ,
                      const float* emb_row = nullptr) {
    int B = Bfull;
    const rdm_unet_cfg& c = u.cfg;
    const int mcl = c.model_channels, mc = pad64(mcl);
    const float* emb_all = emb_row;
    const int emb_ld = emb_row ? 0 : u.emb_total;
    if (!emb_row) {
        float* e = o.af32((size_t)B * u.emb_total);
        unet_time_rows(o, u, t, B, e);
        emb_all = e;
    }

    struct Act { bf16_t* p; int C, H, W, L; bool half = false; };
    std::vector<Act> hs;
    Act h{nullptr, 0, H, W, 0};
    B = (Bshared > 0 && Bshared * 2 == Bfull) ? Bshared : Bfull;
    auto expand = [&](Act& a) {
        const size_t n = (size_t)(Bfull / 2) * a.H * a.W * a.C;
        if (!o.plan) o.check(hipMemcpyAsync(a.p + n, a.p, n * 2, hipMemcpyDeviceToDevice, o.c->stream), "expand prefix");
        a.half = false;
    };

    auto resblock = [&](const ResW& r, const Act& a, Act* skip) -> Act {
        const int C0 = a.C, C1 = skip ? skip->C : 0, HW = a.H * a.W, M = B * HW;
        int wrap_b = 0;
        if (skip && skip->half) {
            if (B == Bfull && r.skip && o.lin4_takes({.C0 = C0, .C1 = C1, .M = M, .N = r.cout, .a1_wrap_rows = (Bfull / 2) * HW})) wrap_b = Bfull / 2;
            else expand(*skip);
        }
        const bf16_t* x1 = skip ? skip->p : nullptr;
        const bf16_t* res = a.p;
        bf16_t* sk = nullptr;
        if (r.skip) {
            sk = o.abf((size_t)M * r.cout);
            o.tag = "res.skip";
            o.linear({.A0 = a.p, .A1 = x1, .C0 = C0, .C1 = C1, .W = o.w<bf16_t>(r.wsk), .bias = o.w<float>(r.bsk), .M = M, .N = r.cout, .out_bf16 = sk,
                      .a1_wrap_rows = wrap_b * HW, .sample_rows = HW});
            res = sk;
        }
        bf16_t* n1 = o.abf((size_t)M * r.cin);
        o.tag = "res.gn1";
        o.groupnorm({.x0 = a.p, .x1 = x1, .C0 = C0, .C1 = C1, .HW = HW, .B = B, .L0 = a.L, .L1 = skip ? skip->L : 0,
                     .gamma = o.w<float>(r.gn1g), .beta = o.w<float>(r.gn1b), .eps = 1e-5f, .silu = 1, .out = n1, .x1_bmod = wrap_b});
        o.tap(1, n1, (size_t)M * r.cin * 2);
        bf16_t* h1 = o.abf((size_t)M * r.cout);
        o.tag = "res.conv1";
        o.conv3({.A0 = n1, .C0 = r.cin, .W = o.w<bf16_t>(r.w1), .bias = o.w<float>(r.b1), .B = B, .Hin = a.H, .Win = a.W, .N = r.cout, .out_bf16 = h1,
                 .rowvec = emb_all + r.emb_off, .rowvec_ld = emb_ld});
        o.tap(2, h1, (size_t)M * r.cout * 2);
        bf16_t* n2 = o.abf((size_t)M * r.cout);
        o.tag = "res.gn2";
        o.groupnorm({.x0 = h1, .C0 = r.cout, .HW = HW, .B = B, .L0 = r.lout, .gamma = o.w<float>(r.gn2g), .beta = o.w<float>(r.gn2b), .eps = 1e-5f, .silu = 1, .out = n2});
        o.tap(3, n2, (size_t)M * r.cout * 2);
        if (r.skip) o.tap(4, sk, (size_t)M * r.cout * 2);
        bf16_t* out = o.abf((size_t)Bfull * HW * r.cout);
        o.tag = "res.conv2";
        o.conv3({.A0 = n2, .C0 = r.cout, .W = o.w<bf16_t>(r.w2), .bias = o.w<float>(r.b2), .B = B, .Hin = a.H, .Win = a.W, .N = r.cout, .res_bf16 = res, .out_bf16 = out});
        o.tap(5, out, (size_t)M * r.cout * 2);
        return Act{out, r.cout, a.H, a.W, r.lout};
    };
    auto transformer = [&](const StW& s, const Act& a) -> Act {
        const int C = s.c, n = a.H * a.W, M = B * n;
        const int in_wrap = a.half ? Bfull / 2 : 0;
        bf16_t* xn = o.abf((size_t)M * C);
        o.tag = "st.gn";
        o.groupnorm({.x0 = a.p, .C0 = C, .HW = n, .B = B, .L0 = s.lc, .gamma = o.w<float>(s.gng), .beta = o.w<float>(s.gnb), .eps = 1e-6f, .out = xn, .x0_bmod = in_wrap});
        o.tap(1, xn, (size_t)M * C * 2);
        bf16_t* t0 = o.abf((size_t)M * C);
        o.tag = "st.proj_in";
        o.linear({.A0 = xn, .C0 = C, .W = o.w<bf16_t>(s.win), .bias = o.w<float>(s.bin), .M = M, .N = C, .out_bf16 = t0, .sample_rows = n});
        o.tap(2, t0, (size_t)M * C * 2);
        bf16_t* l1 = o.abf((size_t)M * C);
        const bool vrow = (n % 64 == 0) && s.v_follows;
        const int QW = vrow ? 3 * C : 2 * C;
        bf16_t* qk = o.abf((size_t)M * QW);
        o.tag = "st.norm1+qkv";
        o.layernorm({.x_bf16 = t0, .gamma = o.w<float>(s.ln1g), .beta = o.w<float>(s.ln1b), .M = M, .C = C, .out_bf16 = l1, .Clog = s.lc});
        o.tap(3, l1, (size_t)M * C * 2);
        o.linear({.A0 = l1, .C0 = C, .W = o.w<bf16_t>(s.wqk), .M = M, .N = QW, .out_bf16 = qk, .sample_rows = n});
        o.tap(4, qk, (size_t)M * QW * 2);
        bf16_t* ao = o.abf((size_t)M * C);
        o.tag = "st.self_attention";
        if (vrow) {
            o.flash_d32({.q = qk, .ldq = QW, .v = qk + 2 * C, .out = ao, .n = n}, s.heads, B);
        } else if (n % 32 == 0) {
            bf16_t* vt = o.abf((size_t)M * C);
            if (!o.plan) {
                IgemmParams p = o.base(C, n, C);
                p.A0 = o.w<bf16_t>(s.wv); p.C0 = C; p.W = l1; p.sA = 0; p.sW = (long long)n * C; p.sO = (long long)C * n;
                p.out_bf16 = vt; p.ldo = n;
                o.check(launch_igemm(p, false, B, o.c->stream), "v^T gemm");
            }
            o.flash_d32({.q = qk, .ldq = 2 * C, .vt = vt, .out = ao, .n = n}, s.heads, B);
        } else {
            bf16_t* v = o.abf((size_t)M * C);
            o.linear({.A0 = l1, .C0 = C, .W = o.w<bf16_t>(s.wv), .M = M, .N = C, .out_bf16 = v, .sample_rows = n});
            o.small_attention({.q = qk, .ldq = 2 * C, .k = qk + C, .ldk = 2 * C, .v = v, .ldv = C, .out = ao, .ldo = C, .nq = n, .nkv = n, .scale = 1.0f / sqrtf(32.f)},
                              32, s.heads, B, "small self attention");
        }
        o.tap(5, ao, (size_t)M * C * 2);
        bf16_t* t1 = o.abf((size_t)M * C);
        const int Mx = Bx * n;
        const bool xfused = xa && Mx > 0 && xattn_fused_supported({.rows = Mx, .n = n, .C = C, .NP = XA_NP, .ncols = s.heads * k, .group = k});
        const bool xln = xfused && s.lc == C && C <= 2048;
        const bool xfold_shape = xln && !o.c->deterministic;
        const bool bias_fold = xfold_shape && Bx * 2 == B;
        o.tag = "st.attn1.to_out";
        LinearOp to_out{.A0 = ao, .C0 = C, .W = o.w<bf16_t>(s.wo1), .bias = o.w<float>(s.bo1), .M = M, .N = C, .res_bf16 = t0, .out_bf16 = t1, .sample_rows = n};
        if (bias_fold) {
            const float* zb = o.plan ? nullptr : o.c->zero_bias_pair(o.w<float>(s.bo2), C);
            if (!o.plan && !zb && o.rc == 0) o.rc = o.c->fail(-2, "out of memory for a bias table");
            to_out.rowvec = zb; to_out.rowvec_ld = C; to_out.rows_per_sample = Mx;
        }
        o.linear(to_out);
        o.tap(6, t1, (size_t)M * C * 2);
        o.tag = "st.norm2+attn2";
        bf16_t* l2 = o.abf((size_t)M * C);
        if (Mx > 0 && !xln) o.layernorm({.x_bf16 = t1, .gamma = o.w<float>(s.ln2g), .beta = o.w<float>(s.ln2b), .M = Mx, .C = C, .out_bf16 = l2, .Clog = s.lc});
        bf16_t* t2 = xfold_shape ? t1 : o.abf((size_t)M * C);
        bf16_t* l3 = o.abf((size_t)M * C);
        if (Bx < B && !bias_fold && !o.plan)
            o.check(launch_add_bias_rows(t1 + (size_t)Mx * C, o.w<float>(s.bo2), t2 + (size_t)Mx * C, (long long)(M - Mx), C, o.c->stream), "zero-context cross attention");
        if (Mx == 0) {
        } else if (xa) {
            bf16_t* P = o.abf((size_t)M * XA_NP);
            const bf16_t* G = xa + (size_t)B * s.xa_unit; const bf16_t* U = G + (size_t)B * XA_NP * C;
            const bf16_t* Gp = U + (size_t)B * C * XA_NP; const bf16_t* Up = Gp + (size_t)B * XA_NP * C;
            XattnParams xp{.G = Gp, .U = Up, .bias = o.w<float>(s.bo2), .out = t2, .rows = Mx, .n = n, .C = C, .NP = XA_NP, .ncols = s.heads * k, .group = k};
            if (xln) {
                xp.x = t1; xp.ln_g = o.w<float>(s.ln2g); xp.ln_b = o.w<float>(s.ln2b); xp.ln_eps = 1e-5f;
                if (xfold_shape) { xp.ln3_g = o.w<float>(s.ln3g); xp.ln3_b = o.w<float>(s.ln3b); xp.ln3_out = l3; }
                o.xattn_fused(xp);
            } else if (xfused) {
                xp.x = l2; xp.res = t1;
                o.xattn_fused(xp);
            } else if (!o.plan) {
                IgemmParams p = o.base(n, XA_NP, C);
                p.A0 = l2; p.C0 = C; p.sA = (long long)n * C; p.W = G; p.sW = (long long)XA_NP * C; p.out_bf16 = P; p.sO = (long long)n * XA_NP;
                p.act = ACT_SOFTMAXG; p.sm_group = k;
                o.prof_begin(RDM_PROF_LINEAR, 2.0 * Mx * XA_NP * (double)C);
                o.check(launch_igemm(p, false, Bx, o.c->stream), "xattn scores");
                o.prof_end();
                IgemmParams q = o.base(n, C, XA_NP);
                q.A0 = P; q.C0 = XA_NP; q.sA = (long long)n * XA_NP; q.W = U; q.sW = (long long)C * XA_NP; q.bias = o.w<float>(s.bo2);
                q.res_bf16 = t1; q.out_bf16 = t2; q.sO = (long long)n * C;
                o.prof_begin(RDM_PROF_LINEAR, 2.0 * Mx * C * (double)XA_NP);
                o.check(launch_igemm(q, false, Bx, o.c->stream), "xattn out");
                o.prof_end();
            }
        } else {
            bf16_t* q2 = o.abf((size_t)M * C);
            o.linear({.A0 = l2, .C0 = C, .W = o.w<bf16_t>(s.wq2), .M = Mx, .N = C, .out_bf16 = q2, .sample_rows = n});
            bf16_t* ao2 = o.abf((size_t)M * C);
            o.small_attention({.q = q2, .ldq = C, .k = kv + s.kv_off, .ldk = u.kv_total, .v = kv + s.kv_off + C, .ldv = u.kv_total, .out = ao2, .ldo = C,
                               .nq = n, .nkv = k, .scale = 1.0f / sqrtf(32.f)}, 32, s.heads, Bx, "cross attention");
            o.linear({.A0 = ao2, .C0 = C, .W = o.w<bf16_t>(s.wo2), .bias = o.w<float>(s.bo2), .M = Mx, .N = C, .res_bf16 = t1, .out_bf16 = t2, .sample_rows = n});
        }
        o.tap(7, t2, (size_t)M * C * 2);
        o.tag = "st.norm3+geglu";
        const int FI = 4 * s.lc;
        bf16_t* ff = o.abf((size_t)M * FI);
        const int M3 = xfold_shape ? Mx : 0;
        if (M > M3) o.layernorm({.x_bf16 = t2 + (size_t)M3 * C, .gamma = o.w<float>(s.ln3g), .beta = o.w<float>(s.ln3b), .M = M - M3, .C = C,
                                 .out_bf16 = l3 + (size_t)M3 * C, .Clog = s.lc});
        o.linear({.A0 = l3, .C0 = C, .W = o.w<bf16_t>(s.wff1), .bias = o.w<float>(s.bff1), .M = M, .N = 2 * FI, .act = ACT_GEGLU, .out_bf16 = ff, .sample_rows = n});
        o.tap(8, l3, (size_t)M * C * 2);
        o.tap(9, ff, (size_t)M * FI * 2);
        bf16_t* out = o.abf((size_t)M * C);
        o.tag = "st.ff2*proj_out";
        o.linear({.A0 = ff, .A1 = t2, .C0 = FI, .C1 = C, .W = o.w<bf16_t>(s.wfo), .bias = o.w<float>(s.bfo), .M = M, .N = C, .res_bf16 = a.p, .out_bf16 = out,
                  .res_wrap_rows = in_wrap * n, .sample_rows = n});
        o.tap(10, out, (size_t)M * C * 2);
        return Act{out, C, a.H, a.W, s.lc};
    };

    for (const UBlock& blk : u.blocks) {
        Act* skip = nullptr; Act sk{};
        if (blk.where == 2) { sk = hs.back(); hs.pop_back(); skip = &sk; }
        bool first = true;
        o.cur_block = (int)(&blk - &u.blocks[0]); o.cur_layer = 0;
        for (const ULayer& L : blk.layers) {
            switch (L.kind) {
                case 0: {
                    bf16_t* out = o.abf((size_t)Bfull * H * W * mc);
                    if (!o.plan) o.check(launch_conv_in(x, o.w<float>(u.cinw), o.w<float>(u.cinb), out, B, c.in_channels, H, W, mc, o.c->stream), "conv_in");
                    h = Act{out, mc, H, W, mcl};
                } break;
                case 1: h = resblock(u.res[L.idx], h, (first && skip) ? skip : nullptr); break;
                case 2:
                    if (B < Bfull) {
                        {
                            const StW& s0 = u.st[L.idx];
                            const int n0 = h.H * h.W, Mfull = Bfull * n0;
                            if (!o.c->deterministic && o.lin4_takes({.C0 = 4 * s0.lc, .C1 = s0.c, .M = Mfull, .N = s0.c, .res_wrap_rows = (Bfull / 2) * n0})) h.half = true;
                            else expand(h);
                        }
                        for (Act& a : hs) { if (o.c->deterministic) expand(a); else a.half = true; }
                        B = Bfull;
                    }
                    h = transformer(u.st[L.idx], h); break;
                case 3: {
                    const ConvW& d = u.down[L.idx];
                    bf16_t* out = o.abf((size_t)Bfull * (h.H / 2) * (h.W / 2) * d.c);
                    o.tag = "downsample";
                    o.conv3({.A0 = h.p, .C0 = d.c, .W = o.w<bf16_t>(d.w), .bias = o.w<float>(d.b), .B = B, .Hin = h.H, .Win = h.W, .N = d.c, .stride = 2, .out_bf16 = out});
                    h = Act{out, d.c, h.H / 2, h.W / 2, d.lc};
                } break;
                case 4: {
                    const ConvW& d = u.up[L.idx];
                    bf16_t* out = o.abf((size_t)Bfull * (h.H * 2) * (h.W * 2) * d.c);
                    o.tag = "upsample";
                    o.conv3({.A0 = h.p, .C0 = d.c, .W = o.w<bf16_t>(d.w), .bias = o.w<float>(d.b), .B = B, .Hin = h.H, .Win = h.W, .N = d.c, .ups = 1, .out_bf16 = out});
                    h = Act{out, d.c, h.H * 2, h.W * 2, d.lc};
                } break;
            }
            first = false;
            o.cur_layer++;
        }
        if (blk.where == 0) hs.push_back(h);
        if (!o.plan && o.c->tap_buf && o.c->tap_sub == 0 && o.c->tap_block == (int)(&blk - &u.blocks[0])) {
            size_t nb = (size_t)B * h.H * h.W * h.C * 2; if (nb > o.c->tap_bytes) nb = o.c->tap_bytes;
            o.check(hipMemcpyAsync(o.c->tap_buf, h.p, nb, hipMemcpyDeviceToDevice, o.c->stream), "debug tap");
        }
    }
    if (B < Bfull) { expand(h); B = Bfull; }
    bf16_t* no = o.abf((size_t)B * H * W * mc);
    bf16_t* hwp = o.abf(head_conv_wp_bytes(mc) / 2);
    o.tag = "out_head";
    o.head({.x = h.p, .B = B, .H = H, .W = W, .C = mc, .gamma = o.w<float>(u.outg), .beta = o.w<float>(u.outb), .eps = 1e-5f, .w = o.w<float>(u.outw), .wp = hwp,
            .bias = o.w<float>(u.outbias), .out = eps_out, .Cout = c.out_channels}, mcl, no);
}

int unet_forward_impl(rdm_ctx* c, const float* x, const int64_t* t, const float* context, const bf16_t* kv_cached,
                      int b, int k, int H, int W, float* eps_out, int ctx_rows, int shared_half, const float* emb_row) {
    UNet& u = c->unet;
    if (!u.loaded) return c->fail(-1, "unet weights not loaded");
    const int down = 1 << (u.cfg.n_channel_mult - 1);
    if (b < 1 || k < 1 || H % down || W % down) return c->fail(-1, "bad unet_forward shape b=%d k=%d H=%d W=%d", b, k, H, W);
    if (k > 256) return c->fail(-1, "k=%d neighbours exceeds the cross-attention kernel limit (256)", k);
    RDM_TRY(ensure_gn_partial(c, b));
    return run_with_arena(c, u.arena, u.blob, [&](Ops& o) {
        const bf16_t* kv = kv_cached;
        const bf16_t* xa = (kv_cached && xattn_skinny_ok(u, k)) ? u.xa_cache : nullptr;
        if (!kv) {
            bf16_t* kvb = o.abf((size_t)b * k * u.kv_total);
            unet_compute_kv(o, u, context, b, k, kvb);
            kv = kvb;
            if (xattn_skinny_ok(u, k)) {
                bf16_t* xab = o.abf((size_t)b * u.xa_total);
                unet_compute_xattn(o, u, kv, b, k, xab);
                xa = xab;
            }
        }
        unet_body(o, u, x, (const long long*)t, kv, xa, b, k, H, W, eps_out, (ctx_rows >= 0 && ctx_rows <= b) ? ctx_rows : b, shared_half, emb_row);
    });
}

int rdm_unet_forward(rdm_ctx* c, const float* x, const int64_t* t, const float* context, int b, int k, int H, int W,
                     float* eps_out) {
    RDM_ENTER(c);
    if (!c || !x || !t || !context || !eps_out) return c ? c->fail(-1, "null argument") : -1;
    return unet_forward_impl(c, x, t, context, nullptr, b, k, H, W, eps_out);
}

int rdm_debug_tap(rdm_ctx* c, void* buf, size_t nbytes, int block, int sub) {
    if (!c) return -1;
    c->tap_buf = buf; c->tap_bytes = buf ? nbytes : 0; c->tap_block = buf ? block : -1; c->tap_sub = buf ? sub : 0;
    return 0;
}

int unet_prepare_kv(rdm_ctx* c, float* cat, const float* cond, const float* uncond, int B, int k) {
    UNet& u = c->unet;
    const int nb = uncond ? 2 * B : B;
    const size_t cd = u.cfg.context_dim;
    RDM_TRY(ensure_bytes(c, (char**)&u.kv_cache, &u.kv_cache_bytes, (size_t)nb * k * u.kv_total * 2));
    RDM_CHECK_HIP(c, hipMemcpyAsync(cat, cond, (size_t)B * k * cd * 4, hipMemcpyDeviceToDevice, c->stream));
    if (uncond) RDM_CHECK_HIP(c, hipMemcpyAsync(cat + (size_t)B * k * cd, uncond, (size_t)B * k * cd * 4, hipMemcpyDeviceToDevice, c->stream));
    const bool skinny = xattn_skinny_ok(u, k);
    if (skinny) RDM_TRY(ensure_bytes(c, (char**)&u.xa_cache, &u.xa_cache_bytes, (size_t)nb * u.xa_total * 2));
    u.ctx_rows = nb;
    if (uncond) {
        std::vector<int> flags(nb, 1);
        int* dflags = (int*)c->gn_partial;
        RDM_TRY(ensure_gn_partial(c, nb));
        dflags = (int*)c->gn_partial;
        RDM_CHECK_HIP(c, launch_row_nonzero(cat, nb, (long long)k * cd, dflags, c->stream));
        RDM_CHECK_HIP(c, hipMemcpyAsync(flags.data(), dflags, (size_t)nb * 4, hipMemcpyDeviceToHost, c->stream));
        RDM_CHECK_HIP(c, hipStreamSynchronize(c->stream));
        int rows = nb;
        while (rows > 0 && flags[rows - 1] == 0) rows--;
        if (!c->deterministic) u.ctx_rows = rows;
    }
    return run_with_arena(c, u.arena, u.blob, [&](Ops& o) {
        unet_compute_kv(o, u, cat, nb, k, u.kv_cache);
        if (skinny) unet_compute_xattn(o, u, u.kv_cache, nb, k, u.xa_cache);
    });
}

int unet_emb_table(rdm_ctx* c, const std::vector<int>& ts, const float** table) {
    *table = nullptr;
    if (c->deterministic) return 0;
    UNet& u = c->unet;
    const size_t total = ts.size();
    RDM_TRY(ensure_bytes(c, (char**)&u.emb_table, &u.emb_table_bytes, total * u.emb_total * 4 + total * 8 + 256));
    long long* tuniq = (long long*)((char*)u.emb_table + ((total * u.emb_total * 4 + 255) & ~(size_t)255));
    std::vector<long long> th(ts.begin(), ts.end());
    RDM_CHECK_HIP(c, hipMemcpyAsync(tuniq, th.data(), total * 8, hipMemcpyHostToDevice, c->stream));
    RDM_CHECK_HIP(c, hipStreamSynchronize(c->stream));
    RDM_TRY(run_with_arena(c, u.arena, u.blob, [&](Ops& o) { unet_time_rows(o, u, tuniq, (int)total, u.emb_table); }));
    *table = u.emb_table;
    return 0;
}
```

Baseline: 39.77 images/s.

## Extend CFG shared-prefix computation through first transformer self-attention

With classifier-free guidance, the cond and uncond halves share an identical prefix until cross-attention. Previously the batch was expanded to full size before the first transformer. Now the transformer's groupnorm, proj_in, layernorm, QKV and self-attention run on half the rows. The attn1 output projection then reads the half-size activations through a new a0 wrap-rows mode in the lin4 GEMM, with choice_rows keeping kernel selection as if at full size. This adds complexity to GEMM dispatch and depends on the lin4 path accepting the wrapped shapes, falling back to explicit copies otherwise.

```diff
diff --git a/include/rdm_hip.h b/include/rdm_hip.h
--- a/include/rdm_hip.h
+++ b/include/rdm_hip.h
@@ -221,6 +221,7 @@
 int rdm_calib_probe(rdm_ctx* ctx, void* buf , size_t buf_bytes, double mfma_ms, size_t stream_bytes, int stream_reps,
                     double* mfma_tflops , double* stream_gbps );
 int rdm_debug_tap(rdm_ctx* ctx, void* buf , size_t nbytes, int block, int sub);
+int rdm_debug_guidance_prefix(rdm_ctx* ctx, int through_attn1);
 
 int rdm_op_linear(rdm_ctx* ctx, const void* a_bf16, const void* w_bf16, const float* bias, const void* residual_bf16,
                   void* out_bf16, float* out_f32, int M, int N, int K, int act, float alpha);
diff --git a/retrieval-augmented-diffusion-models_amd/_lib.py b/retrieval-augmented-diffusion-models_amd/_lib.py
--- a/retrieval-augmented-diffusion-models_amd/_lib.py
+++ b/retrieval-augmented-diffusion-models_amd/_lib.py
@@ -184,6 +184,7 @@
     "rdm_prof_reset": (C.c_int, [_P]),
     "rdm_prof_dump": (C.c_int, [_P, C.c_char_p]),
     "rdm_debug_tap": (C.c_int, [_P, _P, C.c_size_t, C.c_int, C.c_int]),
+    "rdm_debug_guidance_prefix": (C.c_int, [_P, C.c_int]),
     "rdm_calib_probe": (C.c_int, [_P, _P, C.c_size_t, C.c_double, C.c_size_t, C.c_int, C.POINTER(C.c_double), C.POINTER(C.c_double)]),
     "rdm_comm_unique_id": (C.c_int, [_P, _P]),
     "rdm_comm_init": (C.c_int, [_P, _P, C.c_int, C.c_int]),
@@ -1318,6 +1319,9 @@
         self._tap_keepalive = buf
         self._check(lib.rdm_debug_tap(self._h, _ptr(buf) if buf is not None else None, 0 if buf is None else buf.numel() * buf.element_size(), int(block), int(sub)))
 
+    def debug_guidance_prefix(self, through_attn1=1):
+        self._check(lib.rdm_debug_guidance_prefix(self._h, int(through_attn1)))
+
     def calib_probe(self, mfma_ms=800.0, stream_bytes=1 << 30, stream_reps=6):
         buf = torch.empty(max(1 << 20, 2 * stream_bytes), device=self.device, dtype=torch.uint8)
         tf, gb = C.c_double(0.0), C.c_double(0.0)
diff --git a/retrieval-augmented-diffusion-models_amd/csrc/common.h b/retrieval-augmented-diffusion-models_amd/csrc/common.h
--- a/retrieval-augmented-diffusion-models_amd/csrc/common.h
+++ b/retrieval-augmented-diffusion-models_amd/csrc/common.h
@@ -94,6 +94,8 @@
     const bf16_t* Wfrag;
     const float* ln_sb; float ln_inv_c, ln_eps;
     int dbg;
+    int a0_wrap_rows;
+    int choice_rows;
 };
 inline IgemmParams igemm_plain(int M, int N, int K, const void* zero_page) {
     IgemmParams p{}; p.M = M; p.N = N; p.K = K; p.alpha = 1.f; p.ldo = N; p.zero_page = zero_page;
diff --git a/retrieval-augmented-diffusion-models_amd/csrc/dispatch.hip b/retrieval-augmented-diffusion-models_amd/csrc/dispatch.hip
--- a/retrieval-augmented-diffusion-models_amd/csrc/dispatch.hip
+++ b/retrieval-augmented-diffusion-models_amd/csrc/dispatch.hip
@@ -41,16 +41,20 @@
 bool Ops::lin4_takes(const LinearOp& op) {
     if (c->deterministic) return false;
     IgemmParams t = base(op.M, op.N, op.C0 + op.C1);
-    t.C0 = op.C0; t.C1 = op.C1; t.W = (const bf16_t*)blob; t.Wfrag = t.W; t.out_bf16 = (bf16_t*)blob; t.a1_wrap_rows = op.a1_wrap_rows;
+    t.C0 = op.C0; t.C1 = op.C1; t.W = (const bf16_t*)blob; t.Wfrag = t.W; t.out_bf16 = (bf16_t*)blob;
+    t.a0_wrap_rows = op.a0_wrap_rows; t.a1_wrap_rows = op.a1_wrap_rows;
+    if (op.rowvec) { t.rowvec = op.rowvec; t.rowvec_ld = op.rowvec_ld; t.rows_per_sample = op.rows_per_sample; }
     if (op.res_wrap_rows > 0) { t.res_bf16 = (const bf16_t*)blob; t.res_wrap_rows = op.res_wrap_rows; }
     return lin4_supported(t, 1);
 }
 void Ops::linear(const LinearOp& op) {
     if (plan) return;
     const int M = op.M, N = op.N, K = op.C0 + op.C1;
-    if (!op.A1 && op.C1 == 0 && !op.rowvec && op.alpha == 1.f) {
+    if (!op.A1 && op.C1 == 0 && !op.rowvec && op.alpha == 1.f && op.a0_wrap_rows == 0 && op.res_wrap_rows == 0) {
         SgemmParams q = skinny_params(op);
+        if (op.choice_rows > M) q.M = op.choice_rows;
         const int kernel = linear_kernel(q, c->deterministic, op.single_row);
+        q.M = M;
         if (kernel != RDM_LINEAR_ROWS_TILED) {
             const bool mid = kernel == RDM_LINEAR_ROWS_MGEMM;
             prof_begin(RDM_PROF_LINEAR, 2.0 * M * N * (double)K, M, N, K);
@@ -62,7 +66,7 @@
     IgemmParams p = base(M, N, K);
     p.A0 = op.A0; p.A1 = op.A1; p.C0 = op.C0; p.C1 = op.C1; p.W = op.W; p.bias = op.bias; p.alpha = op.alpha;
     p.act = op.act; p.res_bf16 = op.res_bf16; p.res_f32 = op.res_f32; p.out_bf16 = op.out_bf16; p.out_f32 = op.out_f32;
-    p.a1_wrap_rows = op.a1_wrap_rows; p.res_wrap_rows = op.res_wrap_rows;
+    p.a0_wrap_rows = op.a0_wrap_rows; p.a1_wrap_rows = op.a1_wrap_rows; p.res_wrap_rows = op.res_wrap_rows; p.choice_rows = op.choice_rows;
     if (op.rowvec) { p.rowvec = op.rowvec; p.rowvec_ld = op.rowvec_ld; p.rows_per_sample = op.rows_per_sample; }
     if (op.act == ACT_GEGLU) p.ldo = N / 2;
     {
@@ -118,10 +122,13 @@
     check(launch_conv3x3(p, c->stream), "conv3x3");
     prof_end();
 }
-void Ops::tap(int stage, const void* ptr, size_t nbytes) {
+void Ops::tap(int stage, const void* ptr, size_t nbytes, bool twice) {
     if (plan || !c->tap_buf || c->tap_block != cur_block || c->tap_sub != cur_layer * 16 + stage) return;
-    if (nbytes > c->tap_bytes) nbytes = c->tap_bytes;
-    check(hipMemcpyAsync(c->tap_buf, ptr, nbytes, hipMemcpyDeviceToDevice, c->stream), "debug tap");
+    const size_t n0 = nbytes > c->tap_bytes ? c->tap_bytes : nbytes;
+    check(hipMemcpyAsync(c->tap_buf, ptr, n0, hipMemcpyDeviceToDevice, c->stream), "debug tap");
+    if (!twice || c->tap_bytes <= nbytes) return;
+    const size_t n1 = c->tap_bytes - nbytes < nbytes ? c->tap_bytes - nbytes : nbytes;
+    check(hipMemcpyAsync((char*)c->tap_buf + nbytes, ptr, n1, hipMemcpyDeviceToDevice, c->stream), "debug tap");
 }
 void Ops::prof_begin(int kind, double work, int d0, int d1, int d2) {
     prof_open = (c->prof >> kind) & 1u;
diff --git a/retrieval-augmented-diffusion-models_amd/csrc/host.h b/retrieval-augmented-diffusion-models_amd/csrc/host.h
--- a/retrieval-augmented-diffusion-models_amd/csrc/host.h
+++ b/retrieval-augmented-diffusion-models_amd/csrc/host.h
@@ -193,6 +193,7 @@
     }
     bool deterministic = rdm_env_int(getenv("RDM_DETERMINISTIC"), 0) != 0;
     void* tap_buf = nullptr; size_t tap_bytes = 0; int tap_block = -1, tap_sub = 0;
+    int prefix_through_attn1 = 1;
     void* rccl_lib = nullptr; void* comm = nullptr; int comm_world = 0;
     unsigned prof = 0;
     struct ProfRec { hipEvent_t a, b; int kind; double flops; const char* tag; int d0, d1, d2; };
@@ -228,10 +229,11 @@
     const bf16_t* res_bf16 = nullptr; const float* res_f32 = nullptr;
     bf16_t* out_bf16 = nullptr; float* out_f32 = nullptr;
     const float* rowvec = nullptr; int rowvec_ld = 0, rows_per_sample = 1;
-    int a1_wrap_rows = 0, res_wrap_rows = 0;
+    int a0_wrap_rows = 0, a1_wrap_rows = 0, res_wrap_rows = 0;
     float alpha = 1.f;
     bool single_row = false;
     int sample_rows = 0;
+    int choice_rows = 0;
 };
 struct Conv3Op {
     const bf16_t* A0 = nullptr; const bf16_t* A1 = nullptr; int C0 = 0, C1 = 0;
@@ -271,7 +273,7 @@
     bool linear_ln(const LinearOp& op);
     void conv3(const Conv3Op& op);
     int cur_block = -1, cur_layer = 0;
-    void tap(int stage, const void* ptr, size_t nbytes);
+    void tap(int stage, const void* ptr, size_t nbytes, bool twice = false);
     bool prof_open = false;
     const char* tag = "";
     void prof_begin(int kind, double work, int d0 = 0, int d1 = 0, int d2 = 0);
diff --git a/retrieval-augmented-diffusion-models_amd/csrc/igemm.hip b/retrieval-augmented-diffusion-models_amd/csrc/igemm.hip
--- a/retrieval-augmented-diffusion-models_amd/csrc/igemm.hip
+++ b/retrieval-augmented-diffusion-models_amd/csrc/igemm.hip
@@ -537,10 +537,11 @@
                                   !(p.sm_group == 1 || p.sm_group == 2 || p.sm_group == 4)))
         return hipErrorInvalidValue;
     const bool wide = (p.N % 192 == 0);
-    const long long tiles256 = (long long)((p.M + 255) / 256) * ((p.N + (wide ? 191 : 127)) / (wide ? 192 : 128)) * batch;
+    const int Mc = p.choice_rows > p.M ? p.choice_rows : p.M;
+    const long long tiles256 = (long long)((Mc + 255) / 256) * ((p.N + (wide ? 191 : 127)) / (wide ? 192 : 128)) * batch;
     const bool tall = tiles256 >= 256 && p.M > 128;
     if (!conv && p.Wfrag && lin4_supported(p, batch)) return launch_lin4(p, st);
-    if (p.a1_wrap_rows > 0 || p.res_wrap_rows > 0) return hipErrorInvalidValue;
+    if (p.a0_wrap_rows > 0 || p.a1_wrap_rows > 0 || p.res_wrap_rows > 0) return hipErrorInvalidValue;
     if (p.act == ACT_GEGLU) {
         if (conv) return hipErrorInvalidValue;
         if (tall && p.N % 256 == 0 && (long long)((p.M + 255) / 256) * (p.N / 256) * batch >= 256)
diff --git a/retrieval-augmented-diffusion-models_amd/csrc/lin4.hip b/retrieval-augmented-diffusion-models_amd/csrc/lin4.hip
--- a/retrieval-augmented-diffusion-models_amd/csrc/lin4.hip
+++ b/retrieval-augmented-diffusion-models_amd/csrc/lin4.hip
@@ -61,11 +61,12 @@
     return ((unsigned long long)hi << 32) | lo;
 }
 __device__ __forceinline__ ASrc l4_asrc(bool dead, int row0, int kc, int C0, const char* A0p, const char* A1p, unsigned ld0, unsigned ld1,
-                                        const char* zero, unsigned voffA0, unsigned voffA1, unsigned lane16, int wrap1) {
+                                        const char* zero, unsigned voffA0, unsigned voffA1, unsigned lane16, int wrap0, int wrap1) {
     ASrc s;
     const bool second = kc >= C0;
     const unsigned ld = second ? ld1 : ld0;
     if (second && row0 >= wrap1) row0 -= wrap1;
+    if (!second && row0 >= wrap0) row0 -= wrap0;
     const char* b = (second ? A1p : A0p) + (unsigned long long)row0 * ld + (unsigned)((second ? kc - C0 : kc) * 2);
     s.base = (const char*)l4_uni64((unsigned long long)(dead ? zero : b));
     s.pstride = (unsigned)__builtin_amdgcn_readfirstlane((int)(dead ? 0u : 32u * ld));
@@ -105,6 +106,7 @@
     const char* const zero = (const char*)p.zero_page;
     const char* const Wf = (const char*)p.Wfrag;
     const unsigned ld0 = (unsigned)(p.lda > 0 ? p.lda : p.C0) * 2u, ld1 = (unsigned)p.C1 * 2u;
+    const int wrap0 = p.a0_wrap_rows > 0 ? p.a0_wrap_rows : 0x7fffffff;
     const int wrap1 = p.a1_wrap_rows > 0 ? p.a1_wrap_rows : 0x7fffffff;
 
     unsigned vbase[FM];
@@ -133,7 +135,7 @@
         return (const char*)l4_uni64((unsigned long long)(Wf + off));
     };
     auto a_src = [&](const Cur& c) __attribute__((always_inline)) {
-        return l4_asrc(c.tile >= t_end, c.bm * BM, c.sl * BK, C0, A0p, A1p, ld0, ld1, zero, voffA0, voffA1, lane16, wrap1);
+        return l4_asrc(c.tile >= t_end, c.bm * BM, c.sl * BK, C0, A0p, A1p, ld0, ld1, zero, voffA0, voffA1, lane16, wrap0, wrap1);
     };
 
     asm volatile("" ::: H4_ACC_CLOBBERS);
@@ -498,9 +500,11 @@
     if (p.C1 > 0 && p.lda > 0) return false;
     if (p.res_wrap_rows > 0 && (!p.res_bf16 || p.res_wrap_rows % (128 * wm) != 0 || 2LL * p.res_wrap_rows < p.M)) return false;
     if (p.a1_wrap_rows > 0 && (p.C1 == 0 || p.a1_wrap_rows % (128 * wm) != 0 || 2LL * p.a1_wrap_rows < p.M)) return false;
+    if (p.a0_wrap_rows > 0 && (p.a0_wrap_rows % (128 * wm) != 0 || 2LL * p.a0_wrap_rows < p.M)) return false;
     if (p.ln_sb && (p.C1 > 0 || p.K < 128 || p.res_bf16 || p.bias || lin4_smem_bytes(p, wm) > 160 * 1024 || !(p.ln_inv_c > 0.f))) return false;
     constexpr int L4_MIN_TILES = 128;
-    if (!p.l4_any_tiles && (long long)(p.M / (128 * wm)) * (p.N / (wm == 1 ? 384 : 192)) < L4_MIN_TILES) return false;
+    const int Mc = p.choice_rows > p.M ? p.choice_rows : p.M;
+    if (!p.l4_any_tiles && (long long)(Mc / (128 * wm)) * (p.N / (wm == 1 ? 384 : 192)) < L4_MIN_TILES) return false;
     return true;
 }
 
diff --git a/retrieval-augmented-diffusion-models_amd/csrc/unet_exec.hip b/retrieval-augmented-diffusion-models_amd/csrc/unet_exec.hip
--- a/retrieval-augmented-diffusion-models_amd/csrc/unet_exec.hip
+++ b/retrieval-augmented-diffusion-models_amd/csrc/unet_exec.hip
@@ -77,6 +77,14 @@
         if (!o.plan) o.check(hipMemcpyAsync(a.p + n, a.p, n * 2, hipMemcpyDeviceToDevice, o.c->stream), "expand prefix");
         a.half = false;
     };
+    auto leave_prefix = [&](const StW& s0, Act& in) {
+        const int n0 = in.H * in.W, Mfull = Bfull * n0;
+        if (!o.c->deterministic && o.lin4_takes({.C0 = 4 * s0.lc, .C1 = s0.c, .M = Mfull, .N = s0.c, .res_wrap_rows = (Bfull / 2) * n0})) in.half = true;
+        else expand(in);
+        for (Act& a : hs) { if (o.c->deterministic) expand(a); else a.half = true; }
+        B = Bfull;
+    };
+    const bool through_attn1 = o.c->prefix_through_attn1 && !o.c->deterministic;
 
     auto resblock = [&](const ResW& r, const Act& a, Act* skip) -> Act {
         const int C0 = a.C, C1 = skip ? skip->C : 0, HW = a.H * a.W, M = B * HW;
@@ -116,54 +124,64 @@
         o.tap(5, out, (size_t)M * r.cout * 2);
         return Act{out, r.cout, a.H, a.W, r.lout};
     };
-    auto transformer = [&](const StW& s, const Act& a) -> Act {
-        const int C = s.c, n = a.H * a.W, M = B * n;
-        const int in_wrap = a.half ? Bfull / 2 : 0;
-        bf16_t* xn = o.abf((size_t)M * C);
+    auto transformer = [&](const StW& s, Act& a) -> Act {
+        const int C = s.c, n = a.H * a.W;
+        const bool pre = B < Bfull;
+        const int Bs = B, Ms = Bs * n, M = Bfull * n;
+        const int Mx = Bx * n;
+        const bool xfused = xa && Mx > 0 && xattn_fused_supported({.rows = Mx, .n = n, .C = C, .NP = XA_NP, .ncols = s.heads * k, .group = k});
+        const bool xln = xfused && s.lc == C && C <= 2048;
+        const bool xfold_shape = xln && !o.c->deterministic;
+        const bool bias_fold = xfold_shape && Bx * 2 == Bfull;
+        const bool pre_wrap = pre && o.lin4_takes({.C0 = C, .M = M, .N = C, .rowvec = bias_fold ? o.w<float>(s.bo2) : nullptr ,
+                                                   .rowvec_ld = C, .rows_per_sample = Mx, .a0_wrap_rows = Ms, .res_wrap_rows = Ms});
+        const size_t Mh = pre_wrap ? Ms : M;
+        bf16_t* xn = o.abf((size_t)Ms * C);
         o.tag = "st.gn";
-        o.groupnorm({.x0 = a.p, .C0 = C, .HW = n, .B = B, .L0 = s.lc, .gamma = o.w<float>(s.gng), .beta = o.w<float>(s.gnb), .eps = 1e-6f, .out = xn, .x0_bmod = in_wrap});
-        o.tap(1, xn, (size_t)M * C * 2);
-        bf16_t* t0 = o.abf((size_t)M * C);
+        o.groupnorm({.x0 = a.p, .C0 = C, .HW = n, .B = Bs, .L0 = s.lc, .gamma = o.w<float>(s.gng), .beta = o.w<float>(s.gnb), .eps = 1e-6f, .out = xn,
+                     .x0_bmod = a.half ? Bfull / 2 : 0});
+        o.tap(1, xn, (size_t)Ms * C * 2, pre);
+        bf16_t* t0 = o.abf(Mh * C);
         o.tag = "st.proj_in";
-        o.linear({.A0 = xn, .C0 = C, .W = o.w<bf16_t>(s.win), .bias = o.w<float>(s.bin), .M = M, .N = C, .out_bf16 = t0, .sample_rows = n});
-        o.tap(2, t0, (size_t)M * C * 2);
-        bf16_t* l1 = o.abf((size_t)M * C);
+        o.linear({.A0 = xn, .C0 = C, .W = o.w<bf16_t>(s.win), .bias = o.w<float>(s.bin), .M = Ms, .N = C, .out_bf16 = t0, .sample_rows = n, .choice_rows = M});
+        o.tap(2, t0, (size_t)Ms * C * 2, pre);
+        bf16_t* l1 = o.abf((size_t)Ms * C);
         const bool vrow = (n % 64 == 0) && s.v_follows;
         const int QW = vrow ? 3 * C : 2 * C;
-        bf16_t* qk = o.abf((size_t)M * QW);
+        bf16_t* qk = o.abf((size_t)Ms * QW);
         o.tag = "st.norm1+qkv";
-        o.layernorm({.x_bf16 = t0, .gamma = o.w<float>(s.ln1g), .beta = o.w<float>(s.ln1b), .M = M, .C = C, .out_bf16 = l1, .Clog = s.lc});
-        o.tap(3, l1, (size_t)M * C * 2);
-        o.linear({.A0 = l1, .C0 = C, .W = o.w<bf16_t>(s.wqk), .M = M, .N = QW, .out_bf16 = qk, .sample_rows = n});
-        o.tap(4, qk, (size_t)M * QW * 2);
-        bf16_t* ao = o.abf((size_t)M * C);
+        o.layernorm({.x_bf16 = t0, .gamma = o.w<float>(s.ln1g), .beta = o.w<float>(s.ln1b), .M = Ms, .C = C, .out_bf16 = l1, .Clog = s.lc});
+        o.tap(3, l1, (size_t)Ms * C * 2, pre);
+        o.linear({.A0 = l1, .C0 = C, .W = o.w<bf16_t>(s.wqk), .M = Ms, .N = QW, .out_bf16 = qk, .sample_rows = n, .choice_rows = M});
+        o.tap(4, qk, (size_t)Ms * QW * 2, pre);
+        bf16_t* ao = o.abf(Mh * C);
         o.tag = "st.self_attention";
         if (vrow) {
-            o.flash_d32({.q = qk, .ldq = QW, .v = qk + 2 * C, .out = ao, .n = n}, s.heads, B);
+            o.flash_d32({.q = qk, .ldq = QW, .v = qk + 2 * C, .out = ao, .n = n}, s.heads, Bs);
         } else if (n % 32 == 0) {
-            bf16_t* vt = o.abf((size_t)M * C);
+            bf16_t* vt = o.abf((size_t)Ms * C);
             if (!o.plan) {
                 IgemmParams p = o.base(C, n, C);
                 p.A0 = o.w<bf16_t>(s.wv); p.C0 = C; p.W = l1; p.sA = 0; p.sW = (long long)n * C; p.sO = (long long)C * n;
                 p.out_bf16 = vt; p.ldo = n;
-                o.check(launch_igemm(p, false, B, o.c->stream), "v^T gemm");
+                o.check(launch_igemm(p, false, Bs, o.c->stream), "v^T gemm");
             }
-            o.flash_d32({.q = qk, .ldq = 2 * C, .vt = vt, .out = ao, .n = n}, s.heads, B);
+            o.flash_d32({.q = qk, .ldq = 2 * C, .vt = vt, .out = ao, .n = n}, s.heads, Bs);
         } else {
-            bf16_t* v = o.abf((size_t)M * C);
-            o.linear({.A0 = l1, .C0 = C, .W = o.w<bf16_t>(s.wv), .M = M, .N = C, .out_bf16 = v, .sample_rows = n});
+            bf16_t* v = o.abf((size_t)Ms * C);
+            o.linear({.A0 = l1, .C0 = C, .W = o.w<bf16_t>(s.wv), .M = Ms, .N = C, .out_bf16 = v, .sample_rows = n, .choice_rows = M});
             o.small_attention({.q = qk, .ldq = 2 * C, .k = qk + C, .ldk = 2 * C, .v = v, .ldv = C, .out = ao, .ldo = C, .nq = n, .nkv = n, .scale = 1.0f / sqrtf(32.f)},
-                              32, s.heads, B, "small self attention");
-        }
-        o.tap(5, ao, (size_t)M * C * 2);
+                              32, s.heads, Bs, "small self attention");
+        }
+        o.tap(5, ao, (size_t)Ms * C * 2, pre);
+        if (pre) {
+            leave_prefix(s, a);
+            if (!pre_wrap) { Act t0a{t0, C, a.H, a.W, s.lc}, aoa{ao, C, a.H, a.W, s.lc}; expand(t0a); expand(aoa); }
+        }
         bf16_t* t1 = o.abf((size_t)M * C);
-        const int Mx = Bx * n;
-        const bool xfused = xa && Mx > 0 && xattn_fused_supported({.rows = Mx, .n = n, .C = C, .NP = XA_NP, .ncols = s.heads * k, .group = k});
-        const bool xln = xfused && s.lc == C && C <= 2048;
-        const bool xfold_shape = xln && !o.c->deterministic;
-        const bool bias_fold = xfold_shape && Bx * 2 == B;
         o.tag = "st.attn1.to_out";
         LinearOp to_out{.A0 = ao, .C0 = C, .W = o.w<bf16_t>(s.wo1), .bias = o.w<float>(s.bo1), .M = M, .N = C, .res_bf16 = t0, .out_bf16 = t1, .sample_rows = n};
+        if (pre_wrap) to_out.a0_wrap_rows = to_out.res_wrap_rows = Ms;
         if (bias_fold) {
             const float* zb = o.plan ? nullptr : o.c->zero_bias_pair(o.w<float>(s.bo2), C);
             if (!o.plan && !zb && o.rc == 0) o.rc = o.c->fail(-2, "out of memory for a bias table");
@@ -226,7 +244,7 @@
         bf16_t* out = o.abf((size_t)M * C);
         o.tag = "st.ff2*proj_out";
         o.linear({.A0 = ff, .A1 = t2, .C0 = FI, .C1 = C, .W = o.w<bf16_t>(s.wfo), .bias = o.w<float>(s.bfo), .M = M, .N = C, .res_bf16 = a.p, .out_bf16 = out,
-                  .res_wrap_rows = in_wrap * n, .sample_rows = n});
+                  .res_wrap_rows = a.half ? (Bfull / 2) * n : 0, .sample_rows = n});
         o.tap(10, out, (size_t)M * C * 2);
         return Act{out, C, a.H, a.W, s.lc};
     };
@@ -245,16 +263,7 @@
                 } break;
                 case 1: h = resblock(u.res[L.idx], h, (first && skip) ? skip : nullptr); break;
                 case 2:
-                    if (B < Bfull) {
-                        {
-                            const StW& s0 = u.st[L.idx];
-                            const int n0 = h.H * h.W, Mfull = Bfull * n0;
-                            if (!o.c->deterministic && o.lin4_takes({.C0 = 4 * s0.lc, .C1 = s0.c, .M = Mfull, .N = s0.c, .res_wrap_rows = (Bfull / 2) * n0})) h.half = true;
-                            else expand(h);
-                        }
-                        for (Act& a : hs) { if (o.c->deterministic) expand(a); else a.half = true; }
-                        B = Bfull;
-                    }
+                    if (B < Bfull && !through_attn1) leave_prefix(u.st[L.idx], h);
                     h = transformer(u.st[L.idx], h); break;
                 case 3: {
                     const ConvW& d = u.down[L.idx];
@@ -323,6 +332,12 @@
 int rdm_debug_tap(rdm_ctx* c, void* buf, size_t nbytes, int block, int sub) {
     if (!c) return -1;
     c->tap_buf = buf; c->tap_bytes = buf ? nbytes : 0; c->tap_block = buf ? block : -1; c->tap_sub = buf ? sub : 0;
+    return 0;
+}
+
+int rdm_debug_guidance_prefix(rdm_ctx* c, int through_attn1) {
+    if (!c) return -1;
+    c->prefix_through_attn1 = through_attn1 != 0;
     return 0;
 }
 
```

Result: faster. 40.19 images/s, median of 6 (+1.1%).
